# TheClimateCorporation/photon-ml

Hardware: AMD Instinct MI355X
Metric: examples/sec/node, logistic L-BFGS 1B×1M-sparse (higher is better)
Workload: dtype bf16; 1 GPU; model=logistic_regression_l2_lbfgs, global_batch=125000000, rows_per_gpu=125000000, features=1000000, nnz_per_row=100, parallelism=dp1, optimizer_state=replicated, layout=tiled

## Files before the change

### photon_ml_amd/data/synthetic.py

```python
from __future__ import annotations

import math
from typing import Optional

import numpy as np
import scipy.sparse as sp
import torch

from ..constants import TaskType
from .matrix import LabeledData


INLIER_PROBABILITY = 0.90
INLIER_STANDARD_DEVIATION = 1e-3
OUTLIER_STANDARD_DEVIATION = 1.0
SAMPLE_KINDS = ("benign", "outlier", "invalid_features", "invalid_labels")


def draw_samples(task, kind: str, seed: int, size: int, dimensionality: int,
                 desired_sparsity: float = 0.1) -> LabeledData:
    task = TaskType.parse(task)
    if kind not in SAMPLE_KINDS:
        raise ValueError(f"unknown sample kind {kind!r}, expected one of {SAMPLE_KINDS}")
    rng = np.random.default_rng(5000 * seed)
    n, d = int(size), int(dimensionality)
    u = rng.random(n)
    binary = task in (TaskType.LOGISTIC_REGRESSION, TaskType.SMOOTHED_HINGE_LOSS_LINEAR_SVM)
    if kind == "invalid_labels":
        y = np.array([np.inf, -np.inf, np.nan])[rng.integers(0, 3, n)]
        x0 = 0.1 + 0.9 * u
    elif binary:
        y = (rng.random(n) <= 0.5).astype(np.float64)
        x0 = np.where(y == 1.0, 1.0, -1.0) * (0.1 + 0.9 * u)
    elif task == TaskType.POISSON_REGRESSION:
        y = 1.0 + 10.0 * u
        x0 = (np.log(y) + rng.normal(size=n) * INLIER_STANDARD_DEVIATION) / np.log(11.0)
    elif kind == "benign":
        y = 2.0 * u - 1.0
        x0 = y + rng.normal(size=n) * INLIER_STANDARD_DEVIATION
    else:
        y = 1.0 + u
        x0 = y - 1.0 + rng.normal(size=n) * OUTLIER_STANDARD_DEVIATION
    tail_end = d - 3 if kind == "invalid_features" else d
    mask = rng.random((n, max(tail_end - 1, 0))) < desired_sparsity
    rows, cols = np.nonzero(mask)
    cols = cols + 1
    k = rows.size
    if kind in ("benign", "invalid_labels"):
        vals = 2.0 * (rng.random(k) - 0.5)
    else:
        inlier = rng.random(k) < INLIER_PROBABILITY
        if kind == "outlier":
            bad = np.where(rng.random(k) < 0.5, 1.0, -1.0)
        else:
            bad = np.array([np.nan, np.inf, -np.inf])[rng.integers(0, 3, k)]
        vals = np.where(inlier, rng.normal(size=k) * INLIER_STANDARD_DEVIATION, bad)
    r_all = [np.arange(n), rows]
    c_all = [np.zeros(n, np.int64), cols]
    v_all = [x0, vals]
    if kind == "invalid_features":
        for j, v in zip((d - 3, d - 2, d - 1), (np.nan, np.inf, -np.inf)):
            r_all.append(np.arange(n))
            c_all.append(np.full(n, j))
            v_all.append(np.full(n, v))
    x = sp.csr_matrix((np.concatenate(v_all), (np.concatenate(r_all), np.concatenate(c_all))), shape=(n, d))
    x.sort_indices()
    return LabeledData(x, y)


def generate_glm_data(task, n_rows: int, n_features: int, density: float = 0.2, seed: int = 7,
                      intercept: bool = True, noise: float = 1e-3, kind: str = "benign"):
    task = TaskType.parse(task)
    rng = np.random.default_rng(seed)
    d_feat = n_features - (1 if intercept else 0)
    x = sp.random(n_rows, d_feat, density=density, format="csr", random_state=seed,
                  data_rvs=lambda k: rng.uniform(-1, 1, size=k))
    if kind == "outlier":
        x.data *= np.where(rng.random(x.data.size) < 0.01, 1e3, 1.0)
    if intercept:
        x = sp.hstack([x, np.ones((n_rows, 1))], format="csr")
    w = rng.normal(size=n_features)
    z = x @ w
    if task == TaskType.LOGISTIC_REGRESSION or task == TaskType.SMOOTHED_HINGE_LOSS_LINEAR_SVM:
        y = (rng.random(n_rows) < 1.0 / (1.0 + np.exp(-z))).astype(np.float64)
    elif task == TaskType.POISSON_REGRESSION:
        w *= 0.2
        z = x @ w
        y = rng.poisson(np.exp(np.clip(z, -20, 5))).astype(np.float64)
    else:
        y = z + rng.normal(scale=noise, size=n_rows)
    if kind == "invalid":
        y[0] = np.nan
    return LabeledData(x, y), w


def zipf_cdf(n: int, s: float, device) -> torch.Tensor:
    k = torch.arange(1, n + 1, dtype=torch.float64, device=device)
    p = k.pow(-s)
    c = torch.cumsum(p, 0)
    return (c / c[-1]).to(torch.float32)


def generate_device_shard(n_rows: int, n_features: int, nnz_per_row: int, device="cuda", precision: str = "bf16",
                          seed: int = 1234567890, chunk_rows: int = 1 << 20, zipf_s: float = 1.1,
                          task=TaskType.LOGISTIC_REGRESSION, rank: int = 0, progress=None, layout: str = "auto"):
    from ..ops.device import DeviceGLMData, SegChunk, VAL_DTYPE, resolve_layout
    from ..ops.tiled import TLFwdChunk, TLTChunk

    dev = torch.device(device)
    prec = {"bf16": 0, "f32": 1, "f64": 2}[precision]
    vdt = VAL_DTYPE[prec]
    n_fields = nnz_per_row - 1
    if n_fields < 1:
        raise ValueError("nnz_per_row must be >= 2 (intercept + >= 1 field)")
    fs = (n_features - 1) // n_fields
    if fs < 1:
        raise ValueError("not enough features for the requested nnz per row")
    layout = resolve_layout(layout, n_features, chunk_rows)
    cdf = zipf_cdf(fs, zipf_s, dev)
    field_base = (torch.arange(n_fields, device=dev, dtype=torch.int32) * fs)
    gen = torch.Generator(device=dev)
    gen.manual_seed(seed + 7919 * rank)
    starts = list(range(0, n_rows, chunk_rows)) + [n_rows]
    k = nnz_per_row
    raw = []
    counts = torch.zeros(n_features, dtype=torch.int64, device=dev)
    for ci, (a, b) in enumerate(zip(starts[:-1], starts[1:])):
        m = b - a
        u = torch.rand((m, n_fields), generator=gen, device=dev)
        rank_ = torch.searchsorted(cdf, u).clamp_(max=fs - 1).to(torch.int32)
        del u
        idx = torch.empty((m, k), dtype=torch.int32, device=dev)
        idx[:, :n_fields] = rank_ + field_base
        idx[:, n_fields] = n_features - 1
        del rank_
        val = torch.empty((m, k), dtype=torch.float32, device=dev)
        val[:, :n_fields] = torch.rand((m, n_fields), generator=gen, device=dev) + 0.5
        val[:, n_fields] = 1.0
        idx = idx.reshape(-1)
        counts += torch.bincount(idx.to(torch.int64), minlength=n_features)
        raw.append((idx, val.to(vdt).reshape(-1)))
        if (m + 1) * k >= 2 ** 31:
            raise ValueError("chunk too large for int32 offsets: lower chunk_rows")
    import torch.distributed as dist
    from ..parallel.dist import is_dist
    if is_dist():
        cc = counts if dist.get_backend() == "nccl" else counts.cpu()
        dist.all_reduce(cc)
        counts = cc.to(dev)
    old_of_new = torch.argsort(counts, descending=True, stable=True)
    new_of_old = torch.empty_like(old_of_new)
    new_of_old[old_of_new] = torch.arange(n_features, device=dev)
    new_of_old32 = new_of_old.to(torch.int32)
    del counts
    csr, csc = [], []
    from ..ops.tiled import shard_t_config
    cbits, item_entries = shard_t_config(n_rows * k, n_rows, n_features, chunk_rows)
    for ci, ((a, b), (idx, val)) in enumerate(zip(zip(starts[:-1], starts[1:]), raw)):
        m = b - a
        idx = new_of_old32[idx.to(torch.int64)]
        if layout == "tiled":
            rp = torch.arange(0, (m + 1) * k, k, dtype=torch.int64, device=dev)
            col = idx.to(torch.int64)
            del idx
            csr.append(TLFwdChunk(rp, col, val, n_features))
            csc.append(TLTChunk(rp, col, val, n_features, chunk_rows, cbits=cbits, item_entries=item_entries))
            raw[ci] = None
            del col, val, rp
            if progress is not None:
                progress(ci + 1, len(starts) - 1)
            continue
        seg_ptr = np.arange(0, (m + 1) * k, k, dtype=np.int64).astype(np.int32)
        csr.append(SegChunk(seg_ptr, idx, val, dev, forward=True))
        perm = torch.argsort(idx, stable=True)
        cidx = (perm // k).to(torch.int32)
        cval = val[perm]
        colptr = torch.zeros(n_features + 1, dtype=torch.int64, device=dev)
        colptr[1:] = torch.cumsum(torch.bincount(idx.to(torch.int64), minlength=n_features), 0)
        del perm
        csc.append(SegChunk(colptr.cpu().numpy().astype(np.int32), cidx, cval, dev))
        raw[ci] = None
        del cidx, cval, colptr, idx, val
        if progress is not None:
            progress(ci + 1, len(starts) - 1)
    y = torch.zeros(n_rows, dtype=torch.float32, device=dev)
    data = DeviceGLMData(csr, csc, starts, y, torch.zeros_like(y), torch.ones_like(y), n_features, precision, dev,
                         old_of_new)
    wgen = torch.Generator(device=dev)
    wgen.manual_seed(seed)
    w_true = torch.randn(n_features, generator=wgen, device=dev, dtype=torch.float64) * 0.3
    w_true[torch.rand(n_features, generator=wgen, device=dev) < 0.5] = 0.0
    w_true[-1] = -1.0
    z = data.margins(w_true)
    p = torch.sigmoid(z)
    task = TaskType.parse(task)
    if task == TaskType.LOGISTIC_REGRESSION:
        yy = (torch.rand(n_rows, generator=gen, device=dev, dtype=torch.float64) < p).to(torch.float32)
    elif task == TaskType.POISSON_REGRESSION:
        yy = torch.poisson(torch.exp(z.clamp(max=5.0)) * 0.2, generator=gen).to(torch.float32)
    else:
        yy = (z + 0.1 * torch.randn(n_rows, generator=gen, device=dev, dtype=torch.float64)).to(torch.float32)
    data.y.copy_(yy.to(data.vdt))
    return data, w_true


def _device_csr_to_host(counts: torch.Tensor, cols: torch.Tensor, vals: torch.Tensor, n_cols: int) -> sp.csr_matrix:
    indptr = torch.zeros(counts.numel() + 1, dtype=torch.int64, device=counts.device)
    torch.cumsum(counts, 0, out=indptr[1:])
    x = sp.csr_matrix((vals.cpu().numpy(), cols.to(torch.int32).cpu().numpy(), indptr.cpu().numpy()),
                      shape=(counts.numel(), n_cols))
    x.has_canonical_format = True
    return x


def generate_game_bench_data_device(n_entities: int, rows_per_entity: int, re_dim: int = 100, re_nnz: int = 10,
                                    fe_dim: int = 100_000, fe_nnz: int = 30, re_vocab: int = 1 << 20, seed: int = 7,
                                    entity_offset: int = 0, task: str = "LOGISTIC_REGRESSION", pool: str = "random",
                                    int_ids: bool = False, sizes: str = "uniform", size_alpha: float = 1.3,
                                    max_rows: int = 20000, device="cuda", label_bias: float = 0.0,
                                    heavy_rows=()):
    from ..data.game_data import GameData
    dev = torch.device(device)
    gen = torch.Generator(device=dev)
    gen.manual_seed(int(seed))
    rnd = lambda *shape: torch.rand(shape, generator=gen, device=dev, dtype=torch.float64)
    if sizes == "powerlaw":
        if pool == "exact":
            raise ValueError("pool='exact' needs equal entity sizes")
        u = rnd(n_entities)
        target = n_entities * rows_per_entity
        xm = float(rows_per_entity) * (size_alpha - 1) / size_alpha
        for _ in range(30):
            cnt = torch.clamp(torch.ceil(xm * u ** (-1.0 / size_alpha)), max=max_rows).to(torch.int64)
            tot = int(cnt.sum())
            if abs(tot - target) <= 0.001 * target:
                break
            xm *= target / tot
    elif sizes == "uniform":
        cnt = torch.full((n_entities,), rows_per_entity, dtype=torch.int64, device=dev)
    else:
        raise ValueError(f"unknown entity size law {sizes!r}")
    if len(heavy_rows):
        cnt[:len(heavy_rows)] = torch.tensor([int(r) for r in heavy_rows], dtype=torch.int64, device=dev)
    n = int(cnt.sum())
    ent_sorted = torch.repeat_interleave(torch.arange(n_entities, device=dev), cnt, output_size=n)
    perm = torch.randperm(n, generator=gen, device=dev)
    ent = ent_sorted[perm]
    p = torch.arange(1, fe_dim, device=dev, dtype=torch.float64) ** -1.1
    cdf = torch.cumsum(p, 0)
    cdf /= cdf[-1].clone()
    fcol = torch.searchsorted(cdf, rnd(n, fe_nnz)).clamp_(max=fe_dim - 2)
    fcol, _ = torch.sort(fcol, dim=1)
    keep = torch.ones_like(fcol, dtype=torch.bool)
    keep[:, 1:] = fcol[:, 1:] != fcol[:, :-1]
    fval = rnd(n, fe_nnz) + 0.5
    fcol = torch.cat([fcol, torch.full((n, 1), fe_dim - 1, device=dev, dtype=fcol.dtype)], 1)
    fval = torch.cat([fval, torch.ones(n, 1, device=dev, dtype=torch.float64)], 1)
    keep = torch.cat([keep, torch.ones(n, 1, device=dev, dtype=torch.bool)], 1)
    xg = _device_csr_to_host(keep.sum(1), fcol[keep], fval[keep], fe_dim)
    wg = torch.randn(fe_dim, generator=gen, device=dev, dtype=torch.float64) * 0.2
    wg[-1] = -0.5
    zg = (fval * wg[fcol] * keep).sum(1)
    del fcol, fval, keep
    if pool == "exact":
        if re_nnz > re_dim:
            raise ValueError("pool='exact' needs re_nnz <= re_dim")
        start = torch.zeros(n_entities, dtype=torch.int64, device=dev)
        torch.cumsum(cnt[:-1], 0, out=start[1:])
        within = perm - start[ent]
        slot = (within[:, None] * re_nnz + torch.arange(re_nnz, device=dev)[None, :]) % re_dim
        del within, start
    else:
        slot = torch.randint(0, re_dim, (n, re_nnz), generator=gen, device=dev)
    del ent_sorted, perm
    gid = ent + entity_offset
    base = (gid * 2654435761) % (re_vocab - 1)
    rcol = (base[:, None] + slot * 40503) % (re_vocab - 1)
    rval = torch.randn(n, re_nnz, generator=gen, device=dev, dtype=torch.float64)
    wgen = torch.Generator(device=dev)
    wgen.manual_seed(int(seed) + 1)
    w_slot = torch.randn(re_dim, generator=wgen, device=dev, dtype=torch.float64) * 0.5
    rcol, order = torch.sort(rcol, dim=1)
    slot = torch.gather(slot, 1, order)
    rval = torch.gather(rval, 1, order)
    del order
    rkeep = torch.ones_like(rcol, dtype=torch.bool)
    rkeep[:, 1:] = rcol[:, 1:] != rcol[:, :-1]
    zr = (rval * w_slot[slot] * rkeep).sum(1) + 0.3 * torch.sin(gid.to(torch.float64))
    del slot
    rcol = torch.cat([rcol, torch.full((n, 1), re_vocab - 1, device=dev, dtype=rcol.dtype)], 1)
    rval = torch.cat([rval, torch.ones(n, 1, device=dev, dtype=torch.float64)], 1)
    rkeep = torch.cat([rkeep, torch.ones(n, 1, device=dev, dtype=torch.bool)], 1)
    xr = _device_csr_to_host(rkeep.sum(1), rcol[rkeep], rval[rkeep], re_vocab)
    del rcol, rval, rkeep
    z = zg + zr
    task = TaskType.parse(task)
    if task == TaskType.LOGISTIC_REGRESSION:
        y = (rnd(n) < torch.sigmoid(z + label_bias)).to(torch.float64)
    elif task == TaskType.POISSON_REGRESSION:
        y = torch.poisson(torch.exp(torch.clamp(z * 0.3, -10, 3)), generator=gen)
    else:
        y = z + 0.1 * torch.randn(n, generator=gen, device=dev, dtype=torch.float64)
    gid_h = gid.cpu().numpy()
    ids = gid_h.copy() if int_ids else np.char.add("e", gid_h.astype(str)).astype(object)
    return GameData(y.cpu().numpy(), {"global": xg, "entity": xr}, {"entityId": ids})


def generate_game_bench_data(n_entities: int, rows_per_entity: int, re_dim: int = 100, re_nnz: int = 10,
                             fe_dim: int = 100_000, fe_nnz: int = 30, re_vocab: int = 1 << 20, seed: int = 7,
                             entity_offset: int = 0, task: str = "LOGISTIC_REGRESSION", pool: str = "random",
                             int_ids: bool = False, sizes: str = "uniform", size_alpha: float = 1.3,
                             max_rows: int = 20000):
    from ..data.game_data import GameData
    rng = np.random.default_rng(seed)
    if sizes == "powerlaw":
        if pool == "exact":
            raise ValueError("pool='exact' needs equal entity sizes")
        u = rng.random(n_entities)
# ... 75 lines not shown
```

### photon_ml_amd/ops/csrc/game_kernels.hip

```cpp

#include <hip/hip_runtime.h>
#include <stdint.h>

#include <algorithm>

#ifndef PML_BUILD_ID
#define PML_BUILD_ID "unstamped-build!"
#endif
__attribute__((used)) static const char pml_build_stamp[] = "PML_BUILD_ID=" PML_BUILD_ID;

#define LAUNCH_CHECK()                                         \
  do {                                                         \
    hipError_t e_ = hipGetLastError();                         \
    if (e_ != hipSuccess) return (int)e_;                      \
  } while (0)

#define SCORE_GROUP 16
#define SCORE_THREADS 256
#define SCORE_ROWS_PER_BLOCK (SCORE_THREADS / SCORE_GROUP)

template <bool RE>
__global__ __launch_bounds__(SCORE_THREADS) void score_rows_kernel(
    const long long* __restrict__ indptr, const int* __restrict__ col, const double* __restrict__ val,
    long long n_rows, const double* __restrict__ w, const int* __restrict__ ent,
    const long long* __restrict__ eptr, const int* __restrict__ efeat, double* __restrict__ out) {
  const long long row = (long long)blockIdx.x * SCORE_ROWS_PER_BLOCK + (threadIdx.x / SCORE_GROUP);
  const int g = threadIdx.x % SCORE_GROUP;
  double s = 0.0;
  if (row < n_rows) {
    const long long lo = indptr[row], hi = indptr[row + 1];
    long long e_lo = 0, e_hi = 0;
    bool ok = true;
    if (RE) {
      const int e = ent[row];
      if (e < 0) ok = false;
      else { e_lo = eptr[e]; e_hi = eptr[e + 1]; }
    }
    if (ok) {
      for (long long p = lo + g; p < hi; p += SCORE_GROUP) {
        const int c = col[p];
        double wv;
        if (RE) {
          long long a = e_lo, b = e_hi;
          while (a < b) {
            const long long m = (a + b) >> 1;
            if (efeat[m] < c) a = m + 1; else b = m;
          }
          wv = (a < e_hi && efeat[a] == c) ? w[a] : 0.0;
        } else {
          wv = w[c];
        }
        s += val[p] * wv;
      }
    }
  }
#pragma unroll
  for (int o = SCORE_GROUP / 2; o > 0; o >>= 1) s += __shfl_xor(s, o, SCORE_GROUP);
  if (g == 0 && row < n_rows) out[row] = s;
}

typedef double v4d __attribute__((ext_vector_type(4)));

__device__ __forceinline__ v4d mfma_f64_16x16x4(double a, double b, v4d c) {
  return __builtin_amdgcn_mfma_f64_16x16x4f64(a, b, c, 0, 0, 0);
}


#define GN_T 32
#define GN_K 32
__global__ __launch_bounds__(256) void gemm_nt_mfma_kernel(int M, int N, int K, const double* __restrict__ A, int lda,
                                                            const double* __restrict__ Bm, int ldb,
                                                            double* __restrict__ C, int ldc) {
  __shared__ double sa[GN_T][GN_K + 1];
  __shared__ double sb[GN_T][GN_K + 1];
  const int tn = blockIdx.x, tm = blockIdx.y;
  const int lane = threadIdx.x & 63, wv = threadIdx.x >> 6;
  const int wm = wv >> 1, wn = wv & 1;
  v4d acc = {0.0, 0.0, 0.0, 0.0};
  for (int k0 = 0; k0 < K; k0 += GN_K) {
    __syncthreads();
    for (int idx = threadIdx.x; idx < GN_T * GN_K; idx += 256) {
      const int r = idx / GN_K, c = idx % GN_K;
      const int gr = tm * GN_T + r, gc = k0 + c;
      sa[r][c] = (gr < M && gc < K) ? A[(long long)gr * lda + gc] : 0.0;
      const int hr = tn * GN_T + r;
      sb[r][c] = (hr < N && gc < K) ? Bm[(long long)hr * ldb + gc] : 0.0;
    }
    __syncthreads();
#pragma unroll
    for (int kk = 0; kk < GN_K; kk += 4) {
      const double a = sa[16 * wm + (lane & 15)][kk + (lane >> 4)];
      const double b = sb[16 * wn + (lane & 15)][kk + (lane >> 4)];
      acc = mfma_f64_16x16x4(a, b, acc);
    }
  }
  const int cj = tn * GN_T + 16 * wn + (lane & 15);
#pragma unroll
  for (int i = 0; i < 4; ++i) {
    const int ri = tm * GN_T + 16 * wm + (lane >> 4) + 4 * i;
    if (ri < M && cj < N) C[(long long)ri * ldc + cj] = acc[i];
  }
}

__global__ __launch_bounds__(256) void spmm_rows_kernel(const long long* __restrict__ indptr,
                                                         const int* __restrict__ col, const double* __restrict__ val,
                                                         long long n_rows, const double* __restrict__ PT, int k,
                                                         double* __restrict__ Y) {
  const long long row = (long long)blockIdx.x * 4 + (threadIdx.x >> 6);
  const int lane = threadIdx.x & 63;
  if (row >= n_rows) return;
  const long long lo = indptr[row], hi = indptr[row + 1];
  for (int j0 = 0; j0 < k; j0 += 64) {
    const int j = j0 + lane;
    double acc = 0.0;
    for (long long p = lo; p < hi; ++p) {
      const double v = val[p];
      const long long c = col[p];
      if (j < k) acc += v * PT[c * k + j];
    }
    if (j < k) Y[row * k + j] = acc;
  }
}

__device__ __forceinline__ unsigned long long splitmix64(unsigned long long x) {
  x += 0x9E3779B97F4A7C15ull;
  x = (x ^ (x >> 30)) * 0xBF58476D1CE4E5B9ull;
  x = (x ^ (x >> 27)) * 0x94D049BB133111EBull;
  return x ^ (x >> 31);
}

template <typename T>
__global__ __launch_bounds__(256) void downsample_kernel(const T* __restrict__ y, const T* __restrict__ w0,
                                                          const long long* __restrict__ rowid, long long n,
                                                          unsigned long long seed, double rate, int binary,
                                                          T* __restrict__ w) {
  const long long i = (long long)blockIdx.x * 256 + threadIdx.x;
  if (i >= n) return;
  const unsigned long long id = rowid ? (unsigned long long)rowid[i] : (unsigned long long)i;
  const double u = (double)(splitmix64(seed ^ splitmix64(id)) >> 11) * 0x1.0p-53;
  const double wi = (double)w0[i];
  double out;
  if (binary) {
    const bool pos = (double)y[i] >= 0.5;
    out = pos ? wi : (u < rate ? wi / rate : 0.0);
  } else {
    out = u < rate ? wi : 0.0;
  }
  w[i] = (T)out;
}

#define CMP_SEG 8
struct CmpArgs {
  const int* units;
  int col_e, row_col;
  const int* seg;
  int nseg, sbits, key_is_row;
  const uint32_t* pack;
  const void* val;
  const uint16_t* npack;
  const void* nval;
  const int* nbase;
  const unsigned char* keep;
  int* seg_cnt;
  const long long* seg_first;
  const long long* unit_lo;
  uint32_t* opack;
  void* oval;
};

template <typename VT, int PASS>
__global__ __launch_bounds__(256) void tl_compact_kernel(CmpArgs a) {
  const int lane = threadIdx.x & 63;
  const int s = __builtin_amdgcn_readfirstlane(blockIdx.x * 4 + (threadIdx.x >> 6));
  if (s >= a.nseg) return;
  const int* sg = a.seg + 3 * (long long)s;
  const int u = sg[0], r_lo = sg[1], r_hi = sg[2];
  const int* ut = a.units + 6 * (long long)u;
  const long long e_lo = ut[a.col_e];
  const int nw = ut[a.col_e + 1] - ut[a.col_e];
  const int n_lo = ut[4], nn = ut[5] - ut[4];
  const uint32_t row0 = a.row_col >= 0 ? (uint32_t)ut[a.row_col] : 0u;
  const uint32_t smask = (1u << a.sbits) - 1u;
  const VT* val = (const VT*)a.val;
  const VT* nval = (const VT*)a.nval;
  long long ob = PASS ? a.seg_first[s] : 0;
  const long long olo = PASS ? a.unit_lo[u] : 0;
  const unsigned long long below = (1ull << lane) - 1ull;
  int cnt = 0;
  for (int r = r_lo; r < r_hi; ++r) {
    uint32_t p[4];
    VT v[4];
    bool ok[4];
    if (r < nn) {
      const long long q = (long long)n_lo + r;
      const int base = a.nbase[q];
#pragma unroll
      for (int k = 0; k < 4; ++k) {
        const long long pe = nval ? q * 256 + 4 * lane + k : q * 512 + 8 * lane + k;
        const uint32_t p16 = a.npack[pe];
        p[k] = ((uint32_t)(base + (int)(p16 >> a.sbits)) << a.sbits) | (p16 & smask);
        v[k] = nval ? nval[pe] : ((const VT*)a.npack)[pe + 4];
        ok[k] = true;
      }
    } else {
      const int w = r - nn;
#pragma unroll
      for (int k = 0; k < 4; ++k) {
        ok[k] = 256 * w + 64 * k + lane < nw;
        const long long e = e_lo + 256LL * w + 4 * lane + k;
        p[k] = ok[k] ? a.pack[e] : 0u;
        v[k] = ok[k] ? val[e] : (VT)0;
      }
    }
#pragma unroll
    for (int k = 0; k < 4; ++k) {
      const uint32_t row = a.key_is_row ? (p[k] >> a.sbits) : row0 + (p[k] & smask);
      const bool kp = ok[k] && a.keep[row];
      const unsigned long long m = __ballot(kp);
      if (PASS) {
        if (kp) {
          const long long o = ob + __popcll(m & below);
          const long long ph = olo + (o & ~255LL) + ((o & 63) << 2) + ((o & 255) >> 6);
          a.opack[ph] = p[k];
          ((VT*)a.oval)[ph] = v[k];
        }
        ob += __popcll(m);
      } else {
        cnt += __popcll(m);
      }
    }
  }
  if (!PASS && lane == 0) a.seg_cnt[s] = cnt;
}


template <int S, bool STAGE>
__global__ __launch_bounds__(64) void seg_gram_kernel(int B, int n, int dmax, const long long* __restrict__ ents,
                                                      const long long* __restrict__ row_ptr,
                                                      const long long* __restrict__ col_ptr,
                                                      const long long* __restrict__ nip,
                                                      const long long* __restrict__ pos,
                                                      const double* __restrict__ val, double* __restrict__ K) {
  extern __shared__ double img[];
  const int lane = threadIdx.x;
  const long long b = blockIdx.x;
  if (b >= B) return;
  const long long e = ents[b];
  const long long r0 = row_ptr[e];
  const int ne = (int)(row_ptr[e + 1] - r0);
  const long long cb = col_ptr[e];
  const int de = (int)(col_ptr[e + 1] - cb);
  const long long e0 = nip[r0];
  const int enz = (int)(nip[r0 + ne] - e0);
  double* sval = img + (size_t)dmax * S;
  unsigned short* scol = (unsigned short*)(sval + enz);
  int* sptr = (int*)(scol + ((enz + 3) & ~3));
  for (int c = lane; c < de * S; c += 64) img[c] = 0.0;
  if (STAGE) {
    for (int t = lane; t < enz; t += 64) {
      sval[t] = val[e0 + t];
      scol[t] = (unsigned short)(pos[e0 + t] - cb);
    }
    for (int i = lane; i <= ne; i += 64) sptr[i] = (int)(nip[r0 + i] - e0);
  }
  __syncthreads();
  double* Kb = K + b * (long long)n * n;
  for (int i0 = 0; i0 < ne; i0 += S) {
    const int ns = ne - i0 < S ? ne - i0 : S;
    for (int s = 0; s < ns; ++s) {
      if (STAGE) {
        const int ib = sptr[i0 + s], ie = sptr[i0 + s + 1];
        for (int t = ib + lane; t < ie; t += 64) img[(int)scol[t] * S + s] = sval[t];
      } else {
        const long long ib = nip[r0 + i0 + s], ie = nip[r0 + i0 + s + 1];
        for (long long t = ib + lane; t < ie; t += 64) img[(pos[t] - cb) * S + s] = val[t];
      }
    }
    __syncthreads();
    for (int j = lane; j < n; j += 64) {
      double acc[S];
#pragma unroll
      for (int s = 0; s < S; ++s) acc[s] = 0.0;
      if (j < ne) {
        if (STAGE) {
          const int jb = sptr[j], je = sptr[j + 1];
          for (int t = jb; t < je; ++t) {
            const double v = sval[t];
            const double* im = img + (int)scol[t] * S;
#pragma unroll
            for (int s = 0; s < S; ++s) acc[s] = fma(v, im[s], acc[s]);
          }
        } else {
          const long long jb = nip[r0 + j], je = nip[r0 + j + 1];
          for (long long t = jb; t < je; ++t) {
            const double v = val[t];
            const double* im = img + (pos[t] - cb) * S;
#pragma unroll
            for (int s = 0; s < S; ++s) acc[s] = fma(v, im[s], acc[s]);
          }
        }
      }
#pragma unroll
      for (int s = 0; s < S; ++s)
        if (s < ns) Kb[(long long)j * n + i0 + s] = acc[s];
    }
    __syncthreads();
    for (int s = 0; s < ns; ++s) {
      if (STAGE) {
        const int ib = sptr[i0 + s], ie = sptr[i0 + s + 1];
        for (int t = ib + lane; t < ie; t += 64) img[(int)scol[t] * S + s] = 0.0;
      } else {
        const long long ib = nip[r0 + i0 + s], ie = nip[r0 + i0 + s + 1];
        for (long long t = ib + lane; t < ie; t += 64) img[(pos[t] - cb) * S + s] = 0.0;
      }
    }
    __syncthreads();
  }
  for (int i = ne; i < n; ++i)
    for (int j = lane; j < n; j += 64) Kb[(long long)j * n + i] = 0.0;
}

__global__ __launch_bounds__(64) void batched_chol_kernel(int B, int n, const long long* __restrict__ nv,
                                                          double* __restrict__ K, int* __restrict__ info) {
  extern __shared__ double Lp[];
  const int lane = threadIdx.x;
  const long long b = blockIdx.x;
  if (b >= B) return;
  const int m = (int)nv[b];
  double* Kb = K + b * (long long)n * n;
  for (int i = lane; i < n; i += 64)
    for (int k = 0; k <= i; ++k)
      Lp[i * (i + 1) / 2 + k] = (i < m && k < m) ? Kb[(long long)i * n + k] : (i == k ? 1.0 : 0.0);
  __syncthreads();
  int bad = 0;
  for (int j = 0; j < m && !bad; ++j) {
    const int rj = j * (j + 1) / 2;
    double djj = Lp[rj + j];
    for (int k = 0; k < j; ++k) djj = fma(-Lp[rj + k], Lp[rj + k], djj);
    __syncthreads();
    if (!(djj > 0.0) || !isfinite(djj)) { bad = j + 1; break; }
    const double ljj = sqrt(djj);
    for (int i = j + 1 + lane; i < m; i += 64) {
      const int ri = i * (i + 1) / 2;
      double a = Lp[ri + j];
      for (int k = 0; k < j; ++k) a = fma(-Lp[ri + k], Lp[rj + k], a);
      Lp[ri + j] = a / ljj;
    }
    if (lane == 0) Lp[rj + j] = ljj;
    __syncthreads();
  }
  if (lane == 0) info[b] = bad;
  for (int i = lane; i < n; i += 64)
    for (int k = 0; k < n; ++k) Kb[(long long)i * n + k] = k <= i ? Lp[i * (i + 1) / 2 + k] : 0.0;
}

template <typename PT>
__global__ __launch_bounds__(64) void rs_primal_kernel(const long long* __restrict__ ents,
                                                       const long long* __restrict__ row_ptr,
                                                       const long long* __restrict__ col_ptr,
                                                       const long long* __restrict__ nip,
                                                       const PT* __restrict__ pos,
                                                       const double* __restrict__ val, const double* __restrict__ r,
                                                       double* __restrict__ W) {
  extern __shared__ double acc[];
  const int lane = threadIdx.x;
  const long long e = ents[blockIdx.x];
  const long long r0 = row_ptr[e], r1 = row_ptr[e + 1], c0 = col_ptr[e];
  const int d = (int)(col_ptr[e + 1] - c0);
  for (int j = lane; j < d; j += 64) acc[j] = 0.0;
// ... 1005 lines not shown
```

### photon_ml_amd/ops/csrc/glm_kernels.hip

```cpp

#include <hip/hip_runtime.h>
#include <stdint.h>
#include <math.h>
#include <algorithm>
#include <type_traits>

#define NB 4096
#define NTHREADS 256
#define VEC 8
#define MAXSEG 1024

#define LAUNCH_CHECK()                                         \
  do {                                                         \
    hipError_t e_ = hipGetLastError();                         \
    if (e_ != hipSuccess) return (int)e_;                      \
  } while (0)

enum LossId { LOSS_LOGISTIC = 0, LOSS_POISSON = 1, LOSS_SQUARED = 2, LOSS_HINGE = 3 };
enum FwdMode { FWD_MARGIN = 0, FWD_VALUE_GRAD = 1, FWD_HV = 2, FWD_DZZ = 3, FWD_LS = 4 };

struct bf16x8 { uint4 u; };

template <typename VT, typename AT> struct Loader;
template <> struct Loader<uint16_t, float> {
// ... 605 lines not shown
}

template <typename VT, typename XT, typename AT, bool SQ, int U, int NW>
__device__ __forceinline__ void tl_stream_p1(const uint32_t* __restrict__ pack, const VT* __restrict__ val,
                                          const XT* __restrict__ x, int e_lo, int e_hi, int sbits, AT* acc) {
  typedef typename TLValT<VT>::T LT;
  typedef typename TLVals<VT>::Raw Raw;
  const int lane = threadIdx.x & 63, w = threadIdx.x >> 6;
  const uint32_t smask = (1u << sbits) - 1u;
  const int lo = e_lo & ~(TL_VEC - 1);
  const int nr = (e_hi - lo + TL_ROUND - 1) / TL_ROUND;
  const int r0 = (nr * w) / NW, r1 = (nr * (w + 1)) / NW;
  if (r0 >= r1) return;
  auto load_round = [&](int r, v4u& pk, Raw& v) {
    const int e = lo + r * TL_ROUND + lane * TL_VEC;
    const int es = (r < r1 && e < e_hi) ? e : lo;
    pk = ldg_nt((const v4u*)(pack + es));
    v = TLVals<VT>::load(val + es);
  };
  auto gather = [&](int r, const v4u& pk, XT* xv) {
    const int e = lo + r * TL_ROUND + lane * TL_VEC;
#pragma unroll
    for (int k = 0; k < TL_VEC; ++k) {
      const bool in = (r < r1) && (e + k >= e_lo) && (e + k < e_hi);
      xv[k] = ldg(x + (in ? (pk[k] >> sbits) : 0u));
    }
  };
  auto accumulate = [&](int r, const v4u& pk, const Raw& v_raw, const XT* xv) {
    const int e = lo + r * TL_ROUND + lane * TL_VEC;
    LT v[TL_VEC];
    TLVals<VT>::get(v_raw, v);
#pragma unroll
    for (int k = 0; k < TL_VEC; ++k) {
      if ((e + k >= e_lo) && (e + k < e_hi)) {
        const AT vv = SQ ? static_cast<AT>(v[k]) * static_cast<AT>(v[k]) : static_cast<AT>(v[k]);
        atomicAdd(&acc[pk[k] & smask], vv * static_cast<AT>(xv[k]));
      }
    }
  };
  v4u pkA, pkB;
  Raw vA, vB;
  XT xA[TL_VEC], xB[TL_VEC];
  load_round(r0, pkA, vA);
  load_round(r0 + 1, pkB, vB);
  gather(r0, pkA, xA);
  for (int r = r0; r < r1; r += 2) {
    gather(r + 1, pkB, xB);
    {
      const v4u pk = pkA;
      const Raw vv = vA;
      XT xc[TL_VEC];
#pragma unroll
      for (int k = 0; k < TL_VEC; ++k) xc[k] = xA[k];
      load_round(r + 2, pkA, vA);
      accumulate(r, pk, vv, xc);
    }
    if (r + 1 >= r1) break;
    gather(r + 2, pkA, xA);
    {
      const v4u pk = pkB;
      const Raw vv = vB;
      XT xc[TL_VEC];
#pragma unroll
      for (int k = 0; k < TL_VEC; ++k) xc[k] = xB[k];
      load_round(r + 3, pkB, vB);
      accumulate(r + 1, pk, vv, xc);
    }
  }
}

template <typename VT, typename XT, typename AT, bool SQ, int NW, int Q>
__device__ __forceinline__ void tl_stream_wide(const uint32_t* __restrict__ pack, const VT* __restrict__ val,
                                            const XT* __restrict__ x, int e_lo, int e_hi, int sbits, AT* acc) {
  typedef typename TLValT<VT>::T LT;
  typedef typename TLVals<VT>::Raw Raw;
  constexpr int V = 4 * Q, ROUND = 64 * V;
  const int lane = threadIdx.x & 63, w = threadIdx.x >> 6;
  const uint32_t smask = (1u << sbits) - 1u;
  const int lo = e_lo & ~(TL_VEC - 1);
  const int nr = (e_hi - lo + ROUND - 1) / ROUND;
  const int r0 = (nr * w) / NW, r1 = (nr * (w + 1)) / NW;
  if (r0 >= r1) return;
  struct Slot { v4u pk[Q]; Raw v[Q]; };
  Slot A, B;
  auto load_round = [&](int r, Slot& sl) {
    const int e = lo + r * ROUND + lane * V;
#pragma unroll
    for (int q = 0; q < Q; ++q) {
      const int eq = e + 4 * q;
      const int es = (r < r1 && eq < e_hi) ? eq : lo;
      sl.pk[q] = ldg_nt((const v4u*)(pack + es));
      sl.v[q] = TLVals<VT>::load(val + es);
    }
  };
  auto process = [&](int r, Slot& sl) {
    v4u pk[Q];
    Raw vr[Q];
#pragma unroll
    for (int q = 0; q < Q; ++q) { pk[q] = sl.pk[q]; vr[q] = sl.v[q]; }
    const int e = lo + r * ROUND + lane * V;
    bool in[V];
    XT xv[V];
#pragma unroll
    for (int q = 0; q < Q; ++q)
#pragma unroll
      for (int k = 0; k < 4; ++k) {
        const int i = 4 * q + k;
        in[i] = (e + i >= e_lo) && (e + i < e_hi);
        xv[i] = ldg(x + (in[i] ? (pk[q][k] >> sbits) : 0u));
      }
    if (r + 2 < r1) load_round(r + 2, sl);
#pragma unroll
    for (int q = 0; q < Q; ++q) {
      LT v[4];
      TLVals<VT>::get(vr[q], v);
#pragma unroll
      for (int k = 0; k < 4; ++k) {
        const int i = 4 * q + k;
        if (in[i]) {
          const AT vv = SQ ? static_cast<AT>(v[k]) * static_cast<AT>(v[k]) : static_cast<AT>(v[k]);
          atomicAdd(&acc[pk[q][k] & smask], vv * static_cast<AT>(xv[i]));
        }
      }
    }
  };
  load_round(r0, A);
  if (r0 + 1 < r1) load_round(r0 + 1, B);
  for (int r = r0; r < r1; r += 2) {
    process(r, A);
    if (r + 1 < r1) process(r + 1, B);
  }
}


#ifdef PML_TL_EXPERIMENT
__constant__ int c_tl_ablate = 0;
#define TL_ABL c_tl_ablate
#else
#define TL_ABL 0
#endif

__device__ const int g_zero_base[1] = {0};
typedef const __attribute__((address_space(4))) int* const_int_p;

template <typename VT, typename XT, typename AT, bool SQ, int NW, int S, int D>
__device__ __forceinline__ void tl_stream_ring(const uint32_t* __restrict__ pack, const VT* __restrict__ val,
                                               const XT* __restrict__ x, int e_lo, int e_hi, int sbits, AT* acc,
                                               const int* wbase) {
  constexpr int R = S + 1;
  static_assert(D < S && R % (D + 1) == 0, "gathers run ahead of loaded slots; the gather ring divides the slots");
  typedef typename TLValT<VT>::T LT;
  typedef typename TLVals<VT>::Raw Raw;
  const int lane = threadIdx.x & 63;
  const int w = __builtin_amdgcn_readfirstlane(threadIdx.x >> 6);
  const uint32_t smask = (1u << sbits) - 1u;
  const int nr = (e_hi - e_lo + TL_ROUND - 1) / TL_ROUND;
  const int r0 = (nr * w) / NW, r1 = (nr * (w + 1)) / NW;
  if (r0 >= r1) return;
  v4u pk[R];
  Raw vr[R];
  uint32_t bs[R];
  XT xg[D + 1][TL_VEC];
  const int ws = wbase ? 1 : 0;
  const const_int_p wb = (const_int_p)(wbase ? wbase : g_zero_base);
  const int rb0 = e_lo / TL_ROUND;
  auto load_round = [&](int r, v4u& p, Raw& v, uint32_t& b) {
    const int e = e_lo + min(r, r1 - 1) * TL_ROUND + lane * TL_VEC;
    p = ldg_nt((const v4u*)(pack + e));
    v = TLVals<VT>::load(val + e);
    b = (uint32_t)wb[ws * (rb0 + min(r, r1 - 1))];
  };
  const int abl = TL_ABL;
  AT regsum = AT(0);
  auto gather = [&](int r, const v4u& p, uint32_t b, XT* xv) {
    const int e = e_lo + r * TL_ROUND + lane;
#pragma unroll
    for (int k = 0; k < TL_VEC; ++k) {
      const uint32_t key = (e + 64 * k < e_hi) ? b + (p[k] >> sbits) : 0u;
      const bool hot = key < ((uint32_t)abl >> 8) << 10;
      if (abl & 10) xv[k] = XT(1);
      else if ((abl & 32) && hot) xv[k] = XT(1);
      else if ((abl & 64) && __ballot(!hot) == 0ull) xv[k] = XT(1);
      else xv[k] = ldg(x + key);
    }
  };
#pragma unroll
  for (int i = 0; i < S; ++i) {
    load_round(r0 + i, pk[i], vr[i], bs[i]);
    __builtin_amdgcn_sched_barrier(0);
  }
#pragma unroll
  for (int i = 0; i < D; ++i) {
    gather(r0 + i, pk[i], bs[i], xg[i]);
    __builtin_amdgcn_sched_barrier(0);
  }
  for (int r = r0; r < r1; r += R) {
#pragma unroll
    for (int i = 0; i < R; ++i) {
      const int rc = r + i;
      load_round(rc + S, pk[(i + S) % R], vr[(i + S) % R], bs[(i + S) % R]);
      __builtin_amdgcn_sched_barrier(0);
      gather(rc + D, pk[(i + D) % R], bs[(i + D) % R], xg[(i + D) % (D + 1)]);
      __builtin_amdgcn_sched_barrier(0);
      LT v[TL_VEC];
      TLVals<VT>::get(vr[i], v);
      const int e = e_lo + rc * TL_ROUND + lane;
#pragma unroll
      for (int k = 0; k < TL_VEC; ++k) {
        const bool in = (e + 64 * k < e_hi) && (rc < r1);
        const AT vv = SQ ? static_cast<AT>(v[k]) * static_cast<AT>(v[k]) : static_cast<AT>(v[k]);
        AT add;
        if (abl & 4) add = in ? static_cast<AT>(static_cast<float>(v[k]) * static_cast<float>(xg[i % (D + 1)][k]))
                              : AT(0);
        else add = in ? vv * static_cast<AT>(xg[i % (D + 1)][k]) : AT(0);
        if (abl & 1) regsum += add;
        else atomicAdd(&acc[in ? (pk[i][k] & smask) : 0u], add);
      }
      __builtin_amdgcn_sched_barrier(0);
    }
  }
  if (abl & 1) atomicAdd(&acc[lane], regsum);
}

template <typename T> __device__ __forceinline__ T lane_bcast(T v, int src) { return __shfl(v, src, 64); }

template <typename VT, bool FUSED> struct TLNarrowSlot {
  typedef typename TLVals<VT>::Raw Raw;
  v2u pk;
  Raw v;
  __device__ __forceinline__ void load(const uint16_t* npk, const VT* nvl, size_t e) {
    pk = ldg_nt((const v2u*)(npk + e));
    v = TLVals<VT>::load(nvl + e);
  }
  __device__ __forceinline__ v2u packs() const { return pk; }
  __device__ __forceinline__ Raw vals() const { return v; }
};
template <> struct TLNarrowSlot<uint16_t, true> {
  typedef v2u Raw;
  v4u rec;
  __device__ __forceinline__ void load(const uint16_t* npk, const uint16_t*, size_t e) {
    rec = ldg_nt((const v4u*)(npk + 2 * e));
  }
  __device__ __forceinline__ v2u packs() const { v2u p; p.x = rec.x; p.y = rec.y; return p; }
  __device__ __forceinline__ Raw vals() const { v2u u; u.x = rec.z; u.y = rec.w; return u; }
};

template <typename VT, typename XT, typename AT, bool SQ, int NW, int S = 2, bool FUSED = false>
__device__ __forceinline__ void tl_stream_narrow(const uint16_t* __restrict__ npk, const VT* __restrict__ nvl,
                                                 const int* __restrict__ nbs, int n_lo, int n_hi, int sbits,
                                                 const XT* __restrict__ x, AT* acc) {
  constexpr int R = S + 1;
  typedef typename TLValT<VT>::T LT;
  typedef typename TLVals<VT>::Raw Raw;
  const int lane = threadIdx.x & 63;
  const int w = __builtin_amdgcn_readfirstlane(threadIdx.x >> 6);
  const int nr = n_hi - n_lo;
  const int r0 = n_lo + (nr * w) / NW, r1 = n_lo + (nr * (w + 1)) / NW;
  if (r0 >= r1) return;
  const uint32_t smask = (1u << sbits) - 1u;
  const const_int_p bp = (const_int_p)nbs;
  typedef TLNarrowSlot<VT, FUSED> Slot;
  Slot sl[R];
  XT xs[R];
  const int abl = TL_ABL;
  AT regsum = AT(0);
  auto issue = [&](int r, int base, Slot& s, XT& xw) {
    const size_t e = (size_t)min(r, r1 - 1) * TL_ROUND + lane * TL_VEC;
    s.load(npk, nvl, e);
    xw = (abl & 18) ? XT(1) : ldg(x + base + lane);
  };
#pragma unroll
  for (int i = 0; i < S; ++i) {
    issue(r0 + i, bp[min(r0 + i, r1 - 1)], sl[i], xs[i]);
    __builtin_amdgcn_sched_barrier(0);
  }
  int nb = bp[min(r0 + S, r1 - 1)];
  for (int r = r0; r < r1; r += R) {
#pragma unroll
    for (int i = 0; i < R; ++i) {
      const int rc = r + i;
      issue(rc + S, nb, sl[(i + S) % R], xs[(i + S) % R]);
      nb = bp[min(rc + S + 1, r1 - 1)];
      __builtin_amdgcn_sched_barrier(0);
      const bool live = rc < r1;
      LT v[TL_VEC];
      TLVals<VT>::get(sl[i].vals(), v);
      const v2u pk = sl[i].packs();
      const uint32_t p[TL_VEC] = {pk.x & 0xffffu, pk.x >> 16, pk.y & 0xffffu, pk.y >> 16};
#pragma unroll
      for (int k = 0; k < TL_VEC; ++k) {
        const XT xv = (abl & 16) ? xs[i] : lane_bcast(xs[i], (int)(p[k] >> sbits));
        const AT vv = SQ ? static_cast<AT>(v[k]) * static_cast<AT>(v[k]) : static_cast<AT>(v[k]);
        AT add;
        if (abl & 4) add = live ? static_cast<AT>(static_cast<float>(v[k]) * static_cast<float>(xv)) : AT(0);
        else add = live ? vv * static_cast<AT>(xv) : AT(0);
        if (abl & 1) regsum += add + AT(p[k] & smask);
        else atomicAdd(&acc[live ? (p[k] & smask) : 0u], add);
      }
      __builtin_amdgcn_sched_barrier(0);
    }
  }
  if (abl & 1) atomicAdd(&acc[lane], regsum);
}

template <typename VT, typename XT, typename AT, bool SQ, int U, int NW, int P>
__device__ __forceinline__ void tl_stream(const uint32_t* __restrict__ pack, const VT* __restrict__ val,
                                          const XT* __restrict__ x, int e_lo, int e_hi, int sbits, AT* acc,
                                          const int* wbase = nullptr) {
  if (P == 1) tl_stream_p1<VT, XT, AT, SQ, U, NW>(pack, val, x, e_lo, e_hi, sbits, acc);
  else if (P == 2) tl_stream_wide<VT, XT, AT, SQ, NW, 2>(pack, val, x, e_lo, e_hi, sbits, acc);
  else if (P == 3) tl_stream_ring<VT, XT, AT, SQ, NW, 2, 0>(pack, val, x, e_lo, e_hi, sbits, acc, wbase);
  else if (P == 5) tl_stream_ring<VT, XT, AT, SQ, NW, 3, 1>(pack, val, x, e_lo, e_hi, sbits, acc, wbase);
  else if (P == 6) tl_stream_ring<VT, XT, AT, SQ, NW, 5, 2>(pack, val, x, e_lo, e_hi, sbits, acc, wbase);
  else tl_stream_p0<VT, XT, AT, SQ, U, NW>(pack, val, x, e_lo, e_hi, sbits, acc);
}

struct TLNarrow { const uint16_t* pack; const void* val; const int* base; const int* wbase; };

template <typename VT, typename XT, typename AT, bool SQ, int NW, int S>
__device__ __forceinline__ void tl_narrow(const TLNarrow& nar, int n_lo, int n_hi, int sbits,
                                          const XT* __restrict__ x, AT* acc) {
  if constexpr (sizeof(VT) == 2) {
    if (nar.val == nullptr) {
      tl_stream_narrow<VT, XT, AT, SQ, NW, S, true>(nar.pack, nullptr, nar.base, n_lo, n_hi, sbits, x, acc);
      return;
    }
  }
  tl_stream_narrow<VT, XT, AT, SQ, NW, S, false>(nar.pack, (const VT*)nar.val, nar.base, n_lo, n_hi, sbits, x, acc);
}

template <typename VT, typename XT, typename RT, typename AT, int MAXR, int U, int NW, int P>
__device__ __forceinline__ void tl_fwd_block(int b, int row_lo, int nrows, int e_lo, int e_hi, int n_lo, int n_hi,
                                             int rbits, const uint32_t* __restrict__ pack,
                                             const VT* __restrict__ val, const TLNarrow& nar,
                                             const XT* __restrict__ x, const FwdArgs<XT, RT>& a,
                                             double* __restrict__ stats, AT (*acc)[MAXR], double* red) {
  const int R = 1 << rbits;
  for (int i = threadIdx.x; i < R; i += NW * 64)
#pragma unroll
    for (int w = 0; w < NW; ++w) acc[w][i] = AT(0);
  __syncthreads();
  if (n_hi > n_lo)
    tl_narrow<VT, XT, AT, false, NW, (P >= 5 ? 4 : 2)>(nar, n_lo, n_hi, rbits, x, acc[threadIdx.x >> 6]);
  tl_stream<VT, XT, AT, false, U, NW, P>(pack, val, x, e_lo, e_hi, rbits, acc[threadIdx.x >> 6], nar.wbase);
  __syncthreads();
  double F = 0.0, S = 0.0;
  for (int r = threadIdx.x; r < nrows; r += NW * 64) {
    double z = static_cast<double>(acc[0][r]);
#pragma unroll
    for (int w = 1; w < NW; ++w) z += static_cast<double>(acc[w][r]);
    const int s = row_lo + r;
    fwd_finish(a, s, z, fwd_prefetch(a, s), F, S);
  }
  if (stats) {
    block_sum2_nw<NW>(F, S, red);
    if (threadIdx.x == 0) { stats[2 * b] = F; stats[2 * b + 1] = S; }
  }
}

template <typename VT, typename XT, typename RT, typename AT, int MAXR, int U, int NW, int P>
__global__ __launch_bounds__(NW * 64) void tl_fwd_kernel(const int* __restrict__ blk, int rbits,
                                                          const uint32_t* __restrict__ pack,
                                                          const VT* __restrict__ val, TLNarrow nar,
                                                          const XT* __restrict__ x, FwdArgs<XT, RT> a,
                                                          double* __restrict__ stats,
                                                          const unsigned char* __restrict__ live) {
  __shared__ AT acc[NW][MAXR];
  __shared__ double red[2 * NW];
  const int b = blockIdx.x;
  if (live && !live[b]) return;
  const int* q = blk + 6 * b;
  tl_fwd_block<VT, XT, RT, AT, MAXR, U, NW, P>(b, q[0], q[1], q[2], q[3], q[4], q[5], rbits, pack, val, nar, x, a,
                                              stats, acc, red);
}

template <typename VT, typename XT, typename RT, typename AT, int MAXR, int U, int NW, int P>
__global__ __launch_bounds__(NW * 64) void tl_fwd_multi_kernel(const int* __restrict__ blk, int rbits,
                                                                const unsigned long long* __restrict__ ptrs,
                                                                const XT* __restrict__ x, FwdArgs<XT, RT> a,
                                                                double* __restrict__ stats,
                                                                const unsigned char* __restrict__ live) {
  __shared__ AT acc[NW][MAXR];
  __shared__ double red[2 * NW];
  const int b = blockIdx.x;
  if (live && !live[b]) return;
  const int* q = blk + 8 * b;
  const unsigned long long* pc = ptrs + 6 * q[0];
  const TLNarrow nar = {(const uint16_t*)pc[2], (const void*)pc[3], (const int*)pc[4], (const int*)pc[5]};
  tl_fwd_block<VT, XT, RT, AT, MAXR, U, NW, P>(b, q[1], q[2], q[3], q[4], q[6], q[7], rbits, (const uint32_t*)pc[0],
                                              (const VT*)pc[1], nar, x + q[5], a, stats, acc, red);
}

template <typename VT, typename XT, typename AT, bool SQ, int MAXR, int U, int NW, int P>
__device__ __forceinline__ void tl_t_item(int tile, int e_lo, int e_hi, int part, int n_lo, int n_hi, int cbits,
                                          const uint32_t* __restrict__ pack, const VT* __restrict__ val,
                                          const TLNarrow& nar, const XT* __restrict__ x, double* __restrict__ G,
                                          int dim, double* __restrict__ parts, AT (*acc)[MAXR]) {
  const int C = 1 << cbits;
  for (int i = threadIdx.x; i < C; i += NW * 64)
#pragma unroll
    for (int w = 0; w < NW; ++w) acc[w][i] = AT(0);
  __syncthreads();
  if (n_hi > n_lo)
    tl_narrow<VT, XT, AT, SQ, NW, (P >= 5 ? 4 : 2)>(nar, n_lo, n_hi, cbits, x, acc[threadIdx.x >> 6]);
  tl_stream<VT, XT, AT, SQ, U, NW, P>(pack, val, x, e_lo, e_hi, cbits, acc[threadIdx.x >> 6], nar.wbase);
  __syncthreads();
  const int c0 = tile << cbits;
  for (int c = threadIdx.x; c < C; c += NW * 64) {
    double s = static_cast<double>(acc[0][c]);
#pragma unroll
    for (int w = 1; w < NW; ++w) s += static_cast<double>(acc[w][c]);
    if (part < 0) {
      if (c0 + c < dim) G[c0 + c] += s;
    } else {
      parts[(size_t)part * C + c] = s;
    }
  }
}

template <typename VT, typename XT, typename AT, bool SQ, int MAXR, int U, int NW, int P>
__global__ __launch_bounds__(NW * 64) void tl_t_kernel(const int* __restrict__ items, int cbits,
                                                        const uint32_t* __restrict__ pack,
                                                        const VT* __restrict__ val, TLNarrow nar,
                                                        const XT* __restrict__ x, double* __restrict__ G, int dim,
                                                        double* __restrict__ parts,
                                                        const unsigned char* __restrict__ live) {
  __shared__ AT acc[NW][MAXR];
  if (live && !live[blockIdx.x]) return;
  const int* q = items + 6 * blockIdx.x;
  tl_t_item<VT, XT, AT, SQ, MAXR, U, NW, P>(q[0], q[1], q[2], q[3], q[4], q[5], cbits, pack, val, nar, x, G, dim,
                                            parts, acc);
}

template <typename VT, typename XT, typename AT, bool SQ, int MAXR, int U, int NW, int P>
__global__ __launch_bounds__(NW * 64) void tl_t_multi_kernel(const int* __restrict__ items, int cbits,
                                                              const unsigned long long* __restrict__ ptrs,
                                                              const XT* __restrict__ x, double* __restrict__ G,
                                                              int dim, double* __restrict__ parts,
                                                              const unsigned char* __restrict__ live,
                                                              const int* __restrict__ gate) {
  __shared__ AT acc[NW][MAXR];
  if (gate && *gate == 0) return;
  if (live && !live[blockIdx.x]) return;
  const int* q = items + 8 * blockIdx.x;
  const unsigned long long* pc = ptrs + 6 * q[0];
  const TLNarrow nar = {(const uint16_t*)pc[2], (const void*)pc[3], (const int*)pc[4], (const int*)pc[5]};
  tl_t_item<VT, XT, AT, SQ, MAXR, U, NW, P>(q[1], q[2], q[3], q[4], q[6], q[7], cbits, (const uint32_t*)pc[0],
                                            (const VT*)pc[1], nar, x + q[5], G, dim, parts, acc);
}

__device__ __forceinline__ double rows_sum64(const double* __restrict__ src, int C, int r0, int r1, int c,
                                             double* sh) {
  const int w = threadIdx.x >> 6, lane = threadIdx.x & 63;
  const int n = r1 - r0;
  const int q0 = r0 + (n * w) / 4, q1 = r0 + (n * (w + 1)) / 4;
  double s0 = 0.0, s1 = 0.0, s2 = 0.0, s3 = 0.0;
  if (c < C) {
    int r = q0;
    for (; r + 3 < q1; r += 4) {
      s0 += src[(size_t)r * C + c];
      s1 += src[(size_t)(r + 1) * C + c];
      s2 += src[(size_t)(r + 2) * C + c];
      s3 += src[(size_t)(r + 3) * C + c];
    }
    for (; r < q1; ++r) s0 += src[(size_t)r * C + c];
  }
  sh[w * 64 + lane] = (s0 + s1) + (s2 + s3);
  __syncthreads();
  return (sh[lane] + sh[64 + lane]) + (sh[128 + lane] + sh[192 + lane]);
}

__global__ __launch_bounds__(NTHREADS) void tl_t_combine1_kernel(const int* __restrict__ cu, int cbits,
                                                                 const double* __restrict__ parts,
                                                                 double* __restrict__ l1,
                                                                 const unsigned char* __restrict__ live_mt) {
  __shared__ double sh[NTHREADS];
  const int u = blockIdx.x;
  if (live_mt && !live_mt[cu[3 * u]]) return;
  const int C = 1 << cbits;
  const int c = blockIdx.y * 64 + (threadIdx.x & 63);
  const double s = rows_sum64(parts, C, cu[3 * u + 1], cu[3 * u + 2], c, sh);
  if (threadIdx.x < 64 && c < C) l1[(size_t)u * C + c] = s;
}

__global__ __launch_bounds__(NTHREADS) void tl_t_combine2_kernel(const int* __restrict__ mt_tiles,
                                                                 const int* __restrict__ mt_ptr, int cbits,
                                                                 const double* __restrict__ l1,
                                                                 double* __restrict__ G, int dim,
                                                                 const unsigned char* __restrict__ live_mt) {
  __shared__ double sh[NTHREADS];
  const int t = blockIdx.x;
  if (live_mt && !live_mt[t]) return;
  const int C = 1 << cbits;
  const int c = blockIdx.y * 64 + (threadIdx.x & 63);
  const double s = rows_sum64(l1, C, mt_ptr[t], mt_ptr[t + 1], c, sh);
  if (threadIdx.x < 64 && c < C) {
    const int col = (mt_tiles[t] << cbits) + c;
    if (col < dim) G[col] += s;
  }
}

struct TLFwdDesc { const int* blk; int nblk; int rbits; const uint32_t* pack; const void* val; int il; TLNarrow nar;
                  const unsigned char* live; };
struct TLFwdMultiDesc { const int* blk; int nblk; int rbits; const unsigned long long* ptrs; int il;
                       const unsigned char* live; };
struct TLTDesc {
  const int* items; int nitems; int cbits; const uint32_t* pack; const void* val;
  const int* mt_tiles; const int* mt_ptr; int nmt; int dim;
  const int* cu; int ncu;
  int nparts_total;
  int il;
  TLNarrow nar;
  const unsigned char* live;
  const unsigned char* live_mt;
};
struct TLTMultiDesc {
  const int* items; int nitems; int cbits; const unsigned long long* ptrs;
  const int* mt_tiles; const int* mt_ptr; int nmt; int dim;
  const int* cu; int ncu; int nparts_total; int il;
  const unsigned char* live;
  const unsigned char* live_mt;
};

static int g_ablate = 0;
static double* g_ls_z0 = nullptr;
static double g_ls_t0 = 0.0, g_ls_tpend = 0.0;
static const int* g_gate = nullptr;
static const double* g_ls_z0_in = nullptr;
static const double* g_ls_zd_in = nullptr;
template <typename A>
static inline A& with_ls_in(A& a) {
  a.z0_in = g_ls_z0_in ? g_ls_z0_in : g_ls_z0;
  a.zd_in = g_ls_zd_in ? g_ls_zd_in : a.z_out;
  return a;
}
template <typename XT>
static FwdArgs<XT, XT> fwd_args(int mode, int loss, double shift, const void* y, const void* off, const void* wt,
                                void* coef, void* dzz, double* z_out, int with_offset) {
  FwdArgs<XT, XT> a{mode, loss, shift, (const XT*)y, (const XT*)off, (const XT*)wt, (XT*)coef, (XT*)dzz, z_out,
                    with_offset, g_ablate, 0, g_ls_z0, g_ls_t0, g_ls_tpend};
  return with_ls_in(a);
}
template <typename F>
static int with_prec(int prec, F f) {
  if (prec == 2) return f(double{}, double{});
  if (prec == 1) return f(float{}, float{});
  return f(uint16_t{}, float{});
}
template <typename F>
static int with_prec_sq(int prec, int square, F f) {
  return with_prec(prec, [&](auto vt, auto xt) {
    return square ? f(vt, xt, std::true_type{}) : f(vt, xt, std::false_type{});
  });
}
static int g_tl_acc64 = 1;
static int g_tl_waves = 4;
static int g_tl_waves_t = 4;
static int g_tl_pipe = 0;
static int g_tl_pipe_t = 0;
static int g_rs_variant = 5;
static int g_tl_deep = 0;
static int g_tl_deep_t = 0;

#ifdef PML_TL_EXPERIMENT
constexpr bool TL_EXPERIMENT = true;
#else
constexpr bool TL_EXPERIMENT = false;
#endif

template <typename AT_, int MAXR_> struct TLAcc { using AT = AT_; static constexpr int MAXR = MAXR_; };
template <int NW_, int P_> struct TLPipe { static constexpr int NW = NW_, P = P_; };

template <typename XT> static inline int tl_maxbits() { return sizeof(XT) == 8 ? 11 : TL_MAXBITS; }
template <typename XT, typename F>
static int tl_with_acc(int bits, F f) {
  if (bits < 1 || bits > tl_maxbits<XT>()) return -22;
  if constexpr (sizeof(XT) != 8) {
    if (bits == 12) { f(TLAcc<float, 4096>{}); return 0; }
    if constexpr (TL_EXPERIMENT) {
      if (!g_tl_acc64) {
        if (bits <= 10) f(TLAcc<float, 1024>{}); else f(TLAcc<float, 2048>{});
        return 0;
      }
    }
  }
  if (bits <= 10) f(TLAcc<double, 1024>{}); else f(TLAcc<double, 2048>{});
  return 0;
}

template <int NW_PROD, int ALT_P, typename F>
static void tl_with_pipe(int il, int waves, int deep, int pipe, F f) {
  if constexpr (!TL_EXPERIMENT) {
    if (il) f(TLPipe<NW_PROD, 3>{}); else f(TLPipe<NW_PROD, 0>{});
  } else {
    auto with_p = [&](auto nw) {
      constexpr int NW = decltype(nw)::value;
      if (il) {
        if (deep == 2) f(TLPipe<NW, 6>{}); else if (deep) f(TLPipe<NW, 5>{}); else f(TLPipe<NW, 3>{});
      } else if (pipe == ALT_P) f(TLPipe<NW, ALT_P>{});
      else f(TLPipe<NW, 0>{});
    };
    if (waves == 2) with_p(std::integral_constant<int, 2>{}); else with_p(std::integral_constant<int, 4>{});
  }
}

template <typename VT, typename XT, typename RT>
static int tl_fwd_impl(const TLFwdDesc* c, const void* x, FwdArgs<XT, RT> a, double* stats, hipStream_t st) {
  if (c->nblk <= 0) return 0;
  const int rc = tl_with_acc<XT>(c->rbits, [&](auto acc) {
    tl_with_pipe<2, 1>(c->il, g_tl_waves, g_tl_deep, g_tl_pipe, [&](auto pipe) {
      using A = decltype(acc); using Q = decltype(pipe);
      hipLaunchKernelGGL((tl_fwd_kernel<VT, XT, RT, typename A::AT, A::MAXR, 2, Q::NW, Q::P>), dim3(c->nblk),
                         dim3(Q::NW * 64), 0, st, c->blk, c->rbits, c->pack, (const VT*)c->val, c->nar, (const XT*)x,
                         a, stats, c->live);
    });
  });
  if (rc) return rc;
  LAUNCH_CHECK();
  return 0;
}

template <typename VT, typename XT, typename RT>
static int tl_fwd_multi_impl(const TLFwdMultiDesc* c, const void* x, FwdArgs<XT, RT> a, double* stats,
                             hipStream_t st) {
  if (c->nblk <= 0) return 0;
  const int rc = tl_with_acc<XT>(c->rbits, [&](auto acc) {
    tl_with_pipe<2, 2>(c->il, g_tl_waves, g_tl_deep, g_tl_pipe, [&](auto pipe) {
      using A = decltype(acc); using Q = decltype(pipe);
      hipLaunchKernelGGL((tl_fwd_multi_kernel<VT, XT, RT, typename A::AT, A::MAXR, 2, Q::NW, Q::P>), dim3(c->nblk),
                         dim3(Q::NW * 64), 0, st, c->blk, c->rbits, c->ptrs, (const XT*)x, a, stats, c->live);
    });
  });
  if (rc) return rc;
  LAUNCH_CHECK();
  return 0;
}

template <typename Desc>
static int tl_t_combine(const Desc* c, double* G, double* parts, hipStream_t st) {
  if (c->nmt <= 0) return 0;
  const int C = 1 << c->cbits;
  double* l1 = parts + (size_t)c->nparts_total * C;
  hipLaunchKernelGGL(tl_t_combine1_kernel, dim3(c->ncu, (C + 63) / 64), dim3(NTHREADS), 0, st, c->cu, c->cbits,
                     parts, l1, c->live_mt);
  LAUNCH_CHECK();
  hipLaunchKernelGGL(tl_t_combine2_kernel, dim3(c->nmt, (C + 63) / 64), dim3(NTHREADS), 0, st,
                     c->mt_tiles, c->mt_ptr, c->cbits, l1, G, c->dim, c->live_mt);
  LAUNCH_CHECK();
  return 0;
}

template <typename VT, typename XT, bool SQ>
static int tl_t_impl(const TLTDesc* c, const void* x, double* G, double* parts, hipStream_t st) {
  if (c->nitems <= 0) return 0;
  const int rc = tl_with_acc<XT>(c->cbits, [&](auto acc) {
    tl_with_pipe<4, 1>(c->il, g_tl_waves_t, g_tl_deep_t, g_tl_pipe_t, [&](auto pipe) {
      using A = decltype(acc); using Q = decltype(pipe);
      hipLaunchKernelGGL((tl_t_kernel<VT, XT, typename A::AT, SQ, A::MAXR, 2, Q::NW, Q::P>), dim3(c->nitems),
                         dim3(Q::NW * 64), 0, st, c->items, c->cbits, c->pack, (const VT*)c->val, c->nar, (const XT*)x,
                         G, c->dim, parts, c->live);
    });
  });
  if (rc) return rc;
  LAUNCH_CHECK();
  return tl_t_combine(c, G, parts, st);
}

template <typename VT, typename XT, bool SQ>
static int tl_t_multi_impl(const TLTMultiDesc* c, const void* x, double* G, double* parts, hipStream_t st) {
  if (c->nitems <= 0) return 0;
  const int rc = tl_with_acc<XT>(c->cbits, [&](auto acc) {
    tl_with_pipe<4, 2>(c->il, g_tl_waves_t, g_tl_deep_t, g_tl_pipe_t, [&](auto pipe) {
      using A = decltype(acc); using Q = decltype(pipe);
      hipLaunchKernelGGL((tl_t_multi_kernel<VT, XT, typename A::AT, SQ, A::MAXR, 2, Q::NW, Q::P>), dim3(c->nitems),
                         dim3(Q::NW * 64), 0, st, c->items, c->cbits, c->ptrs, (const XT*)x, G, c->dim, parts, c->live,
                         g_gate);
    });
  });
  if (rc) return rc;
  LAUNCH_CHECK();
  return tl_t_combine(c, G, parts, st);
}

template <typename VT> __device__ __forceinline__ void cs_vals(const typename TLVals<VT>::Raw& raw, double* v) {
  typename TLValT<VT>::T t[TL_VEC];
  TLVals<VT>::get(raw, t);
#pragma unroll
  for (int k = 0; k < TL_VEC; ++k) v[k] = static_cast<double>(t[k]);
}

template <typename VT, int NW, typename F>
__device__ __forceinline__ void cs_for_each(const int* __restrict__ q, int cbits, const uint32_t* __restrict__ pack,
                                            const VT* __restrict__ val, const TLNarrow& nar, int il, F f) {
  typedef typename TLVals<VT>::Raw Raw;
  const int lane = threadIdx.x & 63;
  const int w = __builtin_amdgcn_readfirstlane(threadIdx.x >> 6);
  const uint32_t smask = (1u << cbits) - 1u;
  const int e_lo = q[1], e_hi = q[2], n_lo = q[4], n_hi = q[5];
  double v[TL_VEC];
  {
    const int nr = n_hi - n_lo;
    const int r0 = n_lo + (int)(((long long)nr * w) / NW), r1 = n_lo + (int)(((long long)nr * (w + 1)) / NW);
    bool fused = false;
    if constexpr (sizeof(VT) == 2) fused = nar.val == nullptr;
    for (int r = r0; r < r1; ++r) {
      const size_t e = (size_t)r * TL_ROUND + lane * TL_VEC;
      v2u pk;
      if (fused) {
        if constexpr (sizeof(VT) == 2) {
          const v4u rec = ldg_nt((const v4u*)(nar.pack + 2 * e));
          pk.x = rec.x; pk.y = rec.y;
          v2u u; u.x = rec.z; u.y = rec.w;
          cs_vals<VT>(u, v);
        }
      } else {
        pk = ldg_nt((const v2u*)(nar.pack + e));
        const Raw raw = TLVals<VT>::load((const VT*)nar.val + e);
        cs_vals<VT>(raw, v);
      }
      f(pk.x & 0xffffu & smask, v[0]);
      f((pk.x >> 16) & smask, v[1]);
      f(pk.y & 0xffffu & smask, v[2]);
      f((pk.y >> 16) & smask, v[3]);
    }
  }
  if (il) {
    const int n = e_hi - e_lo;
    const int nr = (n + TL_ROUND - 1) / TL_ROUND;
    const int r0 = (int)(((long long)nr * w) / NW), r1 = (int)(((long long)nr * (w + 1)) / NW);
    for (int r = r0; r < r1; ++r) {
      const size_t e = (size_t)e_lo + (size_t)r * TL_ROUND + lane * TL_VEC;
      const v4u pk = ldg_nt((const v4u*)(pack + e));
      const Raw raw = TLVals<VT>::load(val + e);
      cs_vals<VT>(raw, v);
      const int j = r * TL_ROUND + lane;
#pragma unroll
      for (int k = 0; k < TL_VEC; ++k)
        if (j + 64 * k < n) f(pk[k] & smask, v[k]);
    }
  } else {
    const int lo = e_lo & ~(TL_VEC - 1);
    const int nr = (e_hi - lo + TL_ROUND - 1) / TL_ROUND;
    const int r0 = (int)(((long long)nr * w) / NW), r1 = (int)(((long long)nr * (w + 1)) / NW);
    for (int r = r0; r < r1; ++r) {
      const int e = lo + r * TL_ROUND + lane * TL_VEC;
      if (e >= e_hi) continue;
      const v4u pk = ldg_nt((const v4u*)(pack + e));
      const Raw raw = TLVals<VT>::load(val + e);
      cs_vals<VT>(raw, v);
#pragma unroll
      for (int k = 0; k < TL_VEC; ++k)
        if (e + k >= e_lo && e + k < e_hi) f(pk[k] & smask, v[k]);
    }
  }
}

template <typename VT, int MAXR, int NW>
__global__ __launch_bounds__(NW * 64) void tl_colsum_kernel(const int* __restrict__ items, int cbits,
                                                            const uint32_t* __restrict__ pack,
                                                            const VT* __restrict__ val, TLNarrow nar, int il,
                                                            int which, double* __restrict__ G, int dim,
                                                            double* __restrict__ parts) {
  __shared__ double acc[NW][MAXR];
  const int* q = items + 6 * blockIdx.x;
  const int C = 1 << cbits;
  for (int i = threadIdx.x; i < C; i += NW * 64)
#pragma unroll
    for (int w = 0; w < NW; ++w) acc[w][i] = 0.0;
  __syncthreads();
  double* mine = acc[threadIdx.x >> 6];
  cs_for_each<VT, NW>(q, cbits, pack, val, nar, il, [&](uint32_t slot, double v) {
    const double t = which == 0 ? v : which == 1 ? v * v : which == 2 ? fabs(v) : 1.0;
    atomicAdd(&mine[slot], t);
  });
  __syncthreads();
  const int c0 = q[0] << cbits, part = q[3];
  for (int c = threadIdx.x; c < C; c += NW * 64) {
    double s = acc[0][c];
// ... 2277 lines not shown
```

### photon_ml_amd/ops/device.py

```python
from __future__ import annotations

import ctypes
import os
import threading
from dataclasses import dataclass
from typing import List, Optional, Sequence

import numpy as np
import scipy.sparse as sp
import torch

from ..data.matrix import LabeledData
from .native import SegChunkDesc, check, require_glm_lib, stream_handle
from .reference import GLMComputable
from .tiled import DEFAULT_ITEM_ENTRIES, TLFwdChunk, TLTChunk, tl_supported
from ..utils.timing import phase, trace_range

H2D_GATE = threading.Event()

LAYOUTS = ("auto", "tiled", "segmented")


def resolve_layout(layout: str, dim: int, chunk_rows: int) -> str:
    import os
    if layout == "auto":
        layout = os.environ.get("PML_LAYOUT", "auto")
    if layout not in LAYOUTS:
        raise ValueError(f"unknown layout {layout}")
    if layout == "auto":
        layout = "tiled" if tl_supported(dim, chunk_rows) else "segmented"
    if layout == "tiled" and not tl_supported(dim, chunk_rows):
        raise ValueError(f"tiled layout cannot pack dim={dim} with chunk_rows={chunk_rows}")
    return layout

PRECISIONS = {"bf16": 0, "f32": 1, "f64": 2}
VAL_DTYPE = {0: torch.bfloat16, 1: torch.float32, 2: torch.float64}
VEC_DTYPE = {0: torch.float32, 1: torch.float32, 2: torch.float64}

FWD_MARGIN, FWD_VALUE_GRAD, FWD_HV, FWD_DZZ, FWD_LS = 0, 1, 2, 3, 4


def _pad8(n: int) -> int:
    return ((n + 7) // 8) * 8 + 8


def _ptr(t: Optional[torch.Tensor]) -> Optional[int]:
    return None if t is None else t.data_ptr()


class SegChunk:

    def __init__(self, seg_ptr: np.ndarray, idx: torch.Tensor, val: torch.Tensor, device, nb: Optional[int] = None,
                 maxseg: Optional[int] = None, forward: bool = False):
        lib = require_glm_lib()
        seg_ptr = np.ascontiguousarray(seg_ptr, dtype=np.int32)
        nseg = len(seg_ptr) - 1
        nb = nb or lib.pml_nb()
        maxseg = maxseg or (lib.pml_maxseg_fwd() if forward else lib.pml_maxseg())
        nblk, nlong, npart = ctypes.c_int(), ctypes.c_int(), ctypes.c_int()
        check(lib.pml_build_blocks(seg_ptr.ctypes.data, nseg, nb, maxseg, None, ctypes.byref(nblk), None, None,
                                   ctypes.byref(nlong), ctypes.byref(npart)), "count blocks")
        blk = np.zeros(max(5 * nblk.value, 5), dtype=np.int32)
        long_seg = np.zeros(max(nlong.value, 1), dtype=np.int32)
        long_ptr = np.zeros(nlong.value + 1, dtype=np.int32)
        check(lib.pml_build_blocks(seg_ptr.ctypes.data, nseg, nb, maxseg, blk.ctypes.data, ctypes.byref(nblk),
                                   long_seg.ctypes.data, long_ptr.ctypes.data, ctypes.byref(nlong),
                                   ctypes.byref(npart)), "build blocks")
        self.nseg, self.nblk, self.nlong, self.npart = nseg, nblk.value, nlong.value, npart.value
        self.nnz = int(seg_ptr[-1])
        dev = torch.device(device)
        self.seg_ptr = torch.from_numpy(seg_ptr).to(dev)
        self.blk = torch.from_numpy(blk).to(dev)
        self.long_seg = torch.from_numpy(long_seg).to(dev)
        self.long_ptr = torch.from_numpy(long_ptr).to(dev)
        n_pad = _pad8(self.nnz)
        if idx.numel() < n_pad:
            idx = torch.cat([idx.to(dev, torch.int32), torch.zeros(n_pad - idx.numel(), dtype=torch.int32, device=dev)])
        if val.numel() < n_pad:
            val = torch.cat([val.to(dev), torch.zeros(n_pad - val.numel(), dtype=val.dtype, device=dev)])
        self.idx = idx.contiguous()
        self.val = val.contiguous()
        self.desc = SegChunkDesc(self.blk.data_ptr(), self.nblk, self.seg_ptr.data_ptr(), self.nseg,
                                 self.idx.data_ptr(), self.val.data_ptr(), self.long_seg.data_ptr(),
                                 self.long_ptr.data_ptr(), self.nlong, self.npart)

    kind = "seg"

    @property
    def nstats(self) -> int:
        return self.nblk

    @property
    def parts_needed(self) -> int:
        return self.npart

    def nbytes(self) -> int:
        return sum(t.numel() * t.element_size() for t in (self.seg_ptr, self.blk, self.long_seg, self.long_ptr,
                                                           self.idx, self.val))


MASK_STATS = [] if os.environ.get("PML_TRON_STATS") == "1" else None

NARROW_FILTER_BELOW = float(os.environ.get("PML_DS_NARROW_FILTER_BELOW", "0.23"))

OFFSET_SHIFT_CACHE = os.environ.get("PML_OFFSET_SHIFT_CACHE", "1") != "0"


class VecKey:

    __slots__ = ("src", "ver")

    def __init__(self, w: torch.Tensor):
        self.src = w
        self.ver = w._version

    @property
    def shape(self):
        return self.src.shape

    def matches(self, w: torch.Tensor) -> bool:
        if w is self.src and w._version == self.ver:
            return True
        if self.src._version != self.ver or self.src.shape != w.shape:
            return False
        return bool(torch.equal(self.src, w.to(self.src.device, self.src.dtype)))


def _window_align(chunk_rows: int, precision: str) -> int:
    from .tiled import t_bits
    cb = t_bits(chunk_rows, precision == "f64")
    return 1 << cb if cb is not None else 1


class DeviceGLMData(GLMComputable):

    def __init__(self, csr: List[SegChunk], csc: List[SegChunk], row_starts: Sequence[int], y, offsets, weights,
                 dim: int, precision: str = "f64", device="cuda", old_of_new: Optional[torch.Tensor] = None):
        self.lib = require_glm_lib()
        self.device = torch.device(device)
        if self.device.type == "cuda":
            from .native import check_lds_add_order
            check_lds_add_order(self.device)
        self.prec = PRECISIONS[precision]
        self.precision = precision
        self.vdt = VEC_DTYPE[self.prec]
        self.csr, self.csc = csr, csc
        self.row_starts = list(row_starts)
        self.n_rows = self.row_starts[-1]
        self.dim = int(dim)
        rdt = self.vdt
        self.y = torch.as_tensor(y, device=self.device).to(rdt).contiguous()
        self.o = torch.as_tensor(offsets, device=self.device).to(rdt).contiguous()
        self.wt = torch.as_tensor(weights, device=self.device).to(rdt).contiguous()
        n = self.n_rows
        self.coef = torch.zeros(max(n, 1), dtype=rdt, device=self.device)
        self.dzz = torch.zeros(max(n, 1), dtype=rdt, device=self.device)
        self.track_hessian = False
        self._dzz_key: Optional[torch.Tensor] = None
        self._dzz_shift = None
        self.layout = "tiled" if csr and csr[0].kind == "tl" else "segmented"
        self.col_lo = [0] * len(csr)
        self.blk_off = np.cumsum([0] + [c.nstats for c in csr]).tolist()
        self.long_off = np.cumsum([0] + [getattr(c, "nlong", 0) for c in csr]).tolist()
        self.stats = torch.zeros(2 * max(self.blk_off[-1], 1), dtype=torch.float64, device=self.device)
        self.long_stats = torch.zeros(2 * max(self.long_off[-1], 1), dtype=torch.float64, device=self.device)
        maxpart = max([c.parts_needed for c in csr + csc] + [1])
        self.parts = torch.zeros(maxpart, dtype=torch.float64, device=self.device)
        self.red_scratch = torch.zeros(512, dtype=torch.float64, device=self.device)
        self.out2 = torch.zeros(2, dtype=torch.float64, device=self.device)
        self.n_passes = 0
        self.old_of_new = None if old_of_new is None else old_of_new.to(self.device, torch.int64)
        if self.old_of_new is not None:
            self.new_of_old = torch.empty_like(self.old_of_new)
            self.new_of_old[self.old_of_new] = torch.arange(self.dim, device=self.device)
        if os.environ.get("PML_CHECK_KERNEL_INPUTS", "0") == "1":
            self.validate()

    def validate(self):
        from .tiled import il_phys
        for c, (f, t) in enumerate(zip(self.csr, self.csc)):
            if f.kind != "tl":
                continue
            m = self.row_starts[c + 1] - self.row_starts[c]
            b = f.blk.cpu().to(torch.int64)
            if f.nblk and (int(b[:, 0].min()) < 0 or int((b[:, 0] + b[:, 1]).max()) > m
                           or int(b[:, 1].max()) > (1 << f.rbits)):
                raise ValueError(f"chunk {c}: forward block rows out of range")
            q = 256 if f.il else 4
            end = b[:, 2] + (b[:, 3] - b[:, 2] + q - 1) // q * q if f.il else (b[:, 3] + 3) // 4 * 4
            if f.nblk and (int(b[:, 2].min()) < 0 or int(end.max()) > f.pack.numel()):
                raise ValueError(f"chunk {c}: forward block window outside the stream")
            if f.il and f.nblk and bool((b[:, 2] % 256 != 0).any()):
                raise ValueError(f"chunk {c}: interleaved forward windows not round-aligned")
            ncols = int(self.dim) - self.col_lo[c]
            self._validate_narrow(c, f, b, ncols, "forward")
            pk, _ = f.logical()
            p = pk.cpu().to(torch.int64)
            wb = getattr(f, "wbase", None)
            if wb is not None and wb.numel() and int(wb.min()) < 0:
                raise ValueError(f"chunk {c}: negative wide-round base")
            if p.numel() and int((p >> f.rbits).max()) >= ncols:
                raise ValueError(f"chunk {c}: forward gather index >= column window")
            counts = f.unit_counts().cpu()
            blk_rows = torch.repeat_interleave(b[:, 1], counts)
            if p.numel() and bool(((p & ((1 << f.rbits) - 1)) >= blk_rows).any()):
                raise ValueError(f"chunk {c}: forward LDS slot >= block rows")
            it = t.items.cpu().to(torch.int64)
            if t.nitems:
                if int(it[:, 1].min()) < 0 or int(it[:, 2].max()) > t.pack.numel():
                    raise ValueError(f"chunk {c}: transpose item window outside the stream")
                if int(it[:, 3].max()) >= max(t.nparts, 1) and t.nparts:
                    raise ValueError(f"chunk {c}: transpose partial-row slot out of range")
                self._validate_narrow(c, t, it, m, "transpose")
                tp, _ = t.logical()
                q = tp.cpu().to(torch.int64) & 0xFFFFFFFF
                if q.numel() and int((q >> t.cbits).max()) >= m:
                    raise ValueError(f"chunk {c}: transpose gather row >= chunk rows")
                cols = (torch.repeat_interleave(it[:, 0], t.unit_counts().cpu()) << t.cbits) + (q & ((1 << t.cbits) - 1))
                if q.numel() and int(cols.max()) >= t.dim:
                    raise ValueError(f"chunk {c}: transpose column >= dim")
        if self.parts.numel() < max([c.parts_needed for c in self.csr + self.csc] + [1]):
            raise ValueError("partial-row scratch too small")
        self._validate_multi()
        return True

    def _validate_multi(self):
        mb = getattr(self, "_multi", None)
        if mb is not None and not isinstance(mb, str):
            t = self._multi_blk.cpu().to(torch.int64)
            for c, ch in enumerate(self.csr):
                r = t[t[:, 0] == c]
                if ch.il and r.shape[0] and (int(r[:, 3].min()) < 0 or int((r[:, 3] + (r[:, 4] - r[:, 3] + 255) // 256 * 256).max())
                                   > ch.pack.numel() or int(r[:, 7].max()) > ch.nbase.numel() * (ch.n_narrow_rounds > 0)):
                    raise ValueError(f"chunk {c}: shard-wide forward table outside the chunk's streams")
        mt = getattr(self, "_multi_t", None)
        if mt is not None and not isinstance(mt, str):
            if self.parts.numel() < mt.parts_needed:
                raise ValueError("partial-row scratch too small for the shard-wide transpose")
            t = mt.items.cpu().to(torch.int64)
            for c, ch in enumerate(self.csc):
                r = t[t[:, 0] == c]
                if ch.il and r.shape[0] and (int(r[:, 2].min()) < 0 or int((r[:, 2] + (r[:, 3] - r[:, 2] + 255) // 256 * 256).max())
                                   > ch.pack.numel() or int(r[:, 7].max()) > ch.nbase.numel() * (ch.n_narrow_rounds > 0)):
                    raise ValueError(f"chunk {c}: shard-wide transpose table outside the chunk's streams")

    @staticmethod
    def _validate_narrow(c: int, ch, table: torch.Tensor, xlen: int, what: str):
        if table.shape[0] == 0:
            return
        n_lo, n_hi = table[:, 4], table[:, 5]
        nrounds = ch.nbase.numel() if ch.n_narrow_rounds else 0
        if bool((n_hi < n_lo).any()) or int(n_hi.max()) > nrounds or bool((n_lo[1:] != n_hi[:-1]).any()):
            raise ValueError(f"chunk {c}: {what} narrow round ranges inconsistent")
        if nrounds:
            base = ch.nbase.cpu().to(torch.int64)
            if ch.npack.numel() < 256 * nrounds or ch.nval.numel() < 256 * nrounds:
                raise ValueError(f"chunk {c}: {what} narrow stream shorter than its rounds")
            if ch.fused and (ch.nrec.numel() < 512 * nrounds or ch.val.element_size() != 2
                             or not ch.nrec.is_contiguous()):
                raise ValueError(f"chunk {c}: {what} fused narrow records need 2-byte values, 16 B per lane and round")
            if int(base.min()) < 0 or int(base.max()) + 64 > xlen:
                raise ValueError(f"chunk {c}: {what} narrow key window outside the gathered vector")

    @staticmethod
    def from_labeled(data: LabeledData, device="cuda", precision: str = "f64", chunk_rows: int = 1 << 20,
                     relabel: bool = True, layout: str = "auto", item_entries: Optional[int] = None,
                     col_windows: bool = False):
        if col_windows:
            relabel = False
        prec = PRECISIONS[precision]
        vdt = VAL_DTYPE[prec]
        dev = torch.device(device)
        x = data.x.tocsr()
        n, d = x.shape
        if dev.type == "cuda" and n and resolve_layout(layout, d, chunk_rows) == "tiled":
            return DeviceGLMData._from_labeled_device(x, data, dev, precision, chunk_rows, relabel, item_entries,
                                                      col_windows)
        if hasattr(x, "to_scipy"):
            x = x.to_scipy()
        old_of_new = None
        from ..parallel.dist import is_dist
        shared = relabel and is_dist() and not col_windows
        if shared or (relabel and x.nnz > 0):
            counts = np.bincount(x.indices, minlength=d).astype(np.int64)
            if shared:
                import torch.distributed as tdist
                from ..parallel.sharding import comm_device
                ct = torch.from_numpy(counts).to(comm_device())
                tdist.all_reduce(ct)
                counts = ct.cpu().numpy()
            old_of_new_np = np.argsort(-counts, kind="stable")
            new_of_old_np = np.empty(d, dtype=np.int64)
            new_of_old_np[old_of_new_np] = np.arange(d)
            x = sp.csr_matrix((x.data, new_of_old_np[x.indices], x.indptr), shape=x.shape)
            old_of_new = torch.from_numpy(old_of_new_np)
        starts = list(range(0, n, chunk_rows)) + [n]
        if n == 0:
            starts = [0, 0]
        csr, csc = [], []
        col_lo = []
        wins = []
        align = _window_align(chunk_rows, precision)
        for a, b in zip(starts[:-1], starts[1:]):
            xc = x[a:b]
            if col_windows and xc.nnz:
                lo, hi = int(xc.indices.min()), int(xc.indices.max()) + 1
                lo -= lo % align
            else:
                lo, hi = 0, d
            wins.append((lo, hi))
        dmax = max([hi - lo for lo, hi in wins] + [1])
        layout = resolve_layout(layout, dmax, chunk_rows)
        cbits = None
        if layout == "tiled" and not col_windows and item_entries is None:
            from .tiled import shard_t_config
            cbits, item_entries = shard_t_config(int(x.nnz), n, d, chunk_rows)
        for (a, b), (lo, hi) in zip(zip(starts[:-1], starts[1:]), wins):
            xc = x[a:b]
            col_lo.append(lo)
            if lo != 0 or hi != d:
                xc = sp.csr_matrix((xc.data, xc.indices - lo, xc.indptr), shape=(b - a, hi - lo))
            dc = hi - lo
            if layout == "tiled":
                rp = torch.from_numpy((xc.indptr - xc.indptr[0]).astype(np.int64)).to(dev)
                col = torch.from_numpy(xc.indices.astype(np.int64)).to(dev)
                val = torch.from_numpy(xc.data.astype(np.float64)).to(dev).to(vdt)
                csr.append(TLFwdChunk(rp, col, val, dc))
                csc.append(TLTChunk(rp, col, val, dc, chunk_rows, cbits=cbits, item_entries=item_entries))
                continue
            sp_ = (xc.indptr - xc.indptr[0]).astype(np.int32)
            csr.append(SegChunk(sp_, torch.from_numpy(xc.indices.astype(np.int32)),
                                torch.from_numpy(xc.data.astype(np.float64)).to(vdt), dev, forward=True))
            xt = xc.tocsc()
            xt.sort_indices()
            xc = xc.copy()
            csc.append(SegChunk(xt.indptr.astype(np.int32), torch.from_numpy(xt.indices.astype(np.int32)),
                                torch.from_numpy(xt.data.astype(np.float64)).to(vdt), dev))
        out = DeviceGLMData(csr, csc, starts, torch.from_numpy(data.y), torch.from_numpy(data.offsets),
                            torch.from_numpy(data.weights), d, precision, dev, old_of_new)
        out.col_lo = col_lo
        return out

    @staticmethod
    def _from_labeled_device(x, data: LabeledData, dev, precision: str, chunk_rows: int, relabel: bool,
                             item_entries: Optional[int], col_windows: bool):
        n, d = x.shape
        with phase("tiled build: upload"):
            if isinstance(x.indptr, torch.Tensor):
                indptr, col, val = x.indptr.to(dev), x.indices.to(dev).to(torch.int64), x.data.to(dev)
            else:
                indptr = torch.from_numpy(np.ascontiguousarray(x.indptr, dtype=np.int64)).to(dev)
                col = torch.from_numpy(np.ascontiguousarray(x.indices)).to(dev).to(torch.int64)
                val = torch.from_numpy(np.ascontiguousarray(x.data)).to(dev)
        H2D_GATE.set()
        old_of_new = None
        from ..parallel.dist import is_dist
        shared = relabel and is_dist() and not col_windows
        relabel_phase = phase("tiled build: hottest-first relabel")
        relabel_phase.__enter__()
        if shared or (relabel and col.numel() > 0):
            from .native import key_histogram
            counts = key_histogram(col, d)
            if shared:
                import torch.distributed as tdist
                from ..parallel.sharding import comm_device
                ct = counts.to(comm_device())
                tdist.all_reduce(ct)
                counts = ct.to(dev)
            oon = torch.argsort(-counts, stable=True)
            non = torch.empty_like(oon)
            non[oon] = torch.arange(d, device=dev)
            col = non[col]
            old_of_new = (oon, non)
            del counts
        relabel_phase.__exit__(None, None, None)
        out = DeviceGLMData.from_device_csr(indptr, col, val, torch.from_numpy(data.y), torch.from_numpy(data.offsets),
                                            torch.from_numpy(data.weights), d, dev, precision, chunk_rows,
                                            item_entries=item_entries, col_windows=col_windows)
        if old_of_new is not None:
            out.old_of_new, out.new_of_old = old_of_new
        return out

    @staticmethod
    def from_device_csr(indptr: torch.Tensor, col: torch.Tensor, val: torch.Tensor, y, offsets, weights, dim: int,
                        device="cuda", precision: str = "f64", chunk_rows: int = 1 << 20,
                        item_entries: Optional[int] = None, col_windows: bool = False):
        dev = torch.device(device)
        vdt = VAL_DTYPE[PRECISIONS[precision]]
        indptr = indptr.to(dev, torch.int64)
        col = col.to(dev, torch.int64)
        n = indptr.numel() - 1
        starts = list(range(0, n, chunk_rows)) + [n] if n else [0, 0]
        ip = indptr[torch.tensor(starts, device=dev)].tolist()
        wins = []
        align = _window_align(chunk_rows, precision)
        for i in range(len(starts) - 1):
            ea, eb = ip[i], ip[i + 1]
            if col_windows and eb > ea:
                lo, hi = torch.aminmax(col[ea:eb])
                lo = int(lo)
                wins.append((lo - lo % align, int(hi) + 1))
            else:
                wins.append((0, dim))
        dmax = max([hi - lo for lo, hi in wins] + [1])
        if resolve_layout("auto", dmax, chunk_rows) != "tiled":
            raise ValueError(f"from_device_csr needs the tiled layout (window {dmax} columns)")
        cbits = None
        if not col_windows and item_entries is None:
            from .tiled import shard_t_config
            cbits, item_entries = shard_t_config(int(ip[-1] - ip[0]), n, dim, chunk_rows)
        csr, csc, col_lo = [], [], []
        chunk_phase = phase(f"tiled build: {len(wins)} chunk layouts")
        chunk_phase.__enter__()
        for i, (lo, hi) in enumerate(wins):
            a, b = starts[i], starts[i + 1]
            ea, eb = ip[i], ip[i + 1]
            rp = indptr[a:b + 1] - ea
            c = col[ea:eb] - lo if lo else col[ea:eb]
            v = val[ea:eb].to(dev).to(vdt)
            csr.append(TLFwdChunk(rp, c, v, hi - lo))
            csc.append(TLTChunk(rp, c, v, hi - lo, chunk_rows, cbits=cbits, item_entries=item_entries))
            col_lo.append(lo)
            del c, v
        chunk_phase.__exit__(None, None, None)
        out = DeviceGLMData(csr, csc, starts, y, offsets, weights, dim, precision, dev, None)
        out.col_lo = col_lo
        return out

    def nbytes(self) -> int:
        return sum(c.nbytes() for c in self.csr + self.csc)

    def row_sampled(self, keep: torch.Tensor) -> Optional["DeviceGLMData"]:
        from .tiled import RowCompaction, stream_ptr_table
        from .native import TLFwdMultiDesc
        if self.layout != "tiled" or not self.csr or not all(getattr(ch, "il", 0) for ch in self.csr + self.csc):
            return None
        if any(getattr(ch, "wbase", None) is not None for ch in self.csr):
            return None
        keep = keep.to(self.device, torch.uint8).contiguous()
        assert keep.numel() >= self.n_rows
        n = self.n_rows
        if getattr(self, "_multi", "unset") == "unset":
            self._build_multi()
        if getattr(self, "_multi_t", "unset") == "unset":
            self._build_multi_t()
        frac = float(keep[:n].sum()) / max(n, 1)
        filt = frac < NARROW_FILTER_BELOW
        jobs = []
        for c in range(len(self.csr)):
            kc = keep[self.row_starts[c]: self.row_starts[c + 1]]
            jobs.append(RowCompaction(self.csr[c], kc, True, filt))
            jobs.append(RowCompaction(self.csc[c], kc, False, filt))
        sizes = torch.stack([torch.stack([j.total, j.kept]) for j in jobs]).tolist()
        out = [j.finish(int(t), int(k)) for j, (t, k) in zip(jobs, sizes)]
        view = DeviceGLMData(out[0::2], out[1::2], self.row_starts, self.y, self.o, self.wt, self.dim,
                             self.precision, self.device, None)
        view.col_lo = list(self.col_lo)
        view.old_of_new = self.old_of_new
        if self.old_of_new is not None:
            view.new_of_old = self.new_of_old
        view.sampled_from = self
        view.kept_fraction = frac
        view._frob_sq = self.frob_sq()
        if getattr(self, "z_cache", None) is not None and getattr(self, "_z_key", None) is not None:
            view.enable_margin_cache()
            view.z_cache.copy_(self.z_cache)
            view.zd.copy_(self.zd)
            view._z_key, view._z_chain, view._tpend = self._z_key, self._z_chain, self._tpend
        if self._multi is not None:
            nb = self._multi_blk.clone()
            cb = torch.cat([ch.blk for ch in view.csr])
            nb[:, 3:5] = cb[:, 2:4]
            nb[:, 6:8] = cb[:, 4:6]
            view._multi_blk = nb
            view._multi_ptrs = stream_ptr_table(view.csr, self.device)
            view._multi = TLFwdMultiDesc(nb.data_ptr(), nb.shape[0], self._multi.rbits, view._multi_ptrs.data_ptr(),
                                         self._multi.il)
        view._multi_t = None if self._multi_t is None else self._multi_t.restreamed(view.csc)
        gb = getattr(self, "_gbuckets", None)
        if gb is not None and gb[1] is not None:
            view._gbuckets = (gb[0], [(mt.restreamed(view.csc), c0, c1) for mt, c0, c1 in gb[1]])
        view.parts = self.parts
        if os.environ.get("PML_CHECK_KERNEL_INPUTS", "0") == "1":
            view.validate()
        return view

    def set_offsets_sum(self, base: torch.Tensor, part: torch.Tensor) -> bool:
        n = self.n_rows
        if not (n > 0 and base.is_cuda and part.is_cuda and base.dtype == part.dtype == torch.float64
                and base.numel() == part.numel() == n == self.o.numel() and base.is_contiguous()
                and part.is_contiguous() and base.device == self.o.device == part.device):
            return False
        from .native import offset_update
        zc = getattr(self, "z_cache", None)
        shift = (zc is not None and getattr(self, "_z_key", None) is not None and self._z_chain + 1 < self.LS_REFRESH
                 and getattr(self, "_masked", None) is None and OFFSET_SHIFT_CACHE)
        offset_update(base, part, self.o, zc[:n] if shift else None)
        if shift:
            self._z_chain += 1
            self._ls_t0 = None
        else:
            self._z_key = None
        self._step_base = None
        self._dzz_key = None
        return True

    def set_offsets(self, offsets):
        new = torch.as_tensor(offsets, device=self.device).to(self.vdt)
        zc = getattr(self, "z_cache", None)
        if (zc is not None and getattr(self, "_z_key", None) is not None and self._z_chain + 1 < self.LS_REFRESH
                and getattr(self, "_masked", None) is None and OFFSET_SHIFT_CACHE):
            n = self.n_rows
            zc[:n].add_(new[:n].to(torch.float64) - self.o[:n].to(torch.float64))
            self._z_chain += 1
            self._ls_t0 = None
        else:
            self._z_key = None
        self.o.copy_(new)
        self._step_base = None
        self._dzz_key = None

    def mark_weights_changed(self):
        self._dzz_key = None
        self._ls_t0 = None

    LS_REFRESH = 50

    def enable_margin_cache(self):
        if getattr(self, "z_cache", None) is None:
            n = max(self.n_rows, 1)
            self.z_cache = torch.zeros(n, dtype=torch.float64, device=self.device)
            self.zd = torch.zeros(n, dtype=torch.float64, device=self.device)
            self.ls_stats = torch.zeros(2 * 4096, dtype=torch.float64, device=self.device)
            self.ls_out = torch.zeros(2, dtype=torch.float64, device=self.device)
            self._z_key, self._z_chain, self._tpend, self._ls_t0 = None, 0, 0.0, None
        return True

    def _z_valid_for(self, w_eff, shift) -> bool:
        key = getattr(self, "_z_key", None)
        return (key is not None and key[1] == float(shift) and self._z_chain < self.LS_REFRESH
                and key[0].matches(w_eff))

    def ls_begin(self, w0_eff, shift0, d_eff, d_shift, t0: float = 1.0, loss=None, alt: bool = False,
                 stats_out: Optional[torch.Tensor] = None) -> bool:
        if loss is None:
            return False
        if getattr(self, "z_cache", None) is None:
            if alt:
                return False
            self.enable_margin_cache()
        if not self._z_valid_for(w0_eff, shift0):
            if alt:
                return False
            self.fwd_all(self._vec(w0_eff), FWD_MARGIN, 0, shift0, None, None, z_out=self.z_cache, with_offset=1,
                         stats=False)
            self._z_key, self._z_chain, self._tpend = (VecKey(w0_eff), float(shift0)), 0, 0.0
        if alt:
            from .native import KERNEL_CONFIG
            if getattr(self, "_multi", "unset") == "unset":
                self._build_multi()
            if (self._multi is None or not KERNEL_CONFIG.get("tl_multi", 1)
                    or getattr(self, "_masked", None) is not None):
                return False
        with trace_range("K1' direction pass (margins of d + first trial)"):
            if alt:
                zin, din = self.z_cache, self.zd
                if getattr(self, "_zalt", None) is None:
                    self._zalt = (torch.empty_like(zin), torch.empty_like(din))
                zout, dout = self._zalt
                self.lib.pml_set_ls_in(zin.data_ptr(), din.data_ptr())
            else:
                zout, dout = self.z_cache, self.zd
            self.lib.pml_set_ls_args(zout.data_ptr(), float(t0), float(self._tpend))
            try:
                self.fwd_all(self._vec(d_eff), FWD_LS, loss.loss_id, d_shift, self.coef, None, z_out=dout)
            finally:
                self.lib.pml_set_ls_args(None, 0.0, 0.0)
                if alt:
                    self.lib.pml_set_ls_in(None, None)
            if alt:
                self.z_cache, self.zd, self._zalt = zout, dout, (zin, din)
            self._tpend = 0.0
            self._ls_t0 = float(t0)
            self._coef_stale = False
            if stats_out is None:
                stats_out = torch.empty(2, dtype=torch.float64, device=self.device)
            self._ls_t0_dev = self._reduce_stats(stats_out)
            self._ls_t0_host = None
        return True

    _LS_STATE = ("z_cache", "zd", "_zalt", "_tpend", "_ls_t0", "_ls_t0_dev", "_ls_t0_host", "_z_key", "_z_chain",
                 "_track_u", "_dzz_key", "_dzz_shift", "_coef_stale", "_step_base")

    def ls_checkpoint(self) -> dict:
        return {k: getattr(self, k, None) for k in self._LS_STATE}

    def ls_restore(self, ck: dict, t0_host=None):
        for k, v in ck.items():
            setattr(self, k, v)
        self._coef_stale = True
        if t0_host is not None and self._ls_t0 is not None:
            self._ls_t0_host = tuple(float(v) for v in t0_host)

    @property
    def _ls_t0_vals(self):
        if self._ls_t0_host is None:
            self._ls_t0_host = tuple(self._ls_t0_dev.tolist())
        return self._ls_t0_host

    def _ls(self, loss, t, final, out):
        dzz = self.dzz if (final and self.track_hessian and loss.twice_differentiable) else None
        check(self.lib.pml_ls_eval(self.prec, self.n_rows, float(t), loss.loss_id, self.z_cache.data_ptr(),
                                   self.zd.data_ptr(), self.y.data_ptr(), self.wt.data_ptr(), int(final),
                                   self.coef.data_ptr() if final else None, None if dzz is None else dzz.data_ptr(),
                                   self.ls_stats.data_ptr(), out.data_ptr(), stream_handle(self.device)), "ls_eval")

    def ls_eval(self, loss, t: float):
        if self._ls_t0 is not None and float(t) == self._ls_t0:
            return self._ls_t0_vals
        with trace_range("line-search trial (margin space)"):
            self._ls(loss, t, 0, self.ls_out)
            f, d = self.ls_out.tolist()
        return f, d

    def ls_gate_supported(self) -> bool:
        from .native import KERNEL_CONFIG
        if getattr(self, "_multi_t", "unset") == "unset":
            self._build_multi_t()
        return (self._multi_t is not None and KERNEL_CONFIG.get("tl_multi", 1) and getattr(self, "_masked", None) is None
                and getattr(self, "_ls_t0", None) == 1.0 and not getattr(self, "_coef_stale", False)
# ... 28 lines not shown
            return [self.ls_eval(loss, t) for t in ts]
        with trace_range("line-search trials (margin space, one pass)"):
            need = len(ts) * 2 * 4096
            if getattr(self, "_ls_multi_stats", None) is None or self._ls_multi_stats.numel() < need:
                self._ls_multi_stats = torch.empty(self.LS_MULTI_MAX * 2 * 4096, dtype=torch.float64,
                                                   device=self.device)
            out = torch.empty(2 * len(ts), dtype=torch.float64, device=self.device)
            arr = (ctypes.c_double * len(ts))(*ts)
            check(self.lib.pml_ls_eval_multi(self.prec, self.n_rows, len(ts), arr, loss.loss_id,
                                             self.z_cache.data_ptr(), self.zd.data_ptr(), self.y.data_ptr(),
                                             self.wt.data_ptr(), self._ls_multi_stats.data_ptr(), out.data_ptr(),
                                             stream_handle(self.device)), "ls_eval_multi")
            v = out.tolist()
        return [(v[2 * k], v[2 * k + 1]) for k in range(len(ts))]

    def ls_finish_packed(self, loss, t: float, w_eff, shift, need_s: bool = True, start_reduce=None,
                         nb: int = 0) -> torch.Tensor:
        with trace_range("K1 gradient at the accepted step (transpose pass)"):
            out = torch.zeros(self.dim + 2, dtype=torch.float64, device=self.device)
            if self._ls_t0 is not None and float(t) == self._ls_t0 and not getattr(self, "_coef_stale", False) \
                    and not (self.track_hessian and loss.twice_differentiable):
                out[self.dim] = self._ls_t0_dev[0]
                if need_s:
                    torch.sum(self.coef[: self.n_rows], dim=0, dtype=torch.float64, out=out[self.dim + 1])
            else:
                self._ls(loss, t, 1, out[self.dim:])
            self._tpend = float(t)
            self._ls_t0 = None
            self._track_u = False
            self._z_key, self._z_chain = (VecKey(w_eff), float(shift)), self._z_chain + 1
            if self.track_hessian and loss.twice_differentiable:
                self._dzz_key, self._dzz_shift = VecKey(w_eff), float(shift)
            if start_reduce is not None:
                start_reduce(out[self.dim:])
                self._packed_bucketed(self.coef, out[: self.dim], start_reduce, nb)
            else:
                G = self._grad_target(out)
                self.t_all(self.coef, G)
                self._grad_finish(G, out)
            self.n_passes += 1
            return out

    def ls_finish_fused(self, loss, t: float, x0: torch.Tensor, d: torch.Tensor, l2: float):
        from .native import ls_step_grad
        with trace_range("K1 gradient at the accepted step (transpose pass)"):
            first = (self._ls_t0 is not None and float(t) == self._ls_t0 and not getattr(self, "_coef_stale", False)
                     and not (self.track_hessian and loss.twice_differentiable))
            if first:
                F = self._ls_t0_dev[0]
            else:
                tail = torch.empty(2, dtype=torch.float64, device=self.device)
                self._ls(loss, t, 1, tail)
                F = tail[0]
            g = getattr(self, "_gscr", None)
            if g is None or g.numel() != self.dim:
                g = self._gscr = torch.empty(self.dim, dtype=torch.float64, device=self.device)
            G = g.zero_()
            self.t_all(self.coef, G)
            x, grad = ls_step_grad(x0, d, t, G, self.new_of_old if self.old_of_new is not None else None, l2)
            self._tpend = float(t)
            self._ls_t0 = None
            self._track_u = False
            self._z_key, self._z_chain = (VecKey(x), 0.0), self._z_chain + 1
            if self.track_hessian and loss.twice_differentiable:
                self._dzz_key, self._dzz_shift = VecKey(x), 0.0
            self.n_passes += 1
            return x, F, grad

    def ls_finish_device(self, loss, t: float, w_eff, shift, need_s: bool = True):
        out = self.ls_finish_packed(loss, t, w_eff, shift, need_s)
        return out[self.dim], out[self.dim + 1], out[: self.dim]

    def ls_finish_sums(self, loss, t: float, w_eff, shift, need_s: bool = True):
        out = self.ls_finish_packed(loss, t, w_eff, shift, need_s)
        f, s_ = out[self.dim:].tolist()
        return f, s_, out[: self.dim]

    def step_begin(self, w_eff, shift) -> bool:
        if getattr(self, "z_cache", None) is None:
            self.enable_margin_cache()
        n = max(self.n_rows, 1)
        if not self._z_valid_for(w_eff, shift):
            base = getattr(self, "_step_base", None)
            if (base is not None and base[0] is not None and base[0][1] == float(shift)
                    and base[1] < self.LS_REFRESH and base[0][0].matches(w_eff)):
                self._z_key, self._z_chain = base
            else:
                self.fwd_all(self._vec(w_eff), FWD_MARGIN, 0, shift, None, None, z_out=self.z_cache, with_offset=1,
                             stats=False)
                self._z_key, self._z_chain = (VecKey(w_eff), float(shift)), 0
            self._tpend = 0.0
        if self._tpend:
            self.z_cache.add_(self.zd, alpha=self._tpend)
            self._tpend = 0.0
        self.zd.zero_()
        self._ls_t0 = None
        if getattr(self, "u_dir", None) is None:
            self.u_dir = torch.zeros(n, dtype=torch.float64, device=self.device)
        self._track_u = True
        self._step_base = (self._z_key, self._z_chain)
        return True

    def step_add(self, alpha: float):
        self.zd.add_(self.u_dir, alpha=float(alpha))

    def _u_out(self):
        return self.u_dir if getattr(self, "_track_u", False) else None

    def set_weights(self, weights):
        self.wt.copy_(torch.as_tensor(weights, device=self.device).to(self.vdt))
        self.mark_weights_changed()

    def _rows(self, t: torch.Tensor, c: int) -> int:
        return t.data_ptr() + self.row_starts[c] * t.element_size()

    def _fwd(self, c: int, x: torch.Tensor, mode: int, loss_id: int, shift: float, coef: Optional[torch.Tensor],
             dzz: Optional[torch.Tensor], z_out: Optional[torch.Tensor] = None, with_offset: int = 0,
             stats: bool = True):
        ch = self.csr[c]
        st = self.stats.data_ptr() + 2 * 8 * self.blk_off[c] if stats else None
        xp = x.data_ptr() + self.col_lo[c] * x.element_size()
        if ch.kind == "tl":
            masked = getattr(self, "_masked", None)
            desc = masked[0][c] if masked is not None and isinstance(masked[0], list) else ch.desc
            check(self.lib.pml_tl_fwd(
                self.prec, ctypes.byref(desc), xp, mode, loss_id, float(shift),
                self._rows(self.y, c), self._rows(self.o, c), self._rows(self.wt, c),
                None if coef is None else self._rows(coef, c), None if dzz is None else self._rows(dzz, c),
                None if z_out is None else self._rows(z_out, c), with_offset, st, stream_handle(self.device)),
                "tl_fwd")
            return
        lst = self.long_stats.data_ptr() + 2 * 8 * self.long_off[c] if stats else None
        check(self.lib.pml_seg_fwd(
            self.prec, ctypes.byref(ch.desc), xp, mode, loss_id, float(shift),
            self._rows(self.y, c), self._rows(self.o, c), self._rows(self.wt, c),
            None if coef is None else self._rows(coef, c), None if dzz is None else self._rows(dzz, c),
            None if z_out is None else self._rows(z_out, c), with_offset, st, lst, self.parts.data_ptr(),
            stream_handle(self.device)), "seg_fwd")

    def _t(self, c: int, x: torch.Tensor, G: torch.Tensor, square: int = 0):
        ch = self.csc[c]
        gp = G.data_ptr() + self.col_lo[c] * G.element_size()
        if ch.kind == "tl":
            masked = getattr(self, "_masked", None)
            desc = ch.desc if masked is None else masked[1][c]
            check(self.lib.pml_tl_t(self.prec, ctypes.byref(desc), self._rows(x, c), square, gp,
                                    self.parts.data_ptr(), stream_handle(self.device)), "tl_t")
            return
        check(self.lib.pml_seg_t(self.prec, ctypes.byref(ch.desc), self._rows(x, c), square, gp,
                                 self.parts.data_ptr(), stream_handle(self.device)), "seg_t")

    def _build_multi(self):
        self._multi = None
        if not self.csr or any(ch.kind != "tl" for ch in self.csr) or len({ch.rbits for ch in self.csr}) != 1:
            return
        tabs = []
        for c, ch in enumerate(self.csr):
            b = ch.blk.to(torch.int64)
            t = torch.empty((b.shape[0], 8), dtype=torch.int64, device=b.device)
            t[:, 0] = c
            t[:, 1] = b[:, 0] + self.row_starts[c]
            t[:, 2:5] = b[:, 1:4]
            t[:, 5] = self.col_lo[c]
            t[:, 6:8] = b[:, 4:6]
            tabs.append(t)
        self._multi_blk = torch.cat(tabs).to(torch.int32).contiguous()
        from .tiled import stream_ptr_table
        self._multi_ptrs = stream_ptr_table(self.csr, self.device)
        from .native import TLFwdMultiDesc
        if len({ch.il for ch in self.csr}) != 1:
            return
        self._multi = TLFwdMultiDesc(self._multi_blk.data_ptr(), self._multi_blk.shape[0], self.csr[0].rbits,
                                     self._multi_ptrs.data_ptr(), self.csr[0].il)

    def _build_multi_t(self):
        self._multi_t = None
        if not self.csc or any(ch.kind != "tl" for ch in self.csc) or len({ch.cbits for ch in self.csc}) != 1:
            return
        C = 1 << self.csc[0].cbits
        if any(lo % C for lo in self.col_lo):
            return
        from .tiled import TLTMulti
        self._multi_t = TLTMulti(self.csc, self.row_starts, self.dim,
                                 tile_offsets=[lo // C for lo in self.col_lo] if any(self.col_lo) else None)
        need = self._multi_t.parts_needed
        if need > self.parts.numel():
            self.parts = torch.zeros(need, dtype=torch.float64, device=self.device)

    def fwd_all(self, x, mode, loss_id, shift, coef, dzz, z_out=None, with_offset=0, stats=True):
        from .native import KERNEL_CONFIG
        self.n_fwd = getattr(self, "n_fwd", 0) + 1
        if getattr(self, "_multi", "unset") == "unset":
            self._build_multi()
        if self._multi is not None and KERNEL_CONFIG.get("tl_multi", 1):
            p = lambda t: None if t is None else t.data_ptr()
            masked = getattr(self, "_masked", None)
            desc = self._multi if masked is None or isinstance(masked[0], list) else masked[0]
            check(self.lib.pml_tl_fwd_multi(
                self.prec, ctypes.byref(desc), x.data_ptr(), mode, loss_id, float(shift), self.y.data_ptr(),
                self.o.data_ptr(), self.wt.data_ptr(), p(coef), p(dzz), p(z_out), with_offset,
                self.stats.data_ptr() if stats else None, stream_handle(self.device)), "tl_fwd_multi")
            return
        for c in range(len(self.csr)):
            self._fwd(c, x, mode, loss_id, shift, coef, dzz, z_out, with_offset, stats)

    def t_all(self, x, G, square: int = 0, build_multi: bool = True):
        from .native import KERNEL_CONFIG
        self.n_t = getattr(self, "n_t", 0) + 1
        if getattr(self, "_multi_t", "unset") == "unset":
            if not build_multi:
                for c in range(len(self.csc)):
                    self._t(c, x, G, square)
                return
            self._build_multi_t()
        if (self._multi_t is not None and KERNEL_CONFIG.get("tl_multi", 1)
                and getattr(self, "_masked", None) is None):
            check(self.lib.pml_tl_t_multi(self.prec, ctypes.byref(self._multi_t.desc), x.data_ptr(), square,
                                          G.data_ptr(), self.parts.data_ptr(), stream_handle(self.device)),
                  "tl_t_multi")
            return
        for c in range(len(self.csc)):
            self._t(c, x, G, square)

    def entity_mask_geometry(self, row_entity: torch.Tensor, col_entity: torch.Tensor):
        cached = getattr(self, "_mgeo", None)
        if cached is not None:
            return cached
        self._mgeo = False
        if getattr(self, "_multi", "unset") == "unset":
            self._build_multi()
        if (self.old_of_new is not None or not self.csc or any(ch.kind != "tl" for ch in self.csc + self.csr)
                or not self.n_rows):
            return False
        nr, nc = row_entity.numel(), col_entity.numel()
        rspan = lambda lo, cnt: (row_entity[lo.clamp(0, nr - 1)], row_entity[(lo + cnt - 1).clamp(0, nr - 1)])
        if self._multi is not None:
            blk = self._multi_blk.to(torch.int64)
            f0, f1 = rspan(blk[:, 1], blk[:, 2])
            f_off = [0, int(blk.shape[0])]
        else:
            parts = [rspan(ch.blk[: ch.nblk, 0].to(torch.int64) + self.row_starts[c], ch.blk[: ch.nblk, 1].to(torch.int64))
                     for c, ch in enumerate(self.csr)]
            f0 = torch.cat([p[0] for p in parts])
            f1 = torch.cat([p[1] for p in parts])
            f_off = np.cumsum([0] + [int(ch.nblk) for ch in self.csr]).tolist()
        firsts, lasts, i_off, m_off = [], [], [0], [0]
        for c, ch in enumerate(self.csc):
            C = 1 << ch.cbits
            hi = self.col_lo[c] + ch.dim - 1
            for t in (ch.items[: ch.nitems, 0].to(torch.int64), ch.mt_tiles[: ch.nmt].to(torch.int64)):
                firsts.append(col_entity[(self.col_lo[c] + t * C).clamp(0, nc - 1)])
                lasts.append(col_entity[torch.clamp(self.col_lo[c] + (t + 1) * C - 1, max=hi).clamp(0, nc - 1)])
            i_off.append(i_off[-1] + int(ch.nitems) + int(ch.nmt))
            m_off.append(i_off[-2] + int(ch.nitems))
        t0, t1 = torch.cat(firsts), torch.cat(lasts)
        self._mgeo = (f0, f1, f_off, t0, t1, i_off, m_off)
        return self._mgeo

    def set_entity_mask(self, active: Optional[torch.Tensor], geometry=None):
        self._masked = None
        if active is None or not geometry:
            return
        f0, f1, f_off, t0, t1, i_off, m_off = geometry
        dup = lambda d: type(d).from_buffer_copy(d)
        cs = torch.zeros(active.numel() + 1, dtype=torch.int32, device=active.device)
        torch.cumsum(active.to(torch.int32), 0, out=cs[1:])
        live_f = ((cs[f1 + 1] - cs[f0]) > 0).to(torch.uint8)
        live_t = ((cs[t1 + 1] - cs[t0]) > 0).to(torch.uint8)
        keep = [live_f, live_t]
        if self._multi is not None:
            fdesc = dup(self._multi)
            fdesc.live = live_f.data_ptr()
        else:
            fdesc = []
            for c, ch in enumerate(self.csr):
                d = dup(ch.desc)
                d.live = live_f.data_ptr() + f_off[c]
                fdesc.append(d)
        tdescs = []
        for c, ch in enumerate(self.csc):
            d = dup(ch.desc)
            d.live = live_t.data_ptr() + i_off[c]
            d.live_mt = live_t.data_ptr() + m_off[c + 1]
            tdescs.append(d)
        self._masked = (fdesc, tdescs, keep)
        if MASK_STATS is not None:
            MASK_STATS.append((float(live_f.float().mean()), float(live_t.float().mean())))

    def grad_buckets(self, nb: int):
        cache = getattr(self, "_gbuckets", None)
        if cache is not None and cache[0] == nb:
            return cache[1]
        if getattr(self, "_multi_t", "unset") == "unset":
            self._build_multi_t()
        if self._multi_t is None or nb < 2:
            self._gbuckets = (nb, None)
            return None
        from .tiled import TLTMulti
        C = 1 << self._multi_t.cbits
        ntiles = (self.dim + C - 1) // C
        work = np.zeros(ntiles, np.int64)
        for ch in self.csc:
            it = ch.items[: ch.nitems].cpu().numpy().astype(np.int64)
            np.add.at(work, it[:, 0], it[:, 2] - it[:, 1])
        cum = np.cumsum(work)
        cuts = [0] + [int(np.searchsorted(cum, cum[-1] * k / nb, side="right")) for k in range(1, nb)] + [ntiles]
        cuts = sorted(set(min(max(c, 0), ntiles) for c in cuts))
        out = []
        for t0, t1 in zip(cuts[:-1], cuts[1:]):
            if t1 > t0:
                mt = TLTMulti(self.csc, self.row_starts, self.dim, tile_range=(t0, t1))
                out.append((mt, t0 * C, min(t1 * C, self.dim)))
                if mt.parts_needed > self.parts.numel():
                    self.parts = torch.zeros(mt.parts_needed, dtype=torch.float64, device=self.device)
        self._gbuckets = (nb, out)
        return out

    def _packed_bucketed(self, x, G, start_reduce, nb: int, square: int = 0):
        self.n_t = getattr(self, "n_t", 0) + 1
        for mt, c0, c1 in self.grad_buckets(nb):
            check(self.lib.pml_tl_t_multi(self.prec, ctypes.byref(mt.desc), x.data_ptr(), square, G.data_ptr(),
                                          self.parts.data_ptr(), stream_handle(self.device)), "tl_t_multi")
            start_reduce(G[c0:c1])

    def value_grad_packed_overlap(self, loss, w_eff, margin_shift, start_reduce, nb: int = 4) -> torch.Tensor:
        with trace_range("K1 value+grad pass (bucketed)"):
# ... 259 lines not shown
```

### photon_ml_amd/ops/native.py

```python
from __future__ import annotations

import ctypes
import os
from pathlib import Path
from typing import Optional

import numpy as np
import torch

from .build import StaleLibraryError, expected_id, lib_path, verified_path

c_int = ctypes.c_int
c_double = ctypes.c_double
c_void_p = ctypes.c_void_p
P_int = ctypes.POINTER(ctypes.c_int)


class SegChunkDesc(ctypes.Structure):
    _fields_ = [
        ("blk", c_void_p), ("nblk", c_int),
        ("seg_ptr", c_void_p), ("nseg", c_int),
        ("idx", c_void_p), ("val", c_void_p),
        ("long_seg", c_void_p), ("long_ptr", c_void_p), ("nlong", c_int), ("npart", c_int),
    ]


class TLNarrow(ctypes.Structure):
    _fields_ = [("pack", c_void_p), ("val", c_void_p), ("base", c_void_p), ("wbase", c_void_p)]


class TLFwdDesc(ctypes.Structure):
    _fields_ = [("blk", c_void_p), ("nblk", c_int), ("rbits", c_int), ("pack", c_void_p), ("val", c_void_p),
                ("il", c_int), ("nar", TLNarrow), ("live", c_void_p)]


class TLFwdMultiDesc(ctypes.Structure):
    _fields_ = [("blk", c_void_p), ("nblk", c_int), ("rbits", c_int), ("ptrs", c_void_p), ("il", c_int),
                ("live", c_void_p)]


class TLTMultiDesc(ctypes.Structure):
    _fields_ = [("items", c_void_p), ("nitems", c_int), ("cbits", c_int), ("ptrs", c_void_p),
                ("mt_tiles", c_void_p), ("mt_ptr", c_void_p), ("nmt", c_int), ("dim", c_int), ("cu", c_void_p),
                ("ncu", c_int), ("nparts_total", c_int), ("il", c_int), ("live", c_void_p), ("live_mt", c_void_p)]


class CmpArgs(ctypes.Structure):
    _fields_ = [("units", c_void_p), ("col_e", c_int), ("row_col", c_int), ("seg", c_void_p), ("nseg", c_int),
                ("sbits", c_int), ("key_is_row", c_int), ("pack", c_void_p), ("val", c_void_p),
                ("npack", c_void_p), ("nval", c_void_p), ("nbase", c_void_p), ("keep", c_void_p),
                ("seg_cnt", c_void_p), ("seg_first", c_void_p), ("unit_lo", c_void_p), ("opack", c_void_p),
                ("oval", c_void_p)]


class SegRankArgs(ctypes.Structure):
    _fields_ = [("seg_ptr", c_void_p), ("perm", c_void_p), ("scores", c_void_p), ("wts", c_void_p),
                ("flag", c_void_p), ("list", c_void_p), ("lptr", c_void_p), ("out", c_void_p),
                ("nan_flag", c_void_p), ("n_list", ctypes.c_longlong), ("n_rows", ctypes.c_longlong),
                ("n_groups", ctypes.c_longlong), ("k", c_int)]


class AucCountArgs(ctypes.Structure):
    _fields_ = [("scores", c_void_p), ("flag", c_void_p), ("summ", c_void_p), ("out", c_void_p),
                ("n", ctypes.c_longlong), ("n_blocks", ctypes.c_longlong)]


class TLTDesc(ctypes.Structure):
    _fields_ = [
        ("items", c_void_p), ("nitems", c_int), ("cbits", c_int), ("pack", c_void_p), ("val", c_void_p),
        ("mt_tiles", c_void_p), ("mt_ptr", c_void_p), ("nmt", c_int), ("dim", c_int),
        ("cu", c_void_p), ("ncu", c_int), ("nparts_total", c_int), ("il", c_int), ("nar", TLNarrow),
        ("live", c_void_p), ("live_mt", c_void_p),
    ]


_LIBS = {}


def _load(name: str, auto_build: bool = True) -> Optional[ctypes.CDLL]:
    if name in _LIBS:
        return _LIBS[name]
    override = {"glm": "PML_GLM_LIB", "re": "PML_RE_LIB"}.get(name)
    if override and os.environ.get(override):
        path = Path(os.environ[override])
        want = None
    else:
        try:
            path = verified_path("hip", name, auto_build=auto_build)
        except FileNotFoundError:
            _LIBS[name] = None
            return None
        want = expected_id("hip", name)
    lib = ctypes.CDLL(str(path), mode=ctypes.RTLD_GLOBAL)
    if want is not None:
        lib.pml_build_id.restype = ctypes.c_char_p
        got = lib.pml_build_id().decode()
        if got != want:
            raise StaleLibraryError(f"{path}: loaded build id {got} != {want} of the tree's sources")
    _LIBS[name] = lib
    return lib


def glm_lib() -> Optional[ctypes.CDLL]:
    lib = _load("glm")
    if lib is not None and not getattr(lib, "_pml_typed", False):
        lib.pml_build_blocks.argtypes = [c_void_p, c_int, c_int, c_int, c_void_p, P_int, c_void_p, c_void_p,
                                         P_int, P_int]
        lib.pml_seg_fwd.argtypes = [c_int, ctypes.POINTER(SegChunkDesc), c_void_p, c_int, c_int, c_double,
                                    c_void_p, c_void_p, c_void_p, c_void_p, c_void_p, c_void_p, c_int, c_void_p,
                                    c_void_p, c_void_p, c_void_p]
        lib.pml_seg_t.argtypes = [c_int, ctypes.POINTER(SegChunkDesc), c_void_p, c_int, c_void_p, c_void_p,
                                  c_void_p]
        lib.pml_reduce_stats.argtypes = [c_void_p, c_int, c_void_p, c_int, c_void_p, c_void_p]
        lib.pml_lds_add_order_probe.argtypes = [c_void_p, c_void_p, c_int, c_void_p]
        lib.pml_lds_add_order_probe.restype = c_int
        lib.pml_tl_fwd.argtypes = [c_int, ctypes.POINTER(TLFwdDesc), c_void_p, c_int, c_int, c_double, c_void_p,
                                   c_void_p, c_void_p, c_void_p, c_void_p, c_void_p, c_int, c_void_p, c_void_p]
        lib.pml_tl_t.argtypes = [c_int, ctypes.POINTER(TLTDesc), c_void_p, c_int, c_void_p, c_void_p, c_void_p]
        lib.pml_tl_colstats.argtypes = [c_int, ctypes.POINTER(TLTDesc)] + [c_void_p] * 8
        lib.pml_tl_config.argtypes = [c_int, c_int, c_int, c_int]
        lib.pml_tl_t_multi.argtypes = [c_int, ctypes.POINTER(TLTMultiDesc), c_void_p, c_int, c_void_p, c_void_p,
                                       c_void_p]
        lib.pml_tl_fwd_multi.argtypes = [c_int, ctypes.POINTER(TLFwdMultiDesc), c_void_p, c_int, c_int, c_double,
                                         c_void_p, c_void_p, c_void_p, c_void_p, c_void_p, c_void_p, c_int, c_void_p,
                                         c_void_p]
        lib.pml_segdot.argtypes = [c_void_p, c_void_p, c_int, c_void_p, c_int, c_void_p, c_void_p]
        lib.pml_segdot_long.argtypes = [c_void_p, c_void_p, c_int, c_void_p, c_int, ctypes.c_longlong, c_void_p,
                                        c_void_p, c_void_p]
        lib.pml_seg_expand.argtypes = [c_void_p, c_int, c_void_p, c_void_p, c_int, c_void_p]
        lib.pml_seg_cg_step.argtypes = [c_void_p, c_int] + [c_void_p] * 7 + [c_double, c_void_p]
        lib.pml_bgemv.argtypes = [c_int, c_int, c_void_p, c_void_p, c_void_p, c_int, c_void_p]
        lib.pml_btrsv.argtypes = [c_int, c_int, c_void_p, c_void_p, c_void_p, c_int, c_void_p]
        lib.pml_bhv.argtypes = [c_int, c_int, c_void_p, c_void_p, c_void_p, c_double, c_void_p, c_void_p]
        lib.pml_set_ls_args.argtypes = [c_void_p, c_double, c_double]
        lib.pml_set_ls_in.argtypes = [c_void_p, c_void_p]
        lib.pml_set_gate.argtypes = [c_void_p]
        lib.pml_ls_gate.argtypes = [c_void_p, c_void_p, c_double, c_double, c_double, c_double, c_void_p, c_void_p,
                                    c_void_p]
        lib.pml_ls_gate.restype = c_int
        lib.pml_gram_grid.argtypes = [ctypes.c_longlong]
        lib.pml_gram.argtypes = [c_void_p, c_int, ctypes.c_longlong, c_void_p, c_void_p]
        lib.pml_lincomb.argtypes = [c_void_p, c_void_p, c_int, ctypes.c_longlong, c_void_p, c_void_p]
        lib.pml_lbfgs_pair.argtypes = [c_void_p] * 4 + [ctypes.c_longlong] + [c_void_p] * 6
        lib.pml_ls_dots.argtypes = [c_void_p] * 3 + [ctypes.c_longlong] + [c_void_p] * 4
        lib.pml_perm_cast.argtypes = [c_void_p, c_void_p, ctypes.c_longlong, c_int, c_void_p, c_void_p]
        lib.pml_perm_cast.restype = c_int
        lib.pml_ls_step_grad.argtypes = [c_void_p, c_void_p, c_double, c_void_p, c_void_p, c_double,
                                         ctypes.c_longlong, c_void_p, c_void_p, c_void_p]
        lib.pml_ls_step_grad.restype = c_int
        lib.pml_masked_gather.argtypes = [c_void_p, c_void_p, ctypes.c_longlong, c_void_p, c_void_p]
        lib.pml_masked_gather.restype = c_int
        lib.pml_offset_update.argtypes = [c_void_p, c_void_p, ctypes.c_longlong, c_int, c_void_p, c_void_p, c_void_p]
        lib.pml_cached_margins.argtypes = [c_void_p, c_void_p, c_double, c_int, c_void_p, ctypes.c_longlong,
                                           c_void_p, c_void_p]
        lib.pml_cached_margins.restype = c_int
        lib.pml_offset_update.restype = c_int
        lib.pml_two_loop_chain.argtypes = [c_int] + [c_void_p] * 5 + [ctypes.c_longlong] + [c_void_p] * 4 + \
            [c_int, c_void_p]
        lib.pml_two_loop_gram.argtypes = [c_int, c_void_p, c_void_p, c_void_p, ctypes.c_longlong, c_void_p, c_void_p,
                                          c_void_p, c_int, c_void_p]
        lib.pml_two_loop_gram_grid.argtypes = [ctypes.c_longlong]
        lib.pml_tl_set_deep.argtypes = [c_int, c_int]
        lib.pml_rs_set_variant.argtypes = [c_int]
        lib.pml_rs_set_variant(int(os.environ.get("PML_RS_VARIANT", "5")))
        lib.pml_ls_eval.argtypes = [c_int, c_int, c_double, c_int, c_void_p, c_void_p, c_void_p, c_void_p, c_int,
                                    c_void_p, c_void_p, c_void_p, c_void_p, c_void_p]
        lib.pml_ls_eval_multi.argtypes = [c_int, c_int, c_int, ctypes.POINTER(c_double), c_int, c_void_p, c_void_p,
                                          c_void_p, c_void_p, c_void_p, c_void_p, c_void_p]
        lib.pml_ls_eval_multi.restype = c_int
        lib.pml_rs_tron.argtypes = [c_int, c_int] + [c_void_p] * 8 + [c_int, c_double, c_double, c_int, c_int, c_int,
                                                                      c_void_p, c_void_p, c_void_p]
        for f in ("pml_seg_fwd", "pml_seg_t", "pml_reduce_stats", "pml_build_blocks", "pml_tl_fwd", "pml_tl_t",
                  "pml_tl_colstats",
                  "pml_tl_maxbits", "pml_segdot", "pml_segdot_long", "pml_tl_fwd_multi", "pml_tl_t_multi", "pml_seg_cg_step",
                  "pml_seg_expand", "pml_bgemv", "pml_btrsv", "pml_bhv", "pml_rs_tron", "pml_ls_eval", "pml_gram_grid", "pml_gram",
                  "pml_lincomb", "pml_lbfgs_pair", "pml_ls_dots", "pml_two_loop_chain", "pml_two_loop_gram",
                  "pml_two_loop_gram_grid"):
            getattr(lib, f).restype = c_int
        lib.pml_set_config.argtypes = [c_int, c_int, c_int, c_int]
        lib._pml_typed = True
        configure()
    return lib


KERNEL_CONFIG = {"fwd_strided": 0, "t_strided": 0, "hot_n": 0, "fwd_grid": 1024, "tl_acc64": 1, "tl_waves": 2,
                 "tl_waves_t": 4, "tl_pipe": 0, "tl_pipe_t": 0, "tl_multi": 1, "tl_deep": 0, "tl_deep_t": 0}


def configure(**kw):
    KERNEL_CONFIG.update({k: v for k, v in kw.items() if v is not None})
    for k in list(KERNEL_CONFIG):
        env = os.environ.get("PML_" + k.upper())
        if env is not None and k not in kw:
            KERNEL_CONFIG[k] = int(env)
    lib = _LIBS.get("glm")
    if lib is not None:
        lib.pml_set_config(KERNEL_CONFIG["fwd_strided"], KERNEL_CONFIG["t_strided"], KERNEL_CONFIG["hot_n"],
                           KERNEL_CONFIG["fwd_grid"])
        lib.pml_tl_config(KERNEL_CONFIG["tl_acc64"], KERNEL_CONFIG["tl_waves"], KERNEL_CONFIG["tl_waves_t"],
                          (KERNEL_CONFIG["tl_pipe"] & 3) | ((KERNEL_CONFIG["tl_pipe_t"] & 3) << 2))
        lib.pml_tl_set_deep(KERNEL_CONFIG["tl_deep"], KERNEL_CONFIG["tl_deep_t"])
    return dict(KERNEL_CONFIG)


def tl_experiment_build() -> bool:
# ... 1274 lines not shown
```

### photon_ml_amd/ops/tiled.py

```python
from __future__ import annotations

import ctypes
import math
import os
from typing import Optional, Sequence, Tuple

import numpy as np
import torch

from .native import TLFwdDesc, TLTDesc

TL_MAXBITS = 12
TL_MAXBITS_F64 = 11
TL_MINBITS = 5
DEFAULT_RBITS = int(os.environ.get("PML_TL_RBITS", 10))
DEFAULT_CBITS = int(os.environ.get("PML_TL_CBITS", 10))
DEFAULT_ITEM_ENTRIES = 1 << 18
_PAD = 8
COMBINE_SEG = 16


XCD_GROUPS = int(os.environ.get("PML_TL_XCD", "0"))


def xcd_order(chunk_of_item: np.ndarray, groups: int) -> np.ndarray:
    stream = np.asarray(chunk_of_item) % groups
    lists = [np.flatnonzero(stream == k) for k in range(groups)]
    longest = max(len(l) for l in lists)
    grid = np.full((longest, groups), -1, dtype=np.int64)
    for k, l in enumerate(lists):
        grid[: len(l), k] = l
    order = grid.reshape(-1)
    return order[order >= 0]


def combine_seg(k: int) -> int:
    return max(COMBINE_SEG, int(math.ceil(math.sqrt(k))))
IL_ROUND = 256
TL_VEC = 4
INTERLEAVE = int(os.environ.get("PML_TL_IL", "1"))
NARROW = int(os.environ.get("PML_TL_NARROW", "1"))
NARROW_W = 64
FUSE = int(os.environ.get("PML_TL_FUSE", "1"))
WIDE_BASE = int(os.environ.get("PML_TL_WIDE_BASE", "1"))


def narrow_width(sbits: int) -> int:
    return min(NARROW_W, 1 << max(16 - sbits, 0))


def _bits(n: int) -> int:
    return max(1, int(n - 1).bit_length())


def _cap(want: int, f64: bool) -> int:
    return min(want, TL_MAXBITS_F64 if f64 else TL_MAXBITS)


F64_WIDE_RBITS = 11


def default_rbits(dim: int, f64: bool) -> int:
    if f64 and dim >= (1 << 16) and "PML_TL_RBITS" not in os.environ:
        return F64_WIDE_RBITS
    return DEFAULT_RBITS


def fwd_bits(dim: int, f64: bool = False, want: Optional[int] = None) -> Optional[int]:
    r = min(_cap(default_rbits(dim, f64) if want is None else want, f64), 32 - _bits(dim))
    return r if r >= TL_MINBITS else None


def t_bits(chunk_rows: int, f64: bool = False, want: Optional[int] = None) -> Optional[int]:
    c = min(_cap(DEFAULT_CBITS if want is None else want, f64), 32 - _bits(chunk_rows))
    return c if c >= TL_MINBITS else None


SPARSE_TILE_ENTRIES = 1 << 16


def shard_t_config(nnz: int, n_rows: int, dim: int, chunk_rows: int):
    if "PML_TL_CBITS" in os.environ or "PML_TL_ITEM_ENTRIES" in os.environ or n_rows <= 0 or dim < (1 << 16):
        return None, None
    per_tile = (nnz / n_rows) * min(chunk_rows, n_rows) / math.ceil(dim / 1024)
    if per_tile < SPARSE_TILE_ENTRIES:
        return 11, 1 << 17
    return None, None


def tl_supported(dim: int, chunk_rows: int) -> bool:
    return fwd_bits(dim) is not None and t_bits(chunk_rows) is not None


def _to_u32_bits(x64: torch.Tensor) -> torch.Tensor:
    return torch.where(x64 >= (1 << 31), x64 - (1 << 32), x64).to(torch.int32)


def _pad(t: torch.Tensor) -> torch.Tensor:
    return torch.cat([t, torch.zeros(_PAD, dtype=t.dtype, device=t.device)]).contiguous()


def il_phys(e_lo: torch.Tensor, n: torch.Tensor) -> torch.Tensor:
    e_lo = e_lo.to(torch.int64)
    n = n.to(torch.int64)
    tot = int(n.sum())
    unit = torch.repeat_interleave(torch.arange(n.numel(), device=n.device), n)
    j = torch.arange(tot, device=n.device) - (torch.cumsum(n, 0) - n)[unit]
    t = j & (IL_ROUND - 1)
    return e_lo[unit] + (j - t) + ((t & 63) << 2) + (t >> 6)


def _interleave(pack: torch.Tensor, val: torch.Tensor, n: torch.Tensor):
    n = n.to(torch.int64)
    padded = (n + IL_ROUND - 1) // IL_ROUND * IL_ROUND
    new_lo = torch.cumsum(padded, 0) - padded
    total = int(padded.sum()) + _PAD
    phys = il_phys(new_lo, n)
    p = torch.zeros(total, dtype=pack.dtype, device=pack.device)
    v = torch.zeros(total, dtype=val.dtype, device=val.device)
    p[phys] = pack
    v[phys] = val
    return p, v, new_lo


def _empty_narrow(val: torch.Tensor):
    dev = val.device
    return (torch.zeros(IL_ROUND, dtype=torch.int16, device=dev), torch.zeros(IL_ROUND, dtype=val.dtype, device=dev),
            torch.zeros(1, dtype=torch.int32, device=dev))


def split_narrow(pack: torch.Tensor, val: torch.Tensor, n: torch.Tensor, sbits: int, xlen: int, enable: bool = True):
    dev = pack.device
    n = n.to(torch.int64)
    U = n.numel()
    gcount = n // IL_ROUND
    W = narrow_width(sbits)
    ok = enable and NARROW and W >= 16 and xlen >= NARROW_W and int(gcount.sum()) > 0
    if not ok:
        z = torch.zeros(U, dtype=torch.int64, device=dev)
        return (pack, val, n, *_empty_narrow(val), z)
    starts = torch.cumsum(n, 0) - n
    gu = torch.repeat_interleave(torch.arange(U, device=dev), gcount)
    gi = torch.arange(gu.numel(), device=dev) - (torch.cumsum(gcount, 0) - gcount)[gu]
    gs = starts[gu] + IL_ROUND * gi
    key = pack >> sbits
    first, last = key[gs], key[gs + IL_ROUND - 1]
    base = torch.clamp(first, max=xlen - NARROW_W)
    nar = (last - base) < W
    gs_n, base = gs[nar], base[nar]
    idx = gs_n[:, None] + torch.arange(IL_ROUND, device=dev)[None, :]
    p16 = ((key[idx] - base[:, None]) << sbits) | (pack[idx] & ((1 << sbits) - 1))
    il = lambda t: t.reshape(-1, TL_VEC, 64).transpose(1, 2).reshape(-1)
    npack = il(torch.where(p16 >= 32768, p16 - 65536, p16).to(torch.int16)).contiguous()
    nval = il(val[idx]).contiguous()
    if FUSE and val.dtype == torch.bfloat16:
        npack = torch.cat([npack.view(-1, TL_VEC), nval.view(torch.int16).view(-1, TL_VEC)], 1).reshape(-1)
        nval = None
    nbase = base.to(torch.int32).contiguous()
    cs = torch.zeros(nar.numel() + 1, dtype=torch.int64, device=dev)
    torch.cumsum(nar.to(torch.int64), 0, out=cs[1:])
    ge = torch.cumsum(gcount, 0)
    nrounds = cs[ge] - cs[ge - gcount]
    keep = torch.ones(pack.numel(), dtype=torch.bool, device=dev)
    keep[idx.reshape(-1)] = False
    del idx, p16
    return pack[keep], val[keep], n - IL_ROUND * nrounds, npack, nval, nbase, nrounds



def narrow_logical(npack: torch.Tensor, nval: torch.Tensor, nbase: torch.Tensor, r_lo, r_hi, sbits: int):
    r = torch.arange(int(r_lo), int(r_hi), device=npack.device)
    if not r.numel():
        return torch.zeros(0, dtype=torch.int64, device=npack.device), nval[:0].reshape(-1)
    ph = (r[:, None] * IL_ROUND + torch.arange(IL_ROUND, device=npack.device)[None, :]).reshape(-1, 64, TL_VEC)
    ph = ph.transpose(1, 2).reshape(-1)
    rl, rh = int(r_lo) * IL_ROUND, int(r_hi) * IL_ROUND
    ph = ph - rl
    p16 = npack.reshape(-1, TL_VEC)[rl // TL_VEC:rh // TL_VEC].reshape(-1)[ph].to(torch.int64) & 0xFFFF
    base = nbase[r].to(torch.int64).repeat_interleave(IL_ROUND)
    return ((((p16 >> sbits) + base) << sbits) | (p16 & ((1 << sbits) - 1)),
            nval.reshape(-1, TL_VEC)[rl // TL_VEC:rh // TL_VEC].reshape(-1)[ph])


class _NarrowMixin:

    wbase = None

    nrec = None

    def _set_narrow(self, npack, nval, nbase):
        from .native import TLNarrow
        self.nrec = npack if nval is None else None
        if nval is None:
            rec = npack.view(-1, 2 * TL_VEC)
            npack, nval = rec[:, :TL_VEC], rec[:, TL_VEC:].view(torch.bfloat16)
        self.npack, self.nval, self.nbase = npack, nval, nbase
        self.nar = TLNarrow(npack.data_ptr(), None if self.fused else nval.data_ptr(), nbase.data_ptr(),
                            None if self.wbase is None else self.wbase.data_ptr())

    @property
    def fused(self) -> bool:
        return self.nrec is not None

    @property
    def n_narrow_rounds(self) -> int:
        t = self._table()
        return int((t[:, 5] - t[:, 4]).sum()) if t.shape[0] else 0

    def unit_counts(self) -> torch.Tensor:
        t = self._table().to(torch.int64)
        lo, hi = self._ew
        return (t[:, hi] - t[:, lo]) + IL_ROUND * (t[:, 5] - t[:, 4])

    def narrow_window(self, r_lo: int, r_hi: int):
        return narrow_logical(self.npack, self.nval, self.nbase, r_lo, r_hi, self._sbits)

    def _logical_all(self, wide_pack, wide_val):
        t = self._table().to(torch.int64)
        dev = wide_pack.device
        lo, hi = self._ew
        nn = IL_ROUND * (t[:, 5] - t[:, 4])
        nw = t[:, hi] - t[:, lo]
        if int(nn.sum()) == 0:
            return wide_pack, wide_val
        npk, nvl = narrow_logical(self.npack, self.nval, self.nbase, 0, int(t[:, 5].max()), self._sbits)
        U = t.shape[0]
        nu = torch.repeat_interleave(torch.arange(U, device=dev), nn.to(dev))
        nj = torch.arange(int(nn.sum()), device=dev) - (torch.cumsum(nn, 0) - nn).to(dev)[nu]
        npos = t[:, 4].to(dev)[nu] * IL_ROUND + nj
        wu = torch.repeat_interleave(torch.arange(U, device=dev), nw.to(dev))
        unit = torch.cat([nu, wu])
        order = torch.sort(unit, stable=True).indices
        wp = wide_pack.to(torch.int64) & 0xFFFFFFFF if wide_pack.dtype == torch.int32 else wide_pack.to(torch.int64)
        pk = torch.cat([npk[npos], wp])[order]
        vl = torch.cat([nvl[npos], wide_val])[order]
        return pk, vl


class TLFwdChunk(_NarrowMixin):

    kind = "tl"

    def __init__(self, rowptr: torch.Tensor, col: torch.Tensor, val: torch.Tensor, dim: int,
                 rbits: Optional[int] = None, il: Optional[int] = None):
        dev = val.device
        self.il = INTERLEAVE if il is None else int(il)
        rowptr = rowptr.to(dev, torch.int64)
        col = col.to(dev, torch.int64)
        m = rowptr.numel() - 1
        f64 = val.dtype == torch.float64
        self.rbits = fwd_bits(dim, f64, rbits)
        if self.rbits is None:
            raise ValueError(f"tiled forward layout cannot pack dim={dim}")
        want = _cap(default_rbits(dim, f64) if rbits is None else rbits, f64)
        use_base = bool(self.il) and WIDE_BASE and want > self.rbits
        if use_base:
            self.rbits = want
        R = 1 << self.rbits
        kbits = _bits(dim) + self.rbits
        nnz = col.numel()
        rows = torch.repeat_interleave(torch.arange(m, device=dev), rowptr[1:] - rowptr[:-1]) if nnz else \
            torch.zeros(0, dtype=torch.int64, device=dev)
        pack = (col << self.rbits) | (rows & (R - 1))
        key = ((rows >> self.rbits) << kbits) | pack
        key, perm = torch.sort(key, stable=True)
        nblk = (m + R - 1) // R
        b = torch.arange(nblk, device=dev)
        lo = b * R
        hi = torch.clamp(lo + R, max=m)
        e_lo, e_hi = rowptr[lo], rowptr[hi]
        self._sbits, self._ew = self.rbits, (2, 3)
        n_lo = n_hi = torch.zeros(nblk, dtype=torch.int64, device=dev)
        if self.il:
            wp, wv, wn, npk, nvl, nbs, nr = split_narrow(key & ((1 << kbits) - 1), val[perm], e_hi - e_lo,
                                                         self.rbits, dim)
            del key, perm
            if use_base:
                wp = self._rebase(wp, wn)
                if wp is None:
                    del wv, npk, nvl, nbs
                    self.__init__(rowptr, col, val, dim, fwd_bits(dim, f64, rbits), il)
                    return
            self.pack, self.val, e_lo = _interleave(_to_u32_bits(wp), wv, wn)
            e_hi = e_lo + wn
            n_hi = torch.cumsum(nr, 0)
            n_lo = n_hi - nr
            del wp, wv
        else:
            self.pack = _pad(_to_u32_bits(key & ((1 << kbits) - 1)))
            self.val = _pad(val[perm].contiguous())
            npk, nvl, nbs = _empty_narrow(val)
            del key, perm
        del rows
        self._set_narrow(npk, nvl, nbs)
        self.blk = torch.stack([lo, hi - lo, e_lo, e_hi, n_lo, n_hi], 1).to(torch.int32).contiguous()
        self.nblk, self.m, self.nnz = nblk, m, nnz
        self.desc = TLFwdDesc(self.blk.data_ptr(), nblk, self.rbits, self.pack.data_ptr(), self.val.data_ptr(),
                              self.il, self.nar)

    def _rebase(self, wp: torch.Tensor, wn: torch.Tensor) -> Optional[torch.Tensor]:
        dev = wp.device
        n = wn.to(torch.int64)
        tot = int(n.sum())
        padded = (n + IL_ROUND - 1) // IL_ROUND * IL_ROUND
        nrounds = int(padded.sum()) // IL_ROUND
        wbase = torch.zeros(nrounds + 1, dtype=torch.int64, device=dev)
        if tot:
            unit = torch.repeat_interleave(torch.arange(n.numel(), device=dev), n, output_size=tot)
            j = torch.arange(tot, device=dev) - (torch.cumsum(n, 0) - n)[unit]
            rid = ((torch.cumsum(padded, 0) - padded)[unit] + j) // IL_ROUND
            del unit
            key = wp >> self.rbits
            first = (j % IL_ROUND) == 0
            del j
            wbase[rid[first]] = key[first]
            rel = key - wbase[rid]
            del rid, key, first
            if int(rel.max()) >= 1 << (32 - self.rbits):
                return None
            wp = (rel << self.rbits) | (wp & ((1 << self.rbits) - 1))
        self.wbase = wbase.to(torch.int32).contiguous()
        return wp

    @property
    def nstats(self) -> int:
        return self.nblk

    parts_needed = 0

    def _table(self):
        return self.blk

    def nbytes(self) -> int:
        return sum(t.numel() * t.element_size() for t in (self.blk, self.pack, self.val, self.npack, self.nval,
                                                           self.nbase) + (() if self.wbase is None else (self.wbase,)))

    def logical(self):
        if not self.il:
            return self.pack[: self.nnz].to(torch.int64) & 0xFFFFFFFF, self.val[: self.nnz]
        ph = il_phys(self.blk[:, 2], self.blk[:, 3] - self.blk[:, 2])
        wp = self.pack[ph].to(torch.int64) & 0xFFFFFFFF
        if self.wbase is not None:
            wp = ((self.wbase[ph // IL_ROUND].to(torch.int64) + (wp >> self.rbits)) << self.rbits) | (
                wp & ((1 << self.rbits) - 1))
        return self._logical_all(wp, self.val[ph])

    def emulate_matvec(self, x: torch.Tensor) -> torch.Tensor:
        pk, vl = self.logical()
        p = pk.to(torch.int64)
        col = p >> self.rbits
        blk_of_entry = torch.repeat_interleave(torch.arange(self.nblk, device=p.device), self.unit_counts())
        row = (blk_of_entry << self.rbits) + (p & ((1 << self.rbits) - 1))
        z = torch.zeros(self.m, dtype=torch.float64, device=p.device)
        return z.index_add_(0, row, vl.to(torch.float64) * x.to(torch.float64)[col])


class TLTChunk(_NarrowMixin):

    kind = "tl"

    def __init__(self, rowptr: torch.Tensor, col: torch.Tensor, val: torch.Tensor, dim: int, chunk_rows: int,
                 cbits: Optional[int] = None, item_entries: Optional[int] = None, il: Optional[int] = None):
        self.il = INTERLEAVE if il is None else int(il)
        if item_entries is None:
            item_entries = int(os.environ.get("PML_TL_ITEM_ENTRIES", DEFAULT_ITEM_ENTRIES))
        dev = val.device
        rowptr = rowptr.to(dev, torch.int64)
        col = col.to(dev, torch.int64)
        m = rowptr.numel() - 1
        self.cbits = t_bits(max(chunk_rows, m), val.dtype == torch.float64, cbits)
        if self.cbits is None:
            raise ValueError(f"tiled transpose layout cannot pack chunk_rows={chunk_rows}")
        C = 1 << self.cbits
        nnz = col.numel()
        rows = torch.repeat_interleave(torch.arange(m, device=dev), rowptr[1:] - rowptr[:-1]) if nnz else \
            torch.zeros(0, dtype=torch.int64, device=dev)
        tile = col >> self.cbits
        pack = (rows << self.cbits) | (col & (C - 1))
        key = (tile << 32) | pack
        del rows, pack
        key, perm = torch.sort(key, stable=True)
        del tile
        ntiles = (dim + C - 1) // C
        tptr = torch.searchsorted(key >> 32, torch.arange(ntiles + 1, device=dev)).cpu().numpy().astype(np.int64)
        counts = np.diff(tptr)
        pack = _to_u32_bits(key & 0xFFFFFFFF)
        val = val[perm]
        del key, perm
        nz = np.nonzero(counts)[0]
        n_it = np.maximum(1, -(-counts[nz] // item_entries))
        it_tile = np.repeat(nz, n_it)
        it_i = np.arange(len(it_tile)) - np.repeat(np.cumsum(n_it) - n_it, n_it)
        it_k = np.repeat(n_it, n_it)
        a, b = tptr[it_tile], tptr[it_tile + 1]
        lo, hi = a + (b - a) * it_i // it_k, a + (b - a) * (it_i + 1) // it_k
        split = it_k > 1
        part_of = np.full(len(it_tile), -1, np.int64)
        part_of[split] = np.arange(int(split.sum()))
        km = n_it[n_it > 1]
        plo = np.cumsum(km) - km
        sg = np.maximum(COMBINE_SEG, np.ceil(np.sqrt(km)).astype(np.int64)) if len(km) else km
        nu = -(-km // sg)
        u_mt = np.repeat(np.arange(len(km)), nu)
        u_first = np.repeat(plo, nu) + np.repeat(sg, nu) * (np.arange(int(nu.sum())) - np.repeat(np.cumsum(nu) - nu, nu))
        u_last = np.minimum(u_first + np.repeat(sg, nu), np.repeat(plo + km, nu))
        cu = np.column_stack([u_mt, u_first, u_last]) if len(km) else np.zeros((0, 3), np.int64)
        mt_tiles = nz[n_it > 1].tolist()
        mt_ptr = np.r_[0, np.cumsum(nu)].tolist() if len(km) else [0]
        self.nitems, self.nmt, self.nparts, self.ncu = len(it_tile), len(mt_tiles), int(km.sum()), len(cu)
        items = np.column_stack([it_tile, lo, hi, part_of]).astype(np.int64).reshape(-1, 4)
        items = np.column_stack([items, np.zeros((len(items), 2), np.int64)])
        self._sbits, self._ew = self.cbits, (1, 2)
        if self.il:
            cnt = torch.from_numpy(items[:, 2] - items[:, 1]).to(dev)
            wp, wv, wn, npk, nvl, nbs, nr = split_narrow(pack.to(torch.int64) & 0xFFFFFFFF, val, cnt, self.cbits, m)
            del pack, val
            self.pack, self.val, new_lo = _interleave(_to_u32_bits(wp), wv, wn)
            del wp, wv
            items[:, 1] = new_lo.cpu().numpy()
            items[:, 2] = items[:, 1] + wn.cpu().numpy()
            nr = nr.cpu().numpy()
            items[:, 5] = np.cumsum(nr)
            items[:, 4] = items[:, 5] - nr
        else:
            self.pack, self.val = _pad(pack), _pad(val.contiguous())
            npk, nvl, nbs = _empty_narrow(val)
            del pack, val
        self._set_narrow(npk, nvl, nbs)
        self.items = torch.tensor(items.astype(np.int32), device=dev)
        self.mt_tiles = torch.tensor(np.asarray(mt_tiles or [0], dtype=np.int32), device=dev)
        self.mt_ptr = torch.tensor(np.asarray(mt_ptr, dtype=np.int32), device=dev)
        self.cu = torch.tensor(np.asarray(cu if len(cu) else [(0, 0, 0)], dtype=np.int32).reshape(-1, 3), device=dev)
        self.m, self.nnz, self.dim = m, nnz, dim
        self.desc = TLTDesc(self.items.data_ptr(), self.nitems, self.cbits, self.pack.data_ptr(),
                            self.val.data_ptr(), self.mt_tiles.data_ptr(), self.mt_ptr.data_ptr(), self.nmt, dim,
                            self.cu.data_ptr(), self.ncu, self.nparts, self.il, self.nar)

    @property
    def parts_needed(self) -> int:
        return (self.nparts + self.ncu) << self.cbits

    def _table(self):
        return self.items

    def nbytes(self) -> int:
        return sum(t.numel() * t.element_size() for t in (self.items, self.mt_tiles, self.mt_ptr, self.cu, self.pack,
                                                           self.val, self.npack, self.nval, self.nbase))

    def window(self, e_lo: int, e_hi: int):
        if not self.il:
            return self.pack[e_lo:e_hi], self.val[e_lo:e_hi]
        ph = il_phys(torch.tensor([e_lo]), torch.tensor([e_hi - e_lo])).to(self.pack.device)
        return self.pack[ph], self.val[ph]

    def logical(self):
        if not self.il:
            return self.pack[: self.nnz], self.val[: self.nnz]
        ph = il_phys(self.items[:, 1], self.items[:, 2] - self.items[:, 1])
        return self._logical_all(self.pack[ph], self.val[ph])

    def emulate_rmatvec(self, r: torch.Tensor, square: bool = False) -> torch.Tensor:
        pk, vl = self.logical()
        p = pk.to(torch.int64) & 0xFFFFFFFF
        row = p >> self.cbits
        tile_of_entry = torch.repeat_interleave(self.items[:, 0].to(torch.int64), self.unit_counts())
        col = (tile_of_entry << self.cbits) + (p & ((1 << self.cbits) - 1))
        v = vl.to(torch.float64)
        if square:
            v = v * v
        g = torch.zeros(self.dim, dtype=torch.float64, device=p.device)
        return g.index_add_(0, col, v * r.to(torch.float64)[row])


class TLTMulti:

    def __init__(self, chunks: Sequence["TLTChunk"], row_starts: Sequence[int], dim: int,
                 tile_range: Optional[Tuple[int, int]] = None, tile_offsets: Optional[Sequence[int]] = None):
        from .native import TLTMultiDesc
        dev = chunks[0].pack.device
        self.cbits = chunks[0].cbits
        self.il = chunks[0].il
        if any(ch.il != self.il for ch in chunks):
            raise ValueError("TLTMulti: chunks mix interleaved and plain streams")
        its = []
        for c, ch in enumerate(chunks):
            it = ch.items[: ch.nitems].cpu().numpy().astype(np.int64).reshape(-1, 6)
            toff = 0 if tile_offsets is None else int(tile_offsets[c])
            its.append(np.column_stack([np.full(len(it), c), it[:, 0] + toff, it[:, 1], it[:, 2],
                                        np.full(len(it), row_starts[c]), it[:, 4], it[:, 5]]))
        it = np.concatenate(its) if its else np.zeros((0, 7), np.int64)
        src_all = np.arange(len(it))
        if tile_range is not None:
            in_range = (it[:, 1] >= tile_range[0]) & (it[:, 1] < tile_range[1])
            it = it[in_range]
        n = len(it)
        tile = it[:, 1]
        order = np.lexsort((np.arange(n), tile))
        ts = tile[order]
        starts = np.flatnonzero(np.r_[True, ts[1:] != ts[:-1]]) if n else np.zeros(0, np.int64)
        k = np.diff(np.r_[starts, n])
        multi_tile = np.repeat(k > 1, k)
        part = np.full(n, -1, np.int64)
        part[order[multi_tile]] = np.arange(int(multi_tile.sum()))
        km = k[k > 1]
        plo = np.cumsum(km) - km
        sg = np.maximum(COMBINE_SEG, np.ceil(np.sqrt(km)).astype(np.int64)) if len(km) else km
        nu = -(-km // sg)
        u_tile = np.repeat(np.arange(len(km)), nu)
        u_first = np.repeat(plo, nu) + np.repeat(sg, nu) * (np.arange(int(nu.sum())) - np.repeat(np.cumsum(nu) - nu, nu))
        u_last = np.minimum(u_first + np.repeat(sg, nu), np.repeat(plo + km, nu))
        self.nitems, self.nparts, self.ncu, self.nmt = n, int(km.sum()), int(nu.sum()), len(km)
        rows = np.column_stack([it[:, 0], it[:, 1], it[:, 2], it[:, 3], part, it[:, 4], it[:, 5],
                                it[:, 6]]).astype(np.int32)
        src = src_all if tile_range is None else src_all[in_range]
        if XCD_GROUPS > 1 and n > XCD_GROUPS:
            xo = xcd_order(it[:, 0], XCD_GROUPS)
            rows, src = rows[xo], src[xo]
        self._src = torch.from_numpy(src.astype(np.int64)).to(dev)
        self.items = torch.tensor(rows.reshape(-1, 8), device=dev)
        self.mt_tiles = torch.tensor(np.r_[ts[starts][k > 1], 0].astype(np.int32)[: max(self.nmt, 1)], device=dev)
        self.mt_ptr = torch.tensor(np.r_[0, np.cumsum(nu)].astype(np.int32), device=dev)
        self.cu = torch.tensor(np.column_stack([u_tile, u_first, u_last]).astype(np.int32).reshape(-1, 3)
                               if self.ncu else np.zeros((1, 3), np.int32), device=dev)
        self.ptrs = stream_ptr_table(chunks, dev)
        self._chunks = list(chunks)
        self.desc = TLTMultiDesc(self.items.data_ptr(), n, self.cbits, self.ptrs.data_ptr(),
                                 self.mt_tiles.data_ptr(), self.mt_ptr.data_ptr(), self.nmt, dim,
                                 self.cu.data_ptr(), self.ncu, self.nparts, self.il)

    @property
    def parts_needed(self) -> int:
        return (self.nparts + self.ncu) << self.cbits

    def restreamed(self, chunks: Sequence["TLTChunk"]) -> "TLTMulti":
        import copy
        from .native import TLTMultiDesc
        dev = self.items.device
        cat = torch.cat([ch.items[: ch.nitems].to(torch.int64) for ch in chunks]) if chunks else None
        rows = self.items.to(torch.int64).clone()
        if self.nitems:
            sel = cat[self._src]
            rows[:, 2:4] = sel[:, 1:3]
            rows[:, 6:8] = sel[:, 4:6]
        new = copy.copy(self)
        new.items = rows.to(torch.int32).contiguous()
        new.ptrs = stream_ptr_table(chunks, dev)
        new._chunks = list(chunks)
        d = self.desc
        new.desc = TLTMultiDesc(new.items.data_ptr(), d.nitems, d.cbits, new.ptrs.data_ptr(), d.mt_tiles, d.mt_ptr,
                                d.nmt, d.dim, d.cu, d.ncu, d.nparts_total, d.il)
        return new

    def emulate_rmatvec(self, r: torch.Tensor, square: bool = False) -> torch.Tensor:
        C = 1 << self.cbits
        dim = self.desc.dim
        ntiles = (dim + C - 1) // C
        G = torch.zeros(ntiles * C, dtype=torch.float64)
        parts = torch.zeros((max(self.nparts, 1), C), dtype=torch.float64)
        r = r.to(torch.float64).cpu()
        for c, tile, e_lo, e_hi, part, rb, n_lo, n_hi in self.items.cpu().tolist():
            ch = self._chunks[c]
            pk, vl = ch.window(e_lo, e_hi)
            npk, nvl = ch.narrow_window(n_lo, n_hi)
            p = torch.cat([npk.cpu(), pk.to(torch.int64).cpu() & 0xFFFFFFFF])
            v = torch.cat([nvl.cpu(), vl.cpu()]).to(torch.float64)
            if square:
                v = v * v
            acc = torch.zeros(C, dtype=torch.float64).index_add_(0, p & (C - 1), v * r[rb + (p >> self.cbits)])
            if part < 0:
                G[tile * C:(tile + 1) * C] += acc
            else:
                parts[part] = acc
        cu = self.cu.cpu().tolist()
        l1 = [parts[a:b].sum(0) for _, a, b in cu[: self.ncu]]
        mp = self.mt_ptr.cpu().tolist()
        for t, tile in enumerate(self.mt_tiles.cpu().tolist()[: self.nmt]):
            s = torch.zeros(C, dtype=torch.float64)
            for u in range(mp[t], mp[t + 1]):
                s += l1[u]
            G[tile * C:(tile + 1) * C] += s
        return G[:dim]


def stream_ptr_table(chunks, device) -> torch.Tensor:
    wb = lambda ch: 0 if getattr(ch, "wbase", None) is None else ch.wbase.data_ptr()
    return torch.tensor([[ch.pack.data_ptr(), ch.val.data_ptr(), ch.npack.data_ptr(),
                          0 if ch.fused else ch.nval.data_ptr(), ch.nbase.data_ptr(), wb(ch)] for ch in chunks],
                        dtype=torch.int64, device=device).reshape(-1)


CMP_SEG = 8


def _cmp_segments(ch, narrow: bool):
    cache = ch.__dict__.setdefault("_cmp_seg", {})
    if cache.get(narrow) is not None:
        return cache[narrow]
    t = ch._table().to(torch.int64)
    dev = t.device
    lo, hi = ch._ew
    nn = t[:, 5] - t[:, 4]
    R = (t[:, hi] - t[:, lo] + IL_ROUND - 1) // IL_ROUND + (nn if narrow else 0)
    ns = (R + CMP_SEG - 1) // CMP_SEG
    S = int(ns.sum())
    su = torch.repeat_interleave(torch.arange(t.shape[0], device=dev), ns, output_size=S)
    first = (torch.cumsum(ns, 0) - ns)[su]
    r_lo = (torch.arange(S, device=dev) - first) * CMP_SEG
    r_hi = torch.minimum(r_lo + CMP_SEG, R[su])
    if not narrow:
        r_lo, r_hi = r_lo + nn[su], r_hi + nn[su]
    seg = torch.stack([su, r_lo, r_hi], 1).to(torch.int32).contiguous()
    cache[narrow] = (seg, su, first, S, IL_ROUND * int(nn.sum()))
    return cache[narrow]


class RowCompaction:

    def __init__(self, ch, keep: torch.Tensor, forward: bool, filter_narrow: bool = False):
        from .native import CmpArgs, check, require_game_lib, stream_handle
        if not ch.il:
            raise ValueError("row-sampled copies need the interleaved layout")
        self.ch, self.keep, self.forward = ch, keep, forward
        dev = ch.pack.device
        self.filter_narrow = bool(filter_narrow)
        seg, su, first, S, self.n_narrow = _cmp_segments(ch, self.filter_narrow)
        table = ch._table()
        lo, hi = ch._ew
        self.seg_cnt = torch.zeros(max(S, 1), dtype=torch.int32, device=dev)
        self._keep_alive = (seg, table, keep)
        self.args = CmpArgs(table.data_ptr(), lo, 0 if forward else -1, seg.data_ptr(), S, ch._sbits,
                            0 if forward else 1, ch.pack.data_ptr(), ch.val.data_ptr(), ch.npack.data_ptr(),
                            None if ch.fused else ch.nval.data_ptr(), ch.nbase.data_ptr(), keep.data_ptr(),
                            self.seg_cnt.data_ptr(),
                            None, None, None, None)
        self.lib, self.stream = require_game_lib(), stream_handle(dev)
        self.vbytes = ch.val.element_size()
        if S:
            check(self.lib.pml_tl_compact(0, self.vbytes, ctypes.byref(self.args), self.stream), "tl_compact count")
        cnt = self.seg_cnt[:S].to(torch.int64)
        U = table.shape[0]
        self.unit_cnt = torch.zeros(U, dtype=torch.int64, device=dev).index_add_(0, su, cnt)
        padded = (self.unit_cnt + IL_ROUND - 1) // IL_ROUND * IL_ROUND
        self.unit_lo = (torch.cumsum(padded, 0) - padded).contiguous()
        excl = torch.cumsum(cnt, 0) - cnt
        self.seg_first = (excl - excl[first]).contiguous() if S else excl
        self.total, self.kept = padded.sum(), self.unit_cnt.sum()

    def finish(self, total: int, kept: int):
        import copy
        from .native import TLFwdDesc, TLTDesc, check
        ch = self.ch
        dev = ch.pack.device
        opack = torch.zeros(total + _PAD, dtype=torch.int32, device=dev)
        oval = torch.zeros(total + _PAD, dtype=ch.val.dtype, device=dev)
        a = self.args
        a.seg_first, a.unit_lo = self.seg_first.data_ptr(), self.unit_lo.data_ptr()
        a.opack, a.oval = opack.data_ptr(), oval.data_ptr()
        if a.nseg:
            check(self.lib.pml_tl_compact(1, self.vbytes, ctypes.byref(a), self.stream), "tl_compact write")
        lo, hi = ch._ew
        table = ch._table().to(torch.int64).clone()
        table[:, lo] = self.unit_lo
        table[:, hi] = self.unit_lo + self.unit_cnt
        if self.filter_narrow:
            table[:, 4:6] = 0
        table = table.to(torch.int32).contiguous()
        nc = copy.copy(ch)
        nc._cmp_seg = {}
        nc.pack, nc.val = opack, oval
        if self.filter_narrow:
            nc._set_narrow(*_empty_narrow(oval))
            nc.nnz = kept
        else:
            nc.nnz = kept + self.n_narrow
        if self.forward:
            nc.blk = table
            nc.desc = TLFwdDesc(table.data_ptr(), nc.nblk, nc.rbits, opack.data_ptr(), oval.data_ptr(), 1, nc.nar)
        else:
            nc.items = table
            nc.desc = TLTDesc(table.data_ptr(), nc.nitems, nc.cbits, opack.data_ptr(), oval.data_ptr(),
                              nc.mt_tiles.data_ptr(), nc.mt_ptr.data_ptr(), nc.nmt, nc.dim, nc.cu.data_ptr(), nc.ncu,
                              nc.nparts, 1, nc.nar)
        return nc
```

### photon_ml_amd/ops/warmup.py

```python
from __future__ import annotations

import time

import torch

_DONE = set()


def runtime_warmup(device, force: bool = False) -> float:
    dev = torch.device(device)
    if dev.type != "cuda":
        return 0.0
    key = dev.index if dev.index is not None else torch.cuda.current_device()
    if key in _DONE and not force:
        return 0.0
    torch.cuda.synchronize(dev)
    t0 = time.perf_counter()
    from .native import (auc_counts, batched_gemv, batched_trsv, check_lds_add_order, csr_gather_rows,
                         key_histogram)
    x = torch.linspace(0.0, 1.0, 4096, dtype=torch.float64, device=dev)
    i = torch.arange(4096, dtype=torch.int64, device=dev)
    torch.linalg.vector_norm(x)
    torch.dot(x, x)
    (x * x).sum()
    torch.where(x > 0.5, x, torch.zeros_like(x)).square().sum()
    torch.isfinite(x).all()
    torch.cumsum(i, 0)
    torch.sort(i.flip(0), stable=True)
    torch.argsort(x.flip(0), stable=True)
    torch.searchsorted(i, i)
    torch.unique(i % 7, sorted=True, return_inverse=True)
    torch.repeat_interleave(i[:8], i[:8] % 3)
    torch.nonzero(i % 5 == 0)
    x[i.flip(0)]
    torch.zeros_like(x).index_copy_(0, i, x)
    torch.zeros(8, dtype=torch.int64, device=dev).scatter_reduce_(0, i % 8, i, reduce="amax")
    torch.segment_reduce(x, "sum", lengths=torch.full((64,), 64, dtype=torch.int64, device=dev))
    x.to(torch.float32).to(torch.bfloat16)
    check_lds_add_order(dev)
    key_histogram(i % 13, 13)
    csr_gather_rows(torch.tensor([0, 2], dtype=torch.int64, device=dev), i[:2], x[:2],
                    torch.zeros(1, dtype=torch.int64, device=dev), torch.tensor([0, 4], dtype=torch.int64, device=dev))
    auc_counts(x.flip(0).contiguous(), (i % 2).to(torch.uint8))
    L = torch.eye(65, dtype=torch.float64, device=dev).unsqueeze(0).contiguous()
    batched_trsv(L, torch.ones(1, 65, dtype=torch.float64, device=dev))
    batched_gemv(L[:, :8, :8].contiguous(), torch.ones(1, 8, dtype=torch.float64, device=dev))
    from .native import re_lbfgs_csr, re_lbfgs_grid
    p01 = torch.tensor([0, 1], dtype=torch.int64, device=dev)
    one = torch.ones(1, dtype=torch.float64, device=dev)
    i32 = lambda: torch.zeros(1, dtype=torch.int32, device=dev)
    re_lbfgs_csr(i32(), p01, p01, p01, torch.zeros(1, dtype=torch.int16, device=dev), one, one, torch.zeros_like(one),
                 one, torch.empty(4, dtype=torch.float64, device=dev), torch.zeros_like(one), torch.empty_like(one),
                 i32(), i32(), torch.empty_like(one), 0, 0.0, 0.1, 1e-3, 2, 256,
                 torch.empty(2 * 10 * 256, dtype=torch.float64, device=dev), i32(), min(re_lbfgs_grid(256), 1))
    torch.cuda.Stream(dev, priority=-1)
    torch.cuda.Stream(dev, priority=0)
    torch.cuda.synchronize(dev)
    _DONE.add(key)
    return time.perf_counter() - t0
```

### photon_ml_amd/stat/summary.py

```python
from __future__ import annotations

import logging
from dataclasses import dataclass

import numpy as np
import scipy.sparse as sp
import torch

log = logging.getLogger(__name__)


@dataclass
class BasicStatisticalSummary:
    mean: torch.Tensor
    variance: torch.Tensor
    count: int
    num_nonzeros: torch.Tensor
    max: torch.Tensor
    min: torch.Tensor
    norm_l1: torch.Tensor
    norm_l2: torch.Tensor
    mean_abs: torch.Tensor

    @staticmethod
    def from_sufficient(count, s1, s2, sabs, nnz, mx, mn) -> "BasicStatisticalSummary":
        n = float(count)
        mean = s1 / n if n > 0 else s1
        var = (s2 - n * mean * mean) / (n - 1) if n > 1 else np.zeros_like(s1)
        mx = np.where(nnz < n, np.maximum(mx, 0.0), mx)
        mn = np.where(nnz < n, np.minimum(mn, 0.0), mn)
        bad = ~np.isfinite(var) | (var < 0)
        if bad.any():
            log.warning("Found %d features where variance was either non-positive, not-a-number, or infinite. "
                        "The variances for these features have been re-set to 1.0.", int(bad.sum()))
            var = np.where(bad, 1.0, var)
        t = lambda a: torch.from_numpy(np.asarray(a, dtype=np.float64))
        return BasicStatisticalSummary(t(mean), t(var), int(count), t(nnz), t(mx), t(mn), t(sabs), t(np.sqrt(s2)),
                                       t(sabs / n if n > 0 else sabs))

    @staticmethod
    def compute(x: sp.csr_matrix, all_reduce: bool = False) -> "BasicStatisticalSummary":
        x = x.tocsc()
        n, d = x.shape
        s1 = np.asarray(x.sum(axis=0)).ravel()
        s2 = np.asarray(x.multiply(x).sum(axis=0)).ravel()
        sabs = np.asarray(abs(x).sum(axis=0)).ravel()
        nnz = np.diff(x.indptr).astype(np.float64)
        mx = np.full(d, -np.inf)
        mn = np.full(d, np.inf)
        if x.nnz:
            col = np.repeat(np.arange(d), np.diff(x.indptr))
            np.maximum.at(mx, col, x.data)
            np.minimum.at(mn, col, x.data)
        mx = np.where(np.isinf(mx), 0.0, mx)
        mn = np.where(np.isinf(mn), 0.0, mn)
        count = n
        if all_reduce:
            from ..parallel.dist import is_dist
            import torch.distributed as dist
            if is_dist():
                buf = torch.from_numpy(np.concatenate([[count], s1, s2, sabs, nnz]).astype(np.float64))
                dist.all_reduce(buf)
                b = buf.numpy()
                count, s1, s2, sabs, nnz = int(b[0]), b[1:1 + d], b[1 + d:1 + 2 * d], b[1 + 2 * d:1 + 3 * d], b[1 + 3 * d:]
                tmx, tmn = torch.from_numpy(mx), torch.from_numpy(mn)
                dist.all_reduce(tmx, op=dist.ReduceOp.MAX)
                dist.all_reduce(tmn, op=dist.ReduceOp.MIN)
                mx, mn = tmx.numpy(), tmn.numpy()
        return BasicStatisticalSummary.from_sufficient(count, s1, s2, sabs, nnz, mx, mn)

    @staticmethod
    def on_device(glm_data) -> bool:
        dev = getattr(glm_data, "device", None)
        return (getattr(glm_data, "layout", None) == "tiled" and dev is not None and dev.type == "cuda"
                and getattr(glm_data, "precision", None) == "f64")

    @staticmethod
    def for_shard(x, glm_data, all_reduce: bool = False) -> "BasicStatisticalSummary":
        if BasicStatisticalSummary.on_device(glm_data):
            return BasicStatisticalSummary.from_device(glm_data, all_reduce=all_reduce)
        if hasattr(x, "to_scipy"):
            x = x.to_scipy()
        return BasicStatisticalSummary.compute(x, all_reduce=all_reduce)

    @staticmethod
    def _torch_column_stats(data):
        dev = data.device
        d = data.dim
        f64 = torch.float64
        s1 = torch.zeros(d, dtype=f64, device=dev)
        s2 = torch.zeros(d, dtype=f64, device=dev)
        sabs = torch.zeros(d, dtype=f64, device=dev)
        nnz = torch.zeros(d, dtype=f64, device=dev)
        mx = torch.full((d,), float("-inf"), dtype=f64, device=dev)
        mn = torch.full((d,), float("inf"), dtype=f64, device=dev)
        for c, ch in enumerate(data.csr):
            pk, vl = ch.logical()
            col = (pk.to(torch.int64) >> ch.rbits) + data.col_lo[c]
            v = vl.to(f64)
            s1.index_add_(0, col, v)
            s2.index_add_(0, col, v * v)
            sabs.index_add_(0, col, v.abs())
            nnz.index_add_(0, col, torch.ones_like(v))
            mx.scatter_reduce_(0, col, v, "amax")
            mn.scatter_reduce_(0, col, v, "amin")
            del pk, vl, col, v
        if data.old_of_new is not None:
            def unperm(t):
                out = torch.empty_like(t)
                out[data.old_of_new] = t
                return out
            s1, s2, sabs, nnz, mx, mn = (unperm(t) for t in (s1, s2, sabs, nnz, mx, mn))
        return s1, s2, sabs, nnz, mx, mn

    @staticmethod
    def from_device(data, all_reduce: bool = False) -> "BasicStatisticalSummary":
        dev = data.device
        d = data.dim
        f64 = torch.float64
        if any(getattr(ch, "kind", None) != "tl" for ch in data.csr):
            raise ValueError("from_device needs the tiled layout")
        if dev.type == "cuda":
            s1, s2, sabs, nnz, mx, mn = data.column_stats()
        else:
            s1, s2, sabs, nnz, mx, mn = BasicStatisticalSummary._torch_column_stats(data)
        count = float(data.n_rows)
        if all_reduce:
            from ..parallel.dist import is_dist
            import torch.distributed as dist
            if is_dist():
                cdev = dev if dist.get_backend() == "nccl" else torch.device("cpu")
                buf = torch.cat([torch.tensor([count], dtype=f64, device=dev), s1, s2, sabs, nnz]).to(cdev)
                dist.all_reduce(buf)
                count = float(buf[0])
                s1, s2, sabs, nnz = (t.to(dev) for t in buf[1:].split(d))
                tmx, tmn = mx.to(cdev), mn.to(cdev)
                dist.all_reduce(tmx, op=dist.ReduceOp.MAX)
                dist.all_reduce(tmn, op=dist.ReduceOp.MIN)
                mx, mn = tmx.to(dev), tmn.to(dev)
        mx = torch.where(torch.isinf(mx), torch.zeros_like(mx), mx)
        mn = torch.where(torch.isinf(mn), torch.zeros_like(mn), mn)
        h = lambda t: t.cpu().numpy()
        return BasicStatisticalSummary.from_sufficient(int(count), h(s1), h(s2), h(sabs), h(nnz), h(mx), h(mn))
```

Baseline: 3.308 billion examples/sec.

## Add tall forward tiles spanning four row sub-blocks per workgroup

Introduces a 'tall' forward layout where each workgroup handles a 4096-row tile made of four 1024-row sub-blocks. Narrow entries are processed per sub-block by separate waves and wide entries are streamed by one wave into a shared 4096-entry LDS accumulator, with per-sub-block stats. The aim is to amortize wide-round streaming and block overhead across more rows. The packing, compaction, validation and logical-view code are updated for the new bit layout. In exchange it adds complexity and uses a single wave for the wide stream.

```diff
diff --git a/photon_ml_amd/data/synthetic.py b/photon_ml_amd/data/synthetic.py
--- a/photon_ml_amd/data/synthetic.py
+++ b/photon_ml_amd/data/synthetic.py
@@ -105,7 +105,7 @@
                           seed: int = 1234567890, chunk_rows: int = 1 << 20, zipf_s: float = 1.1,
                           task=TaskType.LOGISTIC_REGRESSION, rank: int = 0, progress=None, layout: str = "auto"):
     from ..ops.device import DeviceGLMData, SegChunk, VAL_DTYPE, resolve_layout
-    from ..ops.tiled import TLFwdChunk, TLTChunk
+    from ..ops.tiled import TLFwdChunk, TLTChunk, shard_tall
 
     dev = torch.device(device)
     prec = {"bf16": 0, "f32": 1, "f64": 2}[precision]
@@ -163,7 +163,7 @@
             rp = torch.arange(0, (m + 1) * k, k, dtype=torch.int64, device=dev)
             col = idx.to(torch.int64)
             del idx
-            csr.append(TLFwdChunk(rp, col, val, n_features))
+            csr.append(TLFwdChunk(rp, col, val, n_features, tall=shard_tall(n_features, min(chunk_rows, n_rows))))
             csc.append(TLTChunk(rp, col, val, n_features, chunk_rows, cbits=cbits, item_entries=item_entries))
             raw[ci] = None
             del col, val, rp
diff --git a/photon_ml_amd/ops/csrc/game_kernels.hip b/photon_ml_amd/ops/csrc/game_kernels.hip
--- a/photon_ml_amd/ops/csrc/game_kernels.hip
+++ b/photon_ml_amd/ops/csrc/game_kernels.hip
@@ -166,6 +166,8 @@
   const long long* unit_lo;
   uint32_t* opack;
   void* oval;
+  int ustride;
+  int wbits;
 };
 
 template <typename VT, int PASS>
@@ -175,12 +177,13 @@
   if (s >= a.nseg) return;
   const int* sg = a.seg + 3 * (long long)s;
   const int u = sg[0], r_lo = sg[1], r_hi = sg[2];
-  const int* ut = a.units + 6 * (long long)u;
+  const int* ut = a.units + a.ustride * (long long)u;
   const long long e_lo = ut[a.col_e];
   const int nw = ut[a.col_e + 1] - ut[a.col_e];
   const int n_lo = ut[4], nn = ut[5] - ut[4];
   const uint32_t row0 = a.row_col >= 0 ? (uint32_t)ut[a.row_col] : 0u;
-  const uint32_t smask = (1u << a.sbits) - 1u;
+  const uint32_t smask = (1u << a.sbits) - 1u, wmask = (1u << a.wbits) - 1u;
+  const bool tall = a.ustride > 6;
   const VT* val = (const VT*)a.val;
   const VT* nval = (const VT*)a.nval;
   long long ob = PASS ? a.seg_first[s] : 0;
@@ -194,11 +197,12 @@
     if (r < nn) {
       const long long q = (long long)n_lo + r;
       const int base = a.nbase[q];
+      const uint32_t sub = tall ? (uint32_t)((q >= ut[6]) + (q >= ut[7]) + (q >= ut[8])) << a.sbits : 0u;
 #pragma unroll
       for (int k = 0; k < 4; ++k) {
         const long long pe = nval ? q * 256 + 4 * lane + k : q * 512 + 8 * lane + k;
         const uint32_t p16 = a.npack[pe];
-        p[k] = ((uint32_t)(base + (int)(p16 >> a.sbits)) << a.sbits) | (p16 & smask);
+        p[k] = ((uint32_t)(base + (int)(p16 >> a.sbits)) << a.wbits) | sub | (p16 & smask);
         v[k] = nval ? nval[pe] : ((const VT*)a.npack)[pe + 4];
         ok[k] = true;
       }
@@ -214,7 +218,7 @@
     }
 #pragma unroll
     for (int k = 0; k < 4; ++k) {
-      const uint32_t row = a.key_is_row ? (p[k] >> a.sbits) : row0 + (p[k] & smask);
+      const uint32_t row = a.key_is_row ? (p[k] >> a.wbits) : row0 + (p[k] & wmask);
       const bool kp = ok[k] && a.keep[row];
       const unsigned long long m = __ballot(kp);
       if (PASS) {
diff --git a/photon_ml_amd/ops/csrc/glm_kernels.hip b/photon_ml_amd/ops/csrc/glm_kernels.hip
--- a/photon_ml_amd/ops/csrc/glm_kernels.hip
+++ b/photon_ml_amd/ops/csrc/glm_kernels.hip
@@ -781,7 +781,7 @@
   typedef typename TLValT<VT>::T LT;
   typedef typename TLVals<VT>::Raw Raw;
   const int lane = threadIdx.x & 63;
-  const int w = __builtin_amdgcn_readfirstlane(threadIdx.x >> 6);
+  const int w = NW == 1 ? 0 : __builtin_amdgcn_readfirstlane(threadIdx.x >> 6);
   const uint32_t smask = (1u << sbits) - 1u;
   const int nr = (e_hi - e_lo + TL_ROUND - 1) / TL_ROUND;
   const int r0 = (nr * w) / NW, r1 = (nr * (w + 1)) / NW;
@@ -882,7 +882,7 @@
   typedef typename TLValT<VT>::T LT;
   typedef typename TLVals<VT>::Raw Raw;
   const int lane = threadIdx.x & 63;
-  const int w = __builtin_amdgcn_readfirstlane(threadIdx.x >> 6);
+  const int w = NW == 1 ? 0 : __builtin_amdgcn_readfirstlane(threadIdx.x >> 6);
   const int nr = n_hi - n_lo;
   const int r0 = n_lo + (nr * w) / NW, r1 = n_lo + (nr * (w + 1)) / NW;
   if (r0 >= r1) return;
@@ -1020,6 +1020,93 @@
                                               (const VT*)pc[1], nar, x + q[5], a, stats, acc, red);
 }
 
+#define TL_TALL_BITS 12
+#define TL_TALL_SUB 10
+template <typename VT, typename XT, typename RT, int PT>
+__device__ __forceinline__ void tl_fwd_tall_block(int row_lo, int nrows, int e_lo, int e_hi,
+                                                  const int* __restrict__ nq ,
+                                                  const uint32_t* __restrict__ pack, const VT* __restrict__ val,
+                                                  const TLNarrow& nar, const XT* __restrict__ x,
+                                                  const FwdArgs<XT, RT>& a, double* __restrict__ stats, double* acc) {
+  constexpr int NW = 4;
+  for (int i = threadIdx.x; i < (1 << TL_TALL_BITS); i += NW * 64) acc[i] = 0.0;
+  __syncthreads();
+  const int w = __builtin_amdgcn_readfirstlane(threadIdx.x >> 6);
+  const int n_lo = w == 0 ? nq[0] : nq[1 + w], n_hi = w == NW - 1 ? nq[1] : nq[2 + w];
+  if (n_hi > n_lo)
+    tl_narrow<VT, XT, double, false, 1, (PT >= 5 ? 4 : 2)>(nar, n_lo, n_hi, TL_TALL_SUB, x, acc + (w << TL_TALL_SUB));
+  __syncthreads();
+  if (w == 0) {
+    if (PT == 6) tl_stream_ring<VT, XT, double, false, 1, 5, 2>(pack, val, x, e_lo, e_hi, TL_TALL_BITS, acc, nar.wbase);
+    else if (PT == 5) tl_stream_ring<VT, XT, double, false, 1, 3, 1>(pack, val, x, e_lo, e_hi, TL_TALL_BITS, acc, nar.wbase);
+    else tl_stream_ring<VT, XT, double, false, 1, 2, 0>(pack, val, x, e_lo, e_hi, TL_TALL_BITS, acc, nar.wbase);
+  }
+  __syncthreads();
+  const int t = ((w & 1) << 6) | (threadIdx.x & 63);
+  double Fk[2], Sk[2];
+#pragma unroll
+  for (int j = 0; j < 2; ++j) {
+    const int k0 = ((w >> 1) * 2 + j) << TL_TALL_SUB;
+    const int nk = min(nrows - k0, 1 << TL_TALL_SUB);
+    double F = 0.0, S = 0.0;
+    for (int r = k0 + t; r < k0 + nk; r += 128) {
+      const int s = row_lo + r;
+      fwd_finish(a, s, acc[r], fwd_prefetch(a, s), F, S);
+    }
+    Fk[j] = F; Sk[j] = S;
+  }
+  if (stats) {
+    const int sb = nq[5];
+#pragma unroll
+    for (int j = 0; j < 2; ++j) { Fk[j] = wave_sum(Fk[j]); Sk[j] = wave_sum(Sk[j]); }
+    __syncthreads();
+    if ((threadIdx.x & 63) == 0) {
+#pragma unroll
+      for (int j = 0; j < 2; ++j) {
+        const int k = (w >> 1) * 2 + j;
+        acc[4 * k + 2 * (w & 1)] = Fk[j]; acc[4 * k + 2 * (w & 1) + 1] = Sk[j];
+      }
+    }
+    __syncthreads();
+    const int k = threadIdx.x;
+    if (k < 4 && (k << TL_TALL_SUB) < nrows) {
+      double F = 0.0, S = 0.0;
+      for (int i = 0; i < 2; ++i) { F += acc[4 * k + 2 * i]; S += acc[4 * k + 2 * i + 1]; }
+      stats[2 * (sb + k)] = F; stats[2 * (sb + k) + 1] = S;
+    }
+  }
+}
+
+template <typename VT, typename XT, typename RT, int PT>
+__global__ __launch_bounds__(256) void tl_fwd_tall_kernel(const int* __restrict__ blk,
+                                                           const uint32_t* __restrict__ pack,
+                                                           const VT* __restrict__ val, TLNarrow nar,
+                                                           const XT* __restrict__ x, FwdArgs<XT, RT> a,
+                                                           double* __restrict__ stats,
+                                                           const unsigned char* __restrict__ live) {
+  __shared__ double acc[1 << TL_TALL_BITS];
+  const int b = blockIdx.x;
+  if (live && !live[b]) return;
+  const int* q = blk + 10 * b;
+  tl_fwd_tall_block<VT, XT, RT, PT>(q[0], q[1], q[2], q[3], q + 4, pack, val, nar, x, a, stats, acc);
+}
+
+template <typename VT, typename XT, typename RT, int PT>
+__global__ __launch_bounds__(256) void tl_fwd_tall_multi_kernel(const int* __restrict__ blk,
+                                                                 const unsigned long long* __restrict__ ptrs,
+                                                                 const XT* __restrict__ x, FwdArgs<XT, RT> a,
+                                                                 double* __restrict__ stats,
+                                                                 const unsigned char* __restrict__ live) {
+  __shared__ double acc[1 << TL_TALL_BITS];
+  const int b = blockIdx.x;
+  if (live && !live[b]) return;
+  const int* q = blk + 12 * b;
+  const unsigned long long* pc = ptrs + 6 * q[0];
+  const TLNarrow nar = {(const uint16_t*)pc[2], (const void*)pc[3], (const int*)pc[4], (const int*)pc[5]};
+  tl_fwd_tall_block<VT, XT, RT, PT>(q[1], q[2], q[3], q[4], q + 6, (const uint32_t*)pc[0], (const VT*)pc[1], nar,
+                                    x + q[5], a, stats, acc);
+}
+
 template <typename VT, typename XT, typename AT, bool SQ, int MAXR, int U, int NW, int P>
 __device__ __forceinline__ void tl_t_item(int tile, int e_lo, int e_hi, int part, int n_lo, int n_hi, int cbits,
                                           const uint32_t* __restrict__ pack, const VT* __restrict__ val,
@@ -1130,9 +1217,9 @@
 }
 
 struct TLFwdDesc { const int* blk; int nblk; int rbits; const uint32_t* pack; const void* val; int il; TLNarrow nar;
-                  const unsigned char* live; };
+                  const unsigned char* live; int tbits; };
 struct TLFwdMultiDesc { const int* blk; int nblk; int rbits; const unsigned long long* ptrs; int il;
-                       const unsigned char* live; };
+                       const unsigned char* live; int tbits; };
 struct TLTDesc {
   const int* items; int nitems; int cbits; const uint32_t* pack; const void* val;
   const int* mt_tiles; const int* mt_ptr; int nmt; int dim;
@@ -1233,9 +1320,36 @@
   }
 }
 
+#define TL_TALL_P 6
+template <typename XT, typename F>
+static int tl_with_tall(int tbits, int rbits, int il, F f) {
+  if constexpr (sizeof(XT) == 8) {
+    return -22;
+  } else {
+    if (tbits != TL_TALL_BITS || rbits != TL_TALL_SUB || !il) return -22;
+    if constexpr (TL_EXPERIMENT) {
+      if (g_tl_deep == 2) f(std::integral_constant<int, 6>{});
+      else if (g_tl_deep) f(std::integral_constant<int, 5>{});
+      else f(std::integral_constant<int, 3>{});
+    } else {
+      f(std::integral_constant<int, TL_TALL_P>{});
+    }
+    return 0;
+  }
+}
+
 template <typename VT, typename XT, typename RT>
 static int tl_fwd_impl(const TLFwdDesc* c, const void* x, FwdArgs<XT, RT> a, double* stats, hipStream_t st) {
   if (c->nblk <= 0) return 0;
+  if (c->tbits) {
+    const int rt = tl_with_tall<XT>(c->tbits, c->rbits, c->il, [&](auto pt) {
+      hipLaunchKernelGGL((tl_fwd_tall_kernel<VT, XT, RT, decltype(pt)::value>), dim3(c->nblk), dim3(256), 0, st,
+                         c->blk, c->pack, (const VT*)c->val, c->nar, (const XT*)x, a, stats, c->live);
+    });
+    if (rt) return rt;
+    LAUNCH_CHECK();
+    return 0;
+  }
   const int rc = tl_with_acc<XT>(c->rbits, [&](auto acc) {
     tl_with_pipe<2, 1>(c->il, g_tl_waves, g_tl_deep, g_tl_pipe, [&](auto pipe) {
       using A = decltype(acc); using Q = decltype(pipe);
@@ -1253,6 +1367,15 @@
 static int tl_fwd_multi_impl(const TLFwdMultiDesc* c, const void* x, FwdArgs<XT, RT> a, double* stats,
                              hipStream_t st) {
   if (c->nblk <= 0) return 0;
+  if (c->tbits) {
+    const int rt = tl_with_tall<XT>(c->tbits, c->rbits, c->il, [&](auto pt) {
+      hipLaunchKernelGGL((tl_fwd_tall_multi_kernel<VT, XT, RT, decltype(pt)::value>), dim3(c->nblk), dim3(256), 0,
+                         st, c->blk, c->ptrs, (const XT*)x, a, stats, c->live);
+    });
+    if (rt) return rt;
+    LAUNCH_CHECK();
+    return 0;
+  }
   const int rc = tl_with_acc<XT>(c->rbits, [&](auto acc) {
     tl_with_pipe<2, 2>(c->il, g_tl_waves, g_tl_deep, g_tl_pipe, [&](auto pipe) {
       using A = decltype(acc); using Q = decltype(pipe);
diff --git a/photon_ml_amd/ops/device.py b/photon_ml_amd/ops/device.py
--- a/photon_ml_amd/ops/device.py
+++ b/photon_ml_amd/ops/device.py
@@ -13,7 +13,7 @@
 from ..data.matrix import LabeledData
 from .native import SegChunkDesc, check, require_glm_lib, stream_handle
 from .reference import GLMComputable
-from .tiled import DEFAULT_ITEM_ENTRIES, TLFwdChunk, TLTChunk, tl_supported
+from .tiled import DEFAULT_ITEM_ENTRIES, TLFwdChunk, TLTChunk, shard_tall, tl_supported
 from ..utils.timing import phase, trace_range
 
 H2D_GATE = threading.Event()
@@ -184,7 +184,7 @@
             m = self.row_starts[c + 1] - self.row_starts[c]
             b = f.blk.cpu().to(torch.int64)
             if f.nblk and (int(b[:, 0].min()) < 0 or int((b[:, 0] + b[:, 1]).max()) > m
-                           or int(b[:, 1].max()) > (1 << f.rbits)):
+                           or int(b[:, 1].max()) > (1 << f.ubits)):
                 raise ValueError(f"chunk {c}: forward block rows out of range")
             q = 256 if f.il else 4
             end = b[:, 2] + (b[:, 3] - b[:, 2] + q - 1) // q * q if f.il else (b[:, 3] + 3) // 4 * 4
@@ -199,11 +199,11 @@
             wb = getattr(f, "wbase", None)
             if wb is not None and wb.numel() and int(wb.min()) < 0:
                 raise ValueError(f"chunk {c}: negative wide-round base")
-            if p.numel() and int((p >> f.rbits).max()) >= ncols:
+            if p.numel() and int((p >> f.ubits).max()) >= ncols:
                 raise ValueError(f"chunk {c}: forward gather index >= column window")
             counts = f.unit_counts().cpu()
             blk_rows = torch.repeat_interleave(b[:, 1], counts)
-            if p.numel() and bool(((p & ((1 << f.rbits) - 1)) >= blk_rows).any()):
+            if p.numel() and bool(((p & ((1 << f.ubits) - 1)) >= blk_rows).any()):
                 raise ValueError(f"chunk {c}: forward LDS slot >= block rows")
             it = t.items.cpu().to(torch.int64)
             if t.nitems:
@@ -325,7 +325,7 @@
                 rp = torch.from_numpy((xc.indptr - xc.indptr[0]).astype(np.int64)).to(dev)
                 col = torch.from_numpy(xc.indices.astype(np.int64)).to(dev)
                 val = torch.from_numpy(xc.data.astype(np.float64)).to(dev).to(vdt)
-                csr.append(TLFwdChunk(rp, col, val, dc))
+                csr.append(TLFwdChunk(rp, col, val, dc, tall=shard_tall(dmax, min(chunk_rows, n))))
                 csc.append(TLTChunk(rp, col, val, dc, chunk_rows, cbits=cbits, item_entries=item_entries))
                 continue
             sp_ = (xc.indptr - xc.indptr[0]).astype(np.int32)
@@ -384,7 +384,8 @@
     @staticmethod
     def from_device_csr(indptr: torch.Tensor, col: torch.Tensor, val: torch.Tensor, y, offsets, weights, dim: int,
                         device="cuda", precision: str = "f64", chunk_rows: int = 1 << 20,
-                        item_entries: Optional[int] = None, col_windows: bool = False):
+                        item_entries: Optional[int] = None, col_windows: bool = False,
+                        tall: Optional[bool] = None):
         dev = torch.device(device)
         vdt = VAL_DTYPE[PRECISIONS[precision]]
         indptr = indptr.to(dev, torch.int64)
@@ -418,7 +419,8 @@
             rp = indptr[a:b + 1] - ea
             c = col[ea:eb] - lo if lo else col[ea:eb]
             v = val[ea:eb].to(dev).to(vdt)
-            csr.append(TLFwdChunk(rp, c, v, hi - lo))
+            csr.append(TLFwdChunk(rp, c, v, hi - lo,
+                                  tall=shard_tall(dmax, min(chunk_rows, n)) if tall is None else tall))
             csc.append(TLTChunk(rp, c, v, hi - lo, chunk_rows, cbits=cbits, item_entries=item_entries))
             col_lo.append(lo)
             del c, v
@@ -471,11 +473,11 @@
             nb = self._multi_blk.clone()
             cb = torch.cat([ch.blk for ch in view.csr])
             nb[:, 3:5] = cb[:, 2:4]
-            nb[:, 6:8] = cb[:, 4:6]
+            nb[:, 6:6 + min(cb.shape[1], 9) - 4] = cb[:, 4:9]
             view._multi_blk = nb
             view._multi_ptrs = stream_ptr_table(view.csr, self.device)
             view._multi = TLFwdMultiDesc(nb.data_ptr(), nb.shape[0], self._multi.rbits, view._multi_ptrs.data_ptr(),
-                                         self._multi.il)
+                                         self._multi.il, tbits=self._multi.tbits)
         view._multi_t = None if self._multi_t is None else self._multi_t.restreamed(view.csc)
         gb = getattr(self, "_gbuckets", None)
         if gb is not None and gb[1] is not None:
@@ -810,17 +812,20 @@
 
     def _build_multi(self):
         self._multi = None
-        if not self.csr or any(ch.kind != "tl" for ch in self.csr) or len({ch.rbits for ch in self.csr}) != 1:
+        if (not self.csr or any(ch.kind != "tl" for ch in self.csr) or len({ch.rbits for ch in self.csr}) != 1
+                or len({ch.tbits for ch in self.csr}) != 1):
             return
         tabs = []
         for c, ch in enumerate(self.csr):
             b = ch.blk.to(torch.int64)
-            t = torch.empty((b.shape[0], 8), dtype=torch.int64, device=b.device)
+            t = torch.empty((b.shape[0], b.shape[1] + 2), dtype=torch.int64, device=b.device)
             t[:, 0] = c
             t[:, 1] = b[:, 0] + self.row_starts[c]
             t[:, 2:5] = b[:, 1:4]
             t[:, 5] = self.col_lo[c]
-            t[:, 6:8] = b[:, 4:6]
+            t[:, 6:] = b[:, 4:]
+            if ch.tbits:
+                t[:, 11] += self.blk_off[c]
             tabs.append(t)
         self._multi_blk = torch.cat(tabs).to(torch.int32).contiguous()
         from .tiled import stream_ptr_table
@@ -829,7 +834,7 @@
         if len({ch.il for ch in self.csr}) != 1:
             return
         self._multi = TLFwdMultiDesc(self._multi_blk.data_ptr(), self._multi_blk.shape[0], self.csr[0].rbits,
-                                     self._multi_ptrs.data_ptr(), self.csr[0].il)
+                                     self._multi_ptrs.data_ptr(), self.csr[0].il, tbits=self.csr[0].tbits)
 
     def _build_multi_t(self):
         self._multi_t = None
diff --git a/photon_ml_amd/ops/native.py b/photon_ml_amd/ops/native.py
--- a/photon_ml_amd/ops/native.py
+++ b/photon_ml_amd/ops/native.py
@@ -31,12 +31,12 @@
 
 class TLFwdDesc(ctypes.Structure):
     _fields_ = [("blk", c_void_p), ("nblk", c_int), ("rbits", c_int), ("pack", c_void_p), ("val", c_void_p),
-                ("il", c_int), ("nar", TLNarrow), ("live", c_void_p)]
+                ("il", c_int), ("nar", TLNarrow), ("live", c_void_p), ("tbits", c_int)]
 
 
 class TLFwdMultiDesc(ctypes.Structure):
     _fields_ = [("blk", c_void_p), ("nblk", c_int), ("rbits", c_int), ("ptrs", c_void_p), ("il", c_int),
-                ("live", c_void_p)]
+                ("live", c_void_p), ("tbits", c_int)]
 
 
 class TLTMultiDesc(ctypes.Structure):
@@ -50,7 +50,7 @@
                 ("sbits", c_int), ("key_is_row", c_int), ("pack", c_void_p), ("val", c_void_p),
                 ("npack", c_void_p), ("nval", c_void_p), ("nbase", c_void_p), ("keep", c_void_p),
                 ("seg_cnt", c_void_p), ("seg_first", c_void_p), ("unit_lo", c_void_p), ("opack", c_void_p),
-                ("oval", c_void_p)]
+                ("oval", c_void_p), ("ustride", c_int), ("wbits", c_int)]
 
 
 class SegRankArgs(ctypes.Structure):
diff --git a/photon_ml_amd/ops/tiled.py b/photon_ml_amd/ops/tiled.py
--- a/photon_ml_amd/ops/tiled.py
+++ b/photon_ml_amd/ops/tiled.py
@@ -43,6 +43,13 @@
 NARROW_W = 64
 FUSE = int(os.environ.get("PML_TL_FUSE", "1"))
 WIDE_BASE = int(os.environ.get("PML_TL_WIDE_BASE", "1"))
+TALL = os.environ.get("PML_TL_TALL")
+TALL = None if TALL is None else bool(int(TALL))
+TALL_DEFAULT = True
+TALL_BITS = 12
+TALL_SUB_BITS = 10
+TALL_MIN_DIM = 1 << 16
+TALL_COLS = 10
 
 
 def narrow_width(sbits: int) -> int:
@@ -110,11 +117,11 @@
     return e_lo[unit] + (j - t) + ((t & 63) << 2) + (t >> 6)
 
 
-def _interleave(pack: torch.Tensor, val: torch.Tensor, n: torch.Tensor):
+def _interleave(pack: torch.Tensor, val: torch.Tensor, n: torch.Tensor, tail: int = _PAD):
     n = n.to(torch.int64)
     padded = (n + IL_ROUND - 1) // IL_ROUND * IL_ROUND
     new_lo = torch.cumsum(padded, 0) - padded
-    total = int(padded.sum()) + _PAD
+    total = int(padded.sum()) + tail
     phys = il_phys(new_lo, n)
     p = torch.zeros(total, dtype=pack.dtype, device=pack.device)
     v = torch.zeros(total, dtype=val.dtype, device=val.device)
@@ -237,12 +244,28 @@
         return pk, vl
 
 
+def tall_engages(tall: Optional[bool], dim: int, m: int, dtype, il: int, want_rbits: int) -> bool:
+    if not (il and NARROW and dtype != torch.float64 and want_rbits == TALL_SUB_BITS):
+        return False
+    if tall is None:
+        tall = TALL
+    if tall is None:
+        tall = TALL_DEFAULT and dim >= TALL_MIN_DIM and m >= (1 << TALL_BITS)
+    return bool(tall)
+
+
+def shard_tall(dim: int, chunk_rows: int) -> Optional[bool]:
+    if TALL is not None:
+        return None
+    return bool(TALL_DEFAULT and dim >= TALL_MIN_DIM and chunk_rows >= (1 << TALL_BITS))
+
+
 class TLFwdChunk(_NarrowMixin):
 
     kind = "tl"
 
     def __init__(self, rowptr: torch.Tensor, col: torch.Tensor, val: torch.Tensor, dim: int,
-                 rbits: Optional[int] = None, il: Optional[int] = None):
+                 rbits: Optional[int] = None, il: Optional[int] = None, tall: Optional[bool] = None):
         dev = val.device
         self.il = INTERLEAVE if il is None else int(il)
         rowptr = rowptr.to(dev, torch.int64)
@@ -253,6 +276,9 @@
         if self.rbits is None:
             raise ValueError(f"tiled forward layout cannot pack dim={dim}")
         want = _cap(default_rbits(dim, f64) if rbits is None else rbits, f64)
+        self.tbits = 0
+        if tall_engages(tall, dim, m, val.dtype, self.il, want) and self._init_tall(rowptr, col, val, dim, m):
+            return
         use_base = bool(self.il) and WIDE_BASE and want > self.rbits
         if use_base:
             self.rbits = want
@@ -279,7 +305,7 @@
                 wp = self._rebase(wp, wn)
                 if wp is None:
                     del wv, npk, nvl, nbs
-                    self.__init__(rowptr, col, val, dim, fwd_bits(dim, f64, rbits), il)
+                    self.__init__(rowptr, col, val, dim, fwd_bits(dim, f64, rbits), il, tall=False)
                     return
             self.pack, self.val, e_lo = _interleave(_to_u32_bits(wp), wv, wn)
             e_hi = e_lo + wn
@@ -298,8 +324,61 @@
         self.desc = TLFwdDesc(self.blk.data_ptr(), nblk, self.rbits, self.pack.data_ptr(), self.val.data_ptr(),
                               self.il, self.nar)
 
-    def _rebase(self, wp: torch.Tensor, wn: torch.Tensor) -> Optional[torch.Tensor]:
+    def _init_tall(self, rowptr: torch.Tensor, col: torch.Tensor, val: torch.Tensor, dim: int, m: int) -> bool:
+        dev = val.device
+        S, T = TALL_SUB_BITS, TALL_BITS
+        cb = _bits(dim)
+        nnz = col.numel()
+        rows = torch.repeat_interleave(torch.arange(m, device=dev), rowptr[1:] - rowptr[:-1]) if nnz else \
+            torch.zeros(0, dtype=torch.int64, device=dev)
+        key = ((rows >> S) << (cb + S)) | (col << S) | (rows & ((1 << S) - 1))
+        del rows
+        key, perm = torch.sort(key, stable=True)
+        nunit = (m + (1 << T) - 1) >> T
+        nsub = nunit << (T - S)
+        slo = torch.clamp(torch.arange(nsub, device=dev) << S, max=m)
+        cnt = rowptr[torch.clamp(slo + (1 << S), max=m)] - rowptr[slo]
+        wp, wv, wn, npk, nvl, nbs, nr = split_narrow(key & ((1 << (cb + S)) - 1), val[perm], cnt, S, dim)
+        del key, perm
+        sub = torch.repeat_interleave(torch.arange(nsub, device=dev), wn)
+        tp = ((wp >> S) << T) | ((sub & ((1 << (T - S)) - 1)) << S) | (wp & ((1 << S) - 1))
+        ukey = ((sub >> (T - S)) << cb) | (wp >> S)
+        del sub, wp
+        if _bits(max(nunit, 1)) + cb <= 31:
+            ukey = ukey.to(torch.int32)
+        tperm = torch.sort(ukey, stable=True).indices
+        del ukey
+        tp, wv = tp[tperm], wv[tperm]
+        del tperm
+        un = wn.view(nunit, -1).sum(1)
+        if cb + T > 32:
+            tp = self._rebase(tp, un, T) if WIDE_BASE else None
+            if tp is None:
+                self.wbase = None
+                return False
+        self.rbits, self.tbits = S, T
+        self.pack, self.val, e_lo = _interleave(_to_u32_bits(tp), wv, un, tail=0)
+        del tp, wv
+        nh = torch.cumsum(nr, 0)
+        nl = (nh - nr).view(nunit, -1)
+        ulo = torch.arange(nunit, device=dev) << T
+        self._sbits, self._ew = S, (2, 3)
+        self._set_narrow(npk, nvl, nbs)
+        self.blk = torch.stack([ulo, torch.clamp(ulo + (1 << T), max=m) - ulo, e_lo, e_lo + un, nl[:, 0],
+                                nh.view(nunit, -1)[:, -1], nl[:, 1], nl[:, 2], nl[:, 3], ulo >> S],
+                               1).to(torch.int32).contiguous()
+        self.nblk, self.m, self.nnz = nunit, m, nnz
+        self.desc = TLFwdDesc(self.blk.data_ptr(), nunit, S, self.pack.data_ptr(), self.val.data_ptr(), 1, self.nar,
+                              tbits=T)
+        return True
+
+    @property
+    def ubits(self) -> int:
+        return self.tbits or self.rbits
+
+    def _rebase(self, wp: torch.Tensor, wn: torch.Tensor, bits: Optional[int] = None) -> Optional[torch.Tensor]:
         dev = wp.device
+        bits = self.rbits if bits is None else bits
         n = wn.to(torch.int64)
         tot = int(n.sum())
         padded = (n + IL_ROUND - 1) // IL_ROUND * IL_ROUND
@@ -310,21 +389,21 @@
             j = torch.arange(tot, device=dev) - (torch.cumsum(n, 0) - n)[unit]
             rid = ((torch.cumsum(padded, 0) - padded)[unit] + j) // IL_ROUND
             del unit
-            key = wp >> self.rbits
+            key = wp >> bits
             first = (j % IL_ROUND) == 0
             del j
             wbase[rid[first]] = key[first]
             rel = key - wbase[rid]
             del rid, key, first
-            if int(rel.max()) >= 1 << (32 - self.rbits):
+            if int(rel.max()) >= 1 << (32 - bits):
                 return None
-            wp = (rel << self.rbits) | (wp & ((1 << self.rbits) - 1))
+            wp = (rel << bits) | (wp & ((1 << bits) - 1))
         self.wbase = wbase.to(torch.int32).contiguous()
         return wp
 
     @property
     def nstats(self) -> int:
-        return self.nblk
+        return (self.m + (1 << self.rbits) - 1) >> self.rbits if self.tbits else self.nblk
 
     parts_needed = 0
 
@@ -340,17 +419,33 @@
             return self.pack[: self.nnz].to(torch.int64) & 0xFFFFFFFF, self.val[: self.nnz]
         ph = il_phys(self.blk[:, 2], self.blk[:, 3] - self.blk[:, 2])
         wp = self.pack[ph].to(torch.int64) & 0xFFFFFFFF
+        ub = self.ubits
         if self.wbase is not None:
-            wp = ((self.wbase[ph // IL_ROUND].to(torch.int64) + (wp >> self.rbits)) << self.rbits) | (
-                wp & ((1 << self.rbits) - 1))
-        return self._logical_all(wp, self.val[ph])
+            wp = ((self.wbase[ph // IL_ROUND].to(torch.int64) + (wp >> ub)) << ub) | (wp & ((1 << ub) - 1))
+        if not self.tbits:
+            return self._logical_all(wp, self.val[ph])
+        t = self.blk.to(torch.int64)
+        dev = wp.device
+        U = t.shape[0]
+        if not U or int((t[:, 5] - t[:, 4]).sum()) == 0:
+            return wp, self.val[ph]
+        S, T = self.rbits, self.tbits
+        npk, nvl = narrow_logical(self.npack, self.nval, self.nbase, 0, int(t[-1, 5]), S)
+        bounds = torch.stack([t[:, 4], t[:, 6], t[:, 7], t[:, 8], t[:, 5]], 1)
+        per_sub = (bounds[:, 1:] - bounds[:, :-1]).reshape(-1)
+        esub = torch.repeat_interleave(torch.arange(per_sub.numel(), device=dev), IL_ROUND * per_sub.to(dev))
+        npk = ((npk >> S) << T) | ((esub & ((1 << (T - S)) - 1)) << S) | (npk & ((1 << S) - 1))
+        unit = torch.cat([esub >> (T - S), torch.repeat_interleave(torch.arange(U, device=dev),
+                                                                   (t[:, 3] - t[:, 2]).to(dev))])
+        order = torch.sort(unit, stable=True).indices
+        return torch.cat([npk, wp])[order], torch.cat([nvl, self.val[ph]])[order]
 
     def emulate_matvec(self, x: torch.Tensor) -> torch.Tensor:
         pk, vl = self.logical()
         p = pk.to(torch.int64)
-        col = p >> self.rbits
+        col = p >> self.ubits
         blk_of_entry = torch.repeat_interleave(torch.arange(self.nblk, device=p.device), self.unit_counts())
-        row = (blk_of_entry << self.rbits) + (p & ((1 << self.rbits) - 1))
+        row = (blk_of_entry << self.ubits) + (p & ((1 << self.ubits) - 1))
         z = torch.zeros(self.m, dtype=torch.float64, device=p.device)
         return z.index_add_(0, row, vl.to(torch.float64) * x.to(torch.float64)[col])
 
@@ -632,7 +727,8 @@
                             0 if forward else 1, ch.pack.data_ptr(), ch.val.data_ptr(), ch.npack.data_ptr(),
                             None if ch.fused else ch.nval.data_ptr(), ch.nbase.data_ptr(), keep.data_ptr(),
                             self.seg_cnt.data_ptr(),
-                            None, None, None, None)
+                            None, None, None, None, table.shape[1], getattr(ch, "ubits", ch._sbits) if forward
+                            else ch._sbits)
         self.lib, self.stream = require_game_lib(), stream_handle(dev)
         self.vbytes = ch.val.element_size()
         if S:
@@ -663,7 +759,7 @@
         table[:, lo] = self.unit_lo
         table[:, hi] = self.unit_lo + self.unit_cnt
         if self.filter_narrow:
-            table[:, 4:6] = 0
+            table[:, 4:9] = 0
         table = table.to(torch.int32).contiguous()
         nc = copy.copy(ch)
         nc._cmp_seg = {}
@@ -675,7 +771,8 @@
             nc.nnz = kept + self.n_narrow
         if self.forward:
             nc.blk = table
-            nc.desc = TLFwdDesc(table.data_ptr(), nc.nblk, nc.rbits, opack.data_ptr(), oval.data_ptr(), 1, nc.nar)
+            nc.desc = TLFwdDesc(table.data_ptr(), nc.nblk, nc.rbits, opack.data_ptr(), oval.data_ptr(), 1, nc.nar,
+                                tbits=nc.tbits)
         else:
             nc.items = table
             nc.desc = TLTDesc(table.data_ptr(), nc.nitems, nc.cbits, opack.data_ptr(), oval.data_ptr(),
diff --git a/photon_ml_amd/ops/warmup.py b/photon_ml_amd/ops/warmup.py
--- a/photon_ml_amd/ops/warmup.py
+++ b/photon_ml_amd/ops/warmup.py
@@ -38,6 +38,12 @@
     torch.segment_reduce(x, "sum", lengths=torch.full((64,), 64, dtype=torch.int64, device=dev))
     x.to(torch.float32).to(torch.bfloat16)
     check_lds_add_order(dev)
+    from .device import DeviceGLMData
+    tiny = DeviceGLMData.from_device_csr(torch.arange(0, 18, 2, device=dev), i[:16] % 5, x[:16].to(torch.float32),
+                                         torch.zeros(8), torch.zeros(8), torch.ones(8), 5, dev, "f32", tall=True)
+    tiny.matvec(torch.zeros(5, dtype=torch.float64, device=dev))
+    z = torch.zeros(8, dtype=torch.float64, device=dev)
+    tiny._fwd(0, torch.zeros(5, dtype=torch.float32, device=dev), 0, 0, 0.0, None, None, z_out=z, stats=False)
     key_histogram(i % 13, 13)
     csr_gather_rows(torch.tensor([0, 2], dtype=torch.int64, device=dev), i[:2], x[:2],
                     torch.zeros(1, dtype=torch.int64, device=dev), torch.tensor([0, 4], dtype=torch.int64, device=dev))
diff --git a/photon_ml_amd/stat/summary.py b/photon_ml_amd/stat/summary.py
--- a/photon_ml_amd/stat/summary.py
+++ b/photon_ml_amd/stat/summary.py
@@ -96,7 +96,7 @@
         mn = torch.full((d,), float("inf"), dtype=f64, device=dev)
         for c, ch in enumerate(data.csr):
             pk, vl = ch.logical()
-            col = (pk.to(torch.int64) >> ch.rbits) + data.col_lo[c]
+            col = (pk.to(torch.int64) >> ch.ubits) + data.col_lo[c]
             v = vl.to(f64)
             s1.index_add_(0, col, v)
             s2.index_add_(0, col, v * v)
```

New measurement: 3.632 billion examples/sec (median of 6 runs). 1.1x the previous value.
